# wyhuai/DDNM

Hardware: NVIDIA H100
Metric: restored 256x256 images/sec @100 DDIM steps (higher is better)
Workload: dtype fp32

## Files before the change

ddnm_b200/csrc/api.cu:

```cuda
#include "../../include/ddnm_b200.h"

#include <cstring>
#include <vector>

#include "api_util.cuh"
#include "engine.cuh"
#include "kernels.cuh"
#include "tc_gemm.cuh"

using namespace ddnm;

namespace ddnm {
thread_local std::string g_last_error;
}

extern "C" {

const char* ddnm_last_error(void) { return g_last_error.c_str(); }
int ddnm_version(void) { return 100; }

int ddnm_unet_simple_create(const ddnm_simple_cfg* c, int batch, void** handle) {
  DDNM_API_BEGIN
  DDNM_CHECK(c && handle, "null argument");
  SimpleCfg cfg;
  cfg.ch = c->ch; cfg.out_ch = c->out_ch; cfg.n_levels = c->n_levels;
  DDNM_CHECK(c->n_levels >= 1 && c->n_levels <= 8 && c->n_attn_res >= 0 && c->n_attn_res <= 4, "bad config");
  for (int i = 0; i < 8; ++i) cfg.ch_mult[i] = c->ch_mult[i];
  cfg.num_res_blocks = c->num_res_blocks;
  cfg.n_attn_res = c->n_attn_res;
  for (int i = 0; i < 4; ++i) cfg.attn_res[i] = c->attn_res[i];
  cfg.in_channels = c->in_channels; cfg.resolution = c->resolution; cfg.groups = c->groups; cfg.eps = c->eps;
  *handle = static_cast<UNetEngine*>(new UNetSimple(cfg, batch));
  DDNM_API_END
}

int ddnm_unet_openai_create(const ddnm_openai_cfg* c, int batch, void** handle) {
  DDNM_API_BEGIN
  DDNM_CHECK(c && handle, "null argument");
  DDNM_CHECK(c->n_levels >= 1 && c->n_levels <= 8 && c->n_attn_ds >= 0 && c->n_attn_ds <= 4, "bad config");
  OpenAICfg cfg;
  cfg.image_size = c->image_size; cfg.model_channels = c->model_channels; cfg.num_res_blocks = c->num_res_blocks;
  cfg.n_levels = c->n_levels;
  for (int i = 0; i < 8; ++i) cfg.channel_mult[i] = c->channel_mult[i];
  cfg.n_attn_ds = c->n_attn_ds;
  for (int i = 0; i < 4; ++i) cfg.attn_ds[i] = c->attn_ds[i];
  cfg.num_head_channels = c->num_head_channels; cfg.out_channels = c->out_channels; cfg.in_channels = c->in_channels;
  cfg.groups = c->groups; cfg.eps = c->eps; cfg.num_classes = c->num_classes; cfg.low_res = c->low_res;
  cfg.num_heads = c->num_heads; cfg.num_heads_upsample = c->num_heads_upsample; cfg.new_attention_order = c->new_attention_order;
  DDNM_CHECK(c->num_classes >= 0, "bad num_classes");
  DDNM_CHECK(c->new_attention_order == 0 || c->new_attention_order == 1, "new_attention_order must be 0 or 1");
  DDNM_CHECK(c->num_head_channels > 0 || c->num_heads >= 1, "num_head_channels <= 0 needs num_heads >= 1");
  *handle = static_cast<UNetEngine*>(new UNetOpenAI(cfg, batch));
  DDNM_API_END
}

int ddnm_classifier_create(const ddnm_classifier_cfg* c, int batch, void** handle) {
  DDNM_API_BEGIN
  DDNM_CHECK(c && handle, "null argument");
  DDNM_CHECK(c->n_levels >= 1 && c->n_levels <= 8 && c->n_attn_ds >= 0 && c->n_attn_ds <= 4, "bad config");
  EncoderCfg cfg;
  cfg.image_size = c->image_size; cfg.model_channels = c->model_channels; cfg.num_res_blocks = c->num_res_blocks;
  cfg.n_levels = c->n_levels;
  for (int i = 0; i < 8; ++i) cfg.channel_mult[i] = c->channel_mult[i];
  cfg.n_attn_ds = c->n_attn_ds;
  for (int i = 0; i < 4; ++i) cfg.attn_ds[i] = c->attn_ds[i];
  cfg.num_head_channels = c->num_head_channels; cfg.out_channels = c->out_channels; cfg.in_channels = c->in_channels;
  cfg.groups = c->groups; cfg.eps = c->eps; cfg.pool = c->pool;
  *handle = static_cast<UNetEngine*>(new UNetEncoder(cfg, batch));
  DDNM_API_END
}

static UNetEncoder* as_classifier(void* h) {
  UNetEncoder* e = dynamic_cast<UNetEncoder*>(static_cast<UNetEngine*>(h));
  DDNM_CHECK(e != nullptr, "handle is not a classifier");
  return e;
}

int ddnm_classifier_forward(void* h, const float* x, const float* t, float* logits, void* stream) {
  DDNM_API_BEGIN
  DDNM_CHECK(x && t && logits, "null argument");
  as_classifier(h)->forward(x, t, logits, (cudaStream_t)stream);
  DDNM_API_END
}

int ddnm_classifier_grad(void* h, const float* x, const float* t, const int* labels, float scale, float* grad_out, float* logits_out,
                         void* stream) {
  DDNM_API_BEGIN
  as_classifier(h)->grad(x, t, labels, scale, grad_out, logits_out, (cudaStream_t)stream);
  DDNM_API_END
}

int ddnm_classifier_guidance_fn(void* user, int, int t, void* stream) {
  DDNM_API_BEGIN
  ddnm_classifier_guidance* g = static_cast<ddnm_classifier_guidance*>(user);
  DDNM_CHECK(g && g->classifier && g->x && g->labels && g->grad_buf, "incomplete guidance context");
  UNetEncoder* e = as_classifier(g->classifier);
  DDNM_CHECK(g->batch == e->batch(), "classifier was built for batch " + std::to_string(e->batch()) + ", the guided loop runs " +
                                         std::to_string(g->batch));
  cudaStream_t st = (cudaStream_t)stream;
  if (!g->labels_checked) {
    e->check_labels(g->labels, st);
    g->labels_checked = 1;
  }
  e->fill_t((float)t, st);
  e->grad(g->x, e->t_in(), g->labels, g->scale, g->grad_buf, nullptr, st, true);
  DDNM_API_END
}

int ddnm_unet_set_param(void* h, const char* name, const float* data, long long numel) {
  DDNM_API_BEGIN
  static_cast<UNetEngine*>(h)->set_param(name, data, numel);
  DDNM_API_END
}
int ddnm_unet_finalize(void* h) {
  DDNM_API_BEGIN
  static_cast<UNetEngine*>(h)->finalize();
  DDNM_API_END
}
int ddnm_unet_forward(void* h, const float* x, const float* t, float* out, void* stream) {
  DDNM_API_BEGIN
  static_cast<UNetEngine*>(h)->forward(x, t, out, (cudaStream_t)stream);
  DDNM_API_END
}
int ddnm_unet_forward_cond(void* h, const float* x, const float* t, const int* labels, float* out, void* stream) {
  DDNM_API_BEGIN
  UNetEngine* u = static_cast<UNetEngine*>(h);
  u->set_labels(labels, (cudaStream_t)stream);
  u->forward(x, t, out, (cudaStream_t)stream);
  DDNM_API_END
}
int ddnm_unet_set_low_res(void* h, const float* low_res, void* stream) {
  DDNM_API_BEGIN
  static_cast<UNetEngine*>(h)->set_low_res(low_res, (cudaStream_t)stream);
  DDNM_API_END
}
int ddnm_unet_set_precision(void* h, int fp16_terms) {
  DDNM_API_BEGIN
  static_cast<UNetEngine*>(h)->set_terms(fp16_terms);
  DDNM_API_END
}
int ddnm_unet_set_graph(void* h, int on) {
  DDNM_API_BEGIN
  static_cast<UNetEngine*>(h)->set_use_graph(on != 0);
  DDNM_API_END
}
int ddnm_unet_read_tap(void* h, const char* name, float* dst, long long cap, void* stream) {
  DDNM_API_BEGIN
  DDNM_CHECK(static_cast<UNetEngine*>(h)->read_tap(name, dst, cap, (cudaStream_t)stream), std::string("unknown tap ") + name);
  DDNM_API_END
}
int ddnm_unet_info(void* h, long long* ws, int* launches, double* flops) {
  DDNM_API_BEGIN
  UNetEngine* u = static_cast<UNetEngine*>(h);
  if (ws) *ws = (long long)u->workspace_bytes();
  if (launches) *launches = u->num_launches();
// ... 145 lines not shown

int ddnm_conv_tc_bench(int N, int H, int W, int Cin, int Cout, int mode, int iters, float* ms_per_iter, double* flops) {
  DDNM_API_BEGIN
  const bool random = iters < 0;
  if (random) iters = -iters;
  const int feat = mode >> 4;
  mode &= 15;
  const bool up2 = (feat & 8) != 0;
  Tmp tmp;
  const int taps = up2 ? 4 : (mode == TAPS_1X1 ? 1 : 9);
  const size_t pe = (size_t)N * H * W * Cin;
  SplitView A;
  A.hi = tmp.get<__half>(pe); A.lo = tmp.get<__half>(pe); A.N = N; A.H = H; A.W = W; A.C = Cin;
  float* xf = tmp.get<float>(pe);
  CUDA_CHECK(cudaMemset(xf, 0, pe * 4));
  if (random) bench_fill_f32<<<(unsigned)cdivll((long long)pe, 256), 256>>>(xf, (long long)pe, 0x1234u);
  gn_apply_split(mkview(xf, N, H, W, Cin), 1, false, nullptr, nullptr, 0.f, false, SPLIT_SAME, A.hi, A.lo, 0);
  const int ktot = taps * Cin;
  __half* wh = tmp.get<__half>((size_t)Cout * ktot);
  __half* wl = tmp.get<__half>((size_t)Cout * ktot);
  CUDA_CHECK(cudaMemset(wh, 0, (size_t)Cout * ktot * 2));
  CUDA_CHECK(cudaMemset(wl, 0, (size_t)Cout * ktot * 2));
  if (random) {
    const long long wn = (long long)Cout * ktot;
    bench_fill_split<<<(unsigned)cdivll(wn, 256), 256>>>(wh, wl, wn, 0x9876u, 1.0f / sqrtf((float)ktot));
  }
  const int oH = up2 ? 2 * H : H, oW = up2 ? 2 * W : W;
  const size_t oe = (size_t)N * oH * oW * Cout;
  float* o = tmp.get<float>(oe);
  View ov = mkview(o, N, oH, oW, Cout);
  if (feat & 1) {
    ov.st = tmp.get<StatAcc>((size_t)N * Cout * 2);
    ov.st_ld = Cout;
    CUDA_CHECK(cudaMemset(ov.st, 0, (size_t)N * Cout * 2 * sizeof(StatAcc)));
  }
  float* res = nullptr;
  if (feat & 2) {
    res = tmp.get<float>(oe);
    CUDA_CHECK(cudaMemset(res, 0, oe * 4));
    if (random) bench_fill_f32<<<(unsigned)cdivll((long long)oe, 256), 256>>>(res, (long long)oe, 0x777u);
  }
  float* ca = nullptr;
  if (feat & 4) {
    ca = tmp.get<float>((size_t)N * Cout);
    CUDA_CHECK(cudaMemset(ca, 0, (size_t)N * Cout * 4));
  }
  TcLaunch L = up2 ? tc_make_up2_launch(A, wh, wl, Cout, ov, ca, Cout, 0, 0, sm_count())
                   : tc_make_launch(A, mode, nullptr, wh, wl, 1, Cout, ov, ca, Cout, res, Cout, 1.0f, sm_count());
  for (int i = 0; i < 3; ++i) tc_run(L, 0);
  cudaEvent_t e0, e1;
  CUDA_CHECK(cudaEventCreate(&e0));
  CUDA_CHECK(cudaEventCreate(&e1));
  CUDA_CHECK(cudaEventRecord(e0, 0));
  for (int i = 0; i < iters; ++i) tc_run(L, 0);
  CUDA_CHECK(cudaEventRecord(e1, 0));
  CUDA_CHECK(cudaEventSynchronize(e1));
  float ms = 0;
  CUDA_CHECK(cudaEventElapsedTime(&ms, e0, e1));
  cudaEventDestroy(e0);
  cudaEventDestroy(e1);
  *ms_per_iter = ms / iters;
  *flops = L.flops;
  DDNM_API_END
}

int ddnm_gnconv_chunk_bench(int N, int chunk, int H, int W, int Cin, int Cout, int iters, float* ms_per_pass) {
  DDNM_API_BEGIN
  DDNM_CHECK(chunk >= 1 && N % chunk == 0, "chunk must divide N");
  Tmp tmp;
  const size_t pe = (size_t)N * H * W * Cin, ce = (size_t)chunk * H * W * Cin, oe = (size_t)N * H * W * Cout;
  float* x = tmp.get<float>(pe);
  bench_fill_f32<<<(unsigned)cdivll((long long)pe, 256), 256>>>(x, (long long)pe, 0x4321u);
  StatAcc* st = tmp.get<StatAcc>((size_t)N * Cin * 2);
  CUDA_CHECK(cudaMemset(st, 0, (size_t)N * Cin * 2 * sizeof(StatAcc)));
  View xv = mkview(x, N, H, W, Cin);
  xv.st = st; xv.st_ld = Cin;
  gn_stats(xv, 0);
  float* gamma = tmp.get<float>(Cin);
  float* beta = tmp.get<float>(Cin);
  bench_fill_f32<<<cdiv(Cin, 256), 256>>>(gamma, Cin, 0x11u);
  bench_fill_f32<<<cdiv(Cin, 256), 256>>>(beta, Cin, 0x22u);
  SplitView A;
  A.hi = tmp.get<__half>(ce); A.lo = tmp.get<__half>(ce); A.N = chunk; A.H = H; A.W = W; A.C = Cin;
  const int ktot = 9 * Cin;
  __half* wh = tmp.get<__half>((size_t)Cout * ktot);
  __half* wl = tmp.get<__half>((size_t)Cout * ktot);
  bench_fill_split<<<(unsigned)cdivll((long long)Cout * ktot, 256), 256>>>(wh, wl, (long long)Cout * ktot, 0x9876u, 1.0f / sqrtf((float)ktot));
  float* o = tmp.get<float>(oe);
  StatAcc* ost = tmp.get<StatAcc>((size_t)N * Cout * 2);
  CUDA_CHECK(cudaMemset(ost, 0, (size_t)N * Cout * 2 * sizeof(StatAcc)));
  float* ca = tmp.get<float>((size_t)N * Cout);
  CUDA_CHECK(cudaMemset(ca, 0, (size_t)N * Cout * 4));
  const int nch = N / chunk;
  std::vector<View> xs;
  std::vector<TcLaunch> Ls;
  for (int c = 0; c < nch; ++c) {
    View xc = xv;
    xc.p = x + (size_t)c * chunk * H * W * Cin; xc.N = chunk; xc.st = st + (size_t)c * chunk * Cin * 2;
    View oc = mkview(o + (size_t)c * chunk * H * W * Cout, chunk, H, W, Cout);
    oc.st = ost + (size_t)c * chunk * Cout * 2; oc.st_ld = Cout;
    xs.push_back(xc);
    Ls.push_back(tc_make_launch(A, TAPS_3X3, nullptr, wh, wl, 1, Cout, oc, ca + (size_t)c * chunk * Cout, Cout, nullptr, 0, 1.0f, sm_count()));
  }
  auto pass = [&]() {
    for (int c = 0; c < nch; ++c) {
      gn_apply_split(xs[c], 32, true, gamma, beta, 1e-6f, true, SPLIT_SAME, A.hi, A.lo, 0);
      tc_run(Ls[c], 0);
    }
  };
  for (int i = 0; i < 2; ++i) pass();
  cudaEvent_t e0, e1;
  CUDA_CHECK(cudaEventCreate(&e0));
  CUDA_CHECK(cudaEventCreate(&e1));
  CUDA_CHECK(cudaEventRecord(e0, 0));
  for (int i = 0; i < iters; ++i) pass();
  CUDA_CHECK(cudaEventRecord(e1, 0));
  CUDA_CHECK(cudaEventSynchronize(e1));
  float ms = 0;
  CUDA_CHECK(cudaEventElapsedTime(&ms, e0, e1));
  cudaEventDestroy(e0);
  cudaEventDestroy(e1);
  *ms_per_pass = ms / iters;
  DDNM_API_END
}

int ddnm_groupnorm(const float* x, int N, int H, int W, int C, int groups, const float* gamma, const float* beta, float eps,
                   int silu, float* out, void* stream) {
  DDNM_API_BEGIN
  cudaStream_t s = (cudaStream_t)stream;
  Tmp tmp;
  StatAcc* st = tmp.get<StatAcc>((size_t)N * C * 2);
  CUDA_CHECK(cudaMemsetAsync(st, 0, (size_t)N * C * 2 * sizeof(StatAcc), s));
  View xv = mkview(const_cast<float*>(x), N, H, W, C);
  xv.st = st;
  xv.st_ld = C;
  gn_stats(xv, s);
  gn_apply_f32(xv, groups, gamma, beta, eps, silu != 0, out, s);
  CUDA_CHECK(cudaStreamSynchronize(s));
  DDNM_API_END
}

int ddnm_conv_gn_tc(const float* x, int N, int H, int W, int Cin, int groups, const float* gamma, const float* beta, float eps, int silu,
                    const float* w, const float* bias, int Cout, const float* side_x, int CinSide, const float* side_w,
                    const float* residual, float* out, int iters, float* ms_per_iter, void* stream) {
  DDNM_API_BEGIN
  cudaStream_t s = (cudaStream_t)stream;
  Tmp tmp;
  View xv = mkview(const_cast<float*>(x), N, H, W, Cin);
  StatAcc* st = tmp.get<StatAcc>((size_t)N * Cin * 2);
  CUDA_CHECK(cudaMemsetAsync(st, 0, (size_t)N * Cin * 2 * sizeof(StatAcc), s));
  xv.st = st;
  xv.st_ld = Cin;
  if (gamma) gn_stats(xv, s);
  View sv;
  if (side_x) sv = mkview(const_cast<float*>(side_x), N, H, W, CinSide);
  const int ktot = 9 * Cin + (side_x ? CinSide : 0);
  __half* wh = tmp.get<__half>((size_t)Cout * ktot);
  __half* wl = tmp.get<__half>((size_t)Cout * ktot);
  split_conv_weight(w, Cout, Cin, 9, wh, wl, ktot, 0, s);
  if (side_x) split_conv_weight(side_w, Cout, CinSide, 1, wh, wl, ktot, 9 * Cin, s);
  GnAffine gn;
  gn.gamma = gamma; gn.beta = beta; gn.eps = eps; gn.groups = groups; gn.silu = silu != 0;
  View ov = mkview(out, N, H, W, Cout);
  TcLaunch L = tc_make_gn_launch(xv, gn, side_x ? &sv : nullptr, wh, wl, Cout, ov, bias, 0, residual, Cout, sm_count());
  tc_run(L, s);
  if (iters > 0 && ms_per_iter) {
    cudaEvent_t e0, e1;
    CUDA_CHECK(cudaEventCreate(&e0));
    CUDA_CHECK(cudaEventCreate(&e1));
    for (int i = 0; i < 2; ++i) tc_run(L, s);
    CUDA_CHECK(cudaEventRecord(e0, s));
    for (int i = 0; i < iters; ++i) tc_run(L, s);
    CUDA_CHECK(cudaEventRecord(e1, s));
    CUDA_CHECK(cudaEventSynchronize(e1));
    float ms = 0;
    CUDA_CHECK(cudaEventElapsedTime(&ms, e0, e1));
    cudaEventDestroy(e0);
    cudaEventDestroy(e1);
    *ms_per_iter = ms / iters;
  }
  CUDA_CHECK(cudaStreamSynchronize(s));
  DDNM_API_END
}
int ddnm_tc_debug_gn_fused(int on) {
  DDNM_API_BEGIN
  tc_debug_gn_fused(on);
  DDNM_API_END
}
int ddnm_tc_debug_deal(int mode) {
  DDNM_API_BEGIN
  tc_debug_deal(mode);
  DDNM_API_END
}
int ddnm_tc_debug_pair_mode(int mode) {
  DDNM_API_BEGIN
  tc_debug_pair_mode(mode);
  DDNM_API_END
}
int ddnm_tc_debug_dual_mode(int mode) {
  DDNM_API_BEGIN
  tc_debug_dual_mode(mode);
  DDNM_API_END
}
int ddnm_tc_debug_pair_dual(int on) {
  DDNM_API_BEGIN
  tc_debug_pair_dual(on);
  DDNM_API_END
}
int ddnm_tc_debug_halo(int on) {
  DDNM_API_BEGIN
  tc_debug_halo(on);
  DDNM_API_END
}
int ddnm_tc_debug_pingpong(int on) {
  DDNM_API_BEGIN
  tc_debug_pingpong(on);
  DDNM_API_END
}
int ddnm_tc_debug_force_bn(int bn) {
  DDNM_API_BEGIN
  tc_debug_force_bn(bn);
  DDNM_API_END
}
}
```

ddnm_b200/csrc/common.cuh:

```cuda
#pragma once
#include <cuda_runtime.h>
#include <cuda_fp16.h>
#include <cuda.h>
#include <cstdint>
#include <cstdio>
#include <stdexcept>
#include <string>

namespace ddnm {

struct Error : std::runtime_error {
  using std::runtime_error::runtime_error;
};

#define DDNM_CHECK(cond, msg)                                                                     \
  do {                                                                                            \
    if (!(cond)) throw ::ddnm::Error(std::string(msg) + " [" #cond "] at " __FILE__ ":" + std::to_string(__LINE__)); \
  } while (0)

#define CUDA_CHECK(expr)                                                                          \
  do {                                                                                            \
    cudaError_t _e = (expr);                                                                      \
    if (_e != cudaSuccess)                                                                        \
      throw ::ddnm::Error(std::string("CUDA error: ") + cudaGetErrorString(_e) + " in " #expr " at " __FILE__ ":" + \
// ... 83 lines not shown
__device__ __forceinline__ void pdl_prologue() {
  asm volatile("griddepcontrol.launch_dependents;" ::: "memory");
  asm volatile("griddepcontrol.wait;" ::: "memory");
}
__device__ __forceinline__ uint32_t smem_u32(const void* p) { return (uint32_t)__cvta_generic_to_shared(p); }

__device__ __forceinline__ void mbar_init(uint32_t bar, uint32_t count) {
  asm volatile("mbarrier.init.shared::cta.b64 [%0], %1;" ::"r"(bar), "r"(count));
}
__device__ __forceinline__ void mbar_fence_init() { asm volatile("fence.mbarrier_init.release.cluster;" ::: "memory"); }
__device__ __forceinline__ void mbar_expect_tx(uint32_t bar, uint32_t bytes) {
  asm volatile("mbarrier.arrive.expect_tx.shared::cta.b64 _, [%0], %1;" ::"r"(bar), "r"(bytes) : "memory");
}
__device__ __forceinline__ void mbar_arrive(uint32_t bar) {
  asm volatile("mbarrier.arrive.shared::cta.b64 _, [%0];" ::"r"(bar) : "memory");
}
__device__ __forceinline__ bool mbar_try_wait(uint32_t bar, uint32_t parity) {
  uint32_t ok;
  asm volatile(
      "{\n\t.reg .pred p;\n\t"
      "mbarrier.try_wait.parity.shared::cta.b64 p, [%1], %2;\n\t"
      "selp.u32 %0, 1, 0, p;\n\t}"
      : "=r"(ok)
      : "r"(bar), "r"(parity)
      : "memory");
  return ok != 0;
}
__device__ __forceinline__ void mbar_wait(uint32_t bar, uint32_t parity) {
  if (mbar_try_wait(bar, parity)) return;
  long long t0 = clock64();
  while (!mbar_try_wait(bar, parity)) {
    if (clock64() - t0 > 4000000000LL) __trap();
  }
}

__device__ __forceinline__ void tma_prefetch_desc(const void* tmap) {
  asm volatile("prefetch.tensormap [%0];" ::"l"(tmap) : "memory");
}
__device__ __forceinline__ void tma_load_2d(uint32_t dst, const void* tmap, uint32_t bar, int c0, int c1) {
  asm volatile(
      "cp.async.bulk.tensor.2d.shared::cluster.global.tile.mbarrier::complete_tx::bytes [%0], [%1, {%3, %4}], [%2];" ::"r"(dst),
      "l"(tmap), "r"(bar), "r"(c0), "r"(c1)
      : "memory");
}
__device__ __forceinline__ void tma_load_3d(uint32_t dst, const void* tmap, uint32_t bar, int c0, int c1, int c2) {
  asm volatile(
      "cp.async.bulk.tensor.3d.shared::cluster.global.tile.mbarrier::complete_tx::bytes [%0], [%1, {%3, %4, %5}], [%2];" ::"r"(dst),
      "l"(tmap), "r"(bar), "r"(c0), "r"(c1), "r"(c2)
      : "memory");
}
__device__ __forceinline__ void tma_load_4d(uint32_t dst, const void* tmap, uint32_t bar, int c0, int c1, int c2, int c3) {
  asm volatile(
      "cp.async.bulk.tensor.4d.shared::cluster.global.tile.mbarrier::complete_tx::bytes [%0], [%1, {%3, %4, %5, %6}], [%2];" ::"r"(dst),
      "l"(tmap), "r"(bar), "r"(c0), "r"(c1), "r"(c2), "r"(c3)
      : "memory");
}

__device__ __forceinline__ uint64_t wgmma_desc_sw128(uint32_t saddr) {
  return (uint64_t)((saddr & 0x3FFFFu) >> 4) | ((uint64_t)1 << 16) | ((uint64_t)(1024 >> 4) << 32) | ((uint64_t)1 << 62);
}
__device__ __forceinline__ void wgmma_fence() { asm volatile("wgmma.fence.sync.aligned;" ::: "memory"); }
__device__ __forceinline__ void wgmma_commit() { asm volatile("wgmma.commit_group.sync.aligned;" ::: "memory"); }
template <int N>
__device__ __forceinline__ void wgmma_wait() { asm volatile("wgmma.wait_group.sync.aligned %0;" ::"n"(N) : "memory"); }
__device__ __forceinline__ void wgmma_m64n64k16(float (&d)[32], uint64_t a_desc, uint64_t b_desc, uint32_t accumulate) {
  asm volatile(
      "{\n\t.reg .pred p;\n\t"
      "setp.ne.b32 p, %34, 0;\n\t"
      "wgmma.mma_async.sync.aligned.m64n64k16.f32.f16.f16 "
      "{%0, %1, %2, %3, %4, %5, %6, %7, %8, %9, %10, %11, %12, %13, %14, %15, %16, %17, %18, %19, %20, %21, %22, %23, %24, %25, %26, %27, %28, %29, %30, %31}, "
      "%32, %33, p, 1, 1, 0, 0;\n\t}"
      : "+f"(d[0]), "+f"(d[1]), "+f"(d[2]), "+f"(d[3]), "+f"(d[4]), "+f"(d[5]), "+f"(d[6]), "+f"(d[7]), "+f"(d[8]), "+f"(d[9]), "+f"(d[10]), "+f"(d[11]), "+f"(d[12]), "+f"(d[13]), "+f"(d[14]), "+f"(d[15]), "+f"(d[16]), "+f"(d[17]), "+f"(d[18]), "+f"(d[19]), "+f"(d[20]), "+f"(d[21]), "+f"(d[22]), "+f"(d[23]), "+f"(d[24]), "+f"(d[25]), "+f"(d[26]), "+f"(d[27]), "+f"(d[28]), "+f"(d[29]), "+f"(d[30]), "+f"(d[31])
      : "l"(a_desc), "l"(b_desc), "r"(accumulate));
}
__device__ __forceinline__ void wgmma_m64n128k16(float (&d)[64], uint64_t a_desc, uint64_t b_desc, uint32_t accumulate) {
  asm volatile(
      "{\n\t.reg .pred p;\n\t"
      "setp.ne.b32 p, %66, 0;\n\t"
      "wgmma.mma_async.sync.aligned.m64n128k16.f32.f16.f16 "
      "{%0, %1, %2, %3, %4, %5, %6, %7, %8, %9, %10, %11, %12, %13, %14, %15, %16, %17, %18, %19, %20, %21, %22, %23, %24, %25, %26, %27, %28, %29, %30, %31, %32, %33, %34, %35, %36, %37, %38, %39, %40, %41, %42, %43, %44, %45, %46, %47, %48, %49, %50, %51, %52, %53, %54, %55, %56, %57, %58, %59, %60, %61, %62, %63}, "
      "%64, %65, p, 1, 1, 0, 0;\n\t}"
      : "+f"(d[0]), "+f"(d[1]), "+f"(d[2]), "+f"(d[3]), "+f"(d[4]), "+f"(d[5]), "+f"(d[6]), "+f"(d[7]), "+f"(d[8]), "+f"(d[9]), "+f"(d[10]), "+f"(d[11]), "+f"(d[12]), "+f"(d[13]), "+f"(d[14]), "+f"(d[15]), "+f"(d[16]), "+f"(d[17]), "+f"(d[18]), "+f"(d[19]), "+f"(d[20]), "+f"(d[21]), "+f"(d[22]), "+f"(d[23]), "+f"(d[24]), "+f"(d[25]), "+f"(d[26]), "+f"(d[27]), "+f"(d[28]), "+f"(d[29]), "+f"(d[30]), "+f"(d[31]), "+f"(d[32]), "+f"(d[33]), "+f"(d[34]), "+f"(d[35]), "+f"(d[36]), "+f"(d[37]), "+f"(d[38]), "+f"(d[39]), "+f"(d[40]), "+f"(d[41]), "+f"(d[42]), "+f"(d[43]), "+f"(d[44]), "+f"(d[45]), "+f"(d[46]), "+f"(d[47]), "+f"(d[48]), "+f"(d[49]), "+f"(d[50]), "+f"(d[51]), "+f"(d[52]), "+f"(d[53]), "+f"(d[54]), "+f"(d[55]), "+f"(d[56]), "+f"(d[57]), "+f"(d[58]), "+f"(d[59]), "+f"(d[60]), "+f"(d[61]), "+f"(d[62]), "+f"(d[63])
      : "l"(a_desc), "l"(b_desc), "r"(accumulate));
}
__device__ __forceinline__ void wgmma_m64n256k16(float (&d)[128], uint64_t a_desc, uint64_t b_desc, uint32_t accumulate) {
  asm volatile(
      "{\n\t.reg .pred p;\n\t"
      "setp.ne.b32 p, %130, 0;\n\t"
      "wgmma.mma_async.sync.aligned.m64n256k16.f32.f16.f16 "
      "{%0, %1, %2, %3, %4, %5, %6, %7, %8, %9, %10, %11, %12, %13, %14, %15, %16, %17, %18, %19, %20, %21, %22, %23, %24, %25, %26, %27, %28, %29, %30, %31, %32, %33, %34, %35, %36, %37, %38, %39, %40, %41, %42, %43, %44, %45, %46, %47, %48, %49, %50, %51, %52, %53, %54, %55, %56, %57, %58, %59, %60, %61, %62, %63, %64, %65, %66, %67, %68, %69, %70, %71, %72, %73, %74, %75, %76, %77, %78, %79, %80, %81, %82, %83, %84, %85, %86, %87, %88, %89, %90, %91, %92, %93, %94, %95, %96, %97, %98, %99, %100, %101, %102, %103, %104, %105, %106, %107, %108, %109, %110, %111, %112, %113, %114, %115, %116, %117, %118, %119, %120, %121, %122, %123, %124, %125, %126, %127}, "
      "%128, %129, p, 1, 1, 0, 0;\n\t}"
      : "+f"(d[0]), "+f"(d[1]), "+f"(d[2]), "+f"(d[3]), "+f"(d[4]), "+f"(d[5]), "+f"(d[6]), "+f"(d[7]), "+f"(d[8]), "+f"(d[9]), "+f"(d[10]), "+f"(d[11]), "+f"(d[12]), "+f"(d[13]), "+f"(d[14]), "+f"(d[15]), "+f"(d[16]), "+f"(d[17]), "+f"(d[18]), "+f"(d[19]), "+f"(d[20]), "+f"(d[21]), "+f"(d[22]), "+f"(d[23]), "+f"(d[24]), "+f"(d[25]), "+f"(d[26]), "+f"(d[27]), "+f"(d[28]), "+f"(d[29]), "+f"(d[30]), "+f"(d[31]), "+f"(d[32]), "+f"(d[33]), "+f"(d[34]), "+f"(d[35]), "+f"(d[36]), "+f"(d[37]), "+f"(d[38]), "+f"(d[39]), "+f"(d[40]), "+f"(d[41]), "+f"(d[42]), "+f"(d[43]), "+f"(d[44]), "+f"(d[45]), "+f"(d[46]), "+f"(d[47]), "+f"(d[48]), "+f"(d[49]), "+f"(d[50]), "+f"(d[51]), "+f"(d[52]), "+f"(d[53]), "+f"(d[54]), "+f"(d[55]), "+f"(d[56]), "+f"(d[57]), "+f"(d[58]), "+f"(d[59]), "+f"(d[60]), "+f"(d[61]), "+f"(d[62]), "+f"(d[63]), "+f"(d[64]), "+f"(d[65]), "+f"(d[66]), "+f"(d[67]), "+f"(d[68]), "+f"(d[69]), "+f"(d[70]), "+f"(d[71]), "+f"(d[72]), "+f"(d[73]), "+f"(d[74]), "+f"(d[75]), "+f"(d[76]), "+f"(d[77]), "+f"(d[78]), "+f"(d[79]), "+f"(d[80]), "+f"(d[81]), "+f"(d[82]), "+f"(d[83]), "+f"(d[84]), "+f"(d[85]), "+f"(d[86]), "+f"(d[87]), "+f"(d[88]), "+f"(d[89]), "+f"(d[90]), "+f"(d[91]), "+f"(d[92]), "+f"(d[93]), "+f"(d[94]), "+f"(d[95]), "+f"(d[96]), "+f"(d[97]), "+f"(d[98]), "+f"(d[99]), "+f"(d[100]), "+f"(d[101]), "+f"(d[102]), "+f"(d[103]), "+f"(d[104]), "+f"(d[105]), "+f"(d[106]), "+f"(d[107]), "+f"(d[108]), "+f"(d[109]), "+f"(d[110]), "+f"(d[111]), "+f"(d[112]), "+f"(d[113]), "+f"(d[114]), "+f"(d[115]), "+f"(d[116]), "+f"(d[117]), "+f"(d[118]), "+f"(d[119]), "+f"(d[120]), "+f"(d[121]), "+f"(d[122]), "+f"(d[123]), "+f"(d[124]), "+f"(d[125]), "+f"(d[126]), "+f"(d[127])
      : "l"(a_desc), "l"(b_desc), "r"(accumulate));
}
__device__ __forceinline__ uint32_t cluster_ctarank() {
  uint32_t r;
  asm volatile("mov.u32 %0, %%cluster_ctarank;" : "=r"(r));
  return r;
}
__device__ __forceinline__ uint32_t cluster_id_x() {
  uint32_t r;
  asm volatile("mov.u32 %0, %%clusterid.x;" : "=r"(r));
  return r;
}
__device__ __forceinline__ void cluster_sync_all() {
  asm volatile("barrier.cluster.arrive.release.aligned;" ::: "memory");
  asm volatile("barrier.cluster.wait.acquire.aligned;" ::: "memory");
}
__device__ __forceinline__ void mbar_arrive_cluster(uint32_t bar, uint32_t cta) {
  uint32_t remote;
  asm volatile("mapa.shared::cluster.u32 %0, %1, %2;" : "=r"(remote) : "r"(bar), "r"(cta));
  asm volatile("mbarrier.arrive.release.cluster.shared::cluster.b64 _, [%0];" ::"r"(remote) : "memory");
}
__device__ __forceinline__ void tma_load_3d_multicast(uint32_t dst, const void* tmap, uint32_t bar, int c0, int c1, int c2, uint16_t mask) {
  asm volatile(
      "cp.async.bulk.tensor.3d.shared::cluster.global.mbarrier::complete_tx::bytes.multicast::cluster [%0], [%1, {%3, %4, %5}], [%2], %6;" ::"r"(dst),
      "l"(tmap), "r"(bar), "r"(c0), "r"(c1), "r"(c2), "h"(mask)
      : "memory");
}
__device__ __forceinline__ void named_bar_sync(int id, int threads) { asm volatile("bar.sync %0, %1;" ::"r"(id), "r"(threads) : "memory"); }
template <int R>
__device__ __forceinline__ void setmaxnreg_dec() { asm volatile("setmaxnreg.dec.sync.aligned.u32 %0;" ::"n"(R)); }
template <int R>
__device__ __forceinline__ void setmaxnreg_inc() { asm volatile("setmaxnreg.inc.sync.aligned.u32 %0;" ::"n"(R)); }

__device__ __forceinline__ void stat_add(StatAcc* acc, float p) {
  const int bits = __float_as_int(p);
  int ex = (bits >> 23) & 0xff;
  unsigned long long m = (unsigned long long)(bits & 0x7fffff);
  if (ex) m |= 0x800000ull; else ex = 1;
  const int sh = ex - 150 + 48;
  unsigned long long lo = 0, hi = 0;
  if (sh >= 64) hi = m << min(sh - 64, 7);
  else if (sh > 0) { lo = m << sh; hi = sh > 40 ? m >> (64 - sh) : 0ull; }
  else if (sh > -24) lo = m >> (-sh);
  if (bits < 0) {
    lo = ~lo + 1ull;
    hi = ~hi + (lo == 0ull ? 1ull : 0ull);
  }
  const unsigned long long w0 = lo & 0xffffffffull;
  const unsigned long long w1 = (hi << 32) | (lo >> 32);
  if (w0) atomicAdd(&acc->lo, w0);
  if (w1) atomicAdd(reinterpret_cast<unsigned long long*>(&acc->hi), w1);
}
__device__ __forceinline__ void two_sum_acc(float& sum, float& comp, float v) {
  const float s = __fadd_rn(sum, v);
  const float bb = __fadd_rn(s, -sum);
  comp = __fadd_rn(comp, __fadd_rn(__fadd_rn(sum, -__fadd_rn(s, -bb)), __fadd_rn(v, -bb)));
  sum = s;
}
__device__ __forceinline__ double stat_value(const StatAcc& a) {
  return ((double)a.hi * 4294967296.0 + (double)a.lo) * (1.0 / 281474976710656.0);
}

__device__ __forceinline__ float swishf_fast(float x) {
  float e;
  asm("ex2.approx.ftz.f32 %0, %1;" : "=f"(e) : "f"(x * -1.4426950408889634f));
  return __fdividef(x, 1.0f + e);
}
__device__ __forceinline__ void split_f16(float x, __half& hi, __half& lo) {
  unsigned short h;
  asm("cvt.rn.satfinite.f16.f32 %0, %1;" : "=h"(h) : "f"(x));
  hi = __ushort_as_half(h);
  float r = x - __half2float(hi);
  asm("cvt.rn.satfinite.f16.f32 %0, %1;" : "=h"(h) : "f"(r));
  lo = __ushort_as_half(h);
}
__device__ __forceinline__ void split2_f16(float x0, float x1, uint32_t& hi, uint32_t& lo) {
  asm("cvt.rn.satfinite.f16x2.f32 %0, %1, %2;" : "=r"(hi) : "f"(x1), "f"(x0));
  const __half2 h = *reinterpret_cast<const __half2*>(&hi);
  const float2 f = __half22float2(h);
  asm("cvt.rn.satfinite.f16x2.f32 %0, %1, %2;" : "=r"(lo) : "f"(x1 - f.y), "f"(x0 - f.x));
}

#endif

}
```

ddnm_b200/csrc/engine.cu:

```cuda
#include "engine.cuh"

#include <algorithm>
#include <cmath>
#include <cstdlib>
#include <sstream>

#include "kernels.cuh"

namespace ddnm {

Arena::~Arena() {
  for (void* b : blocks_) cudaFree(b);
}
void* Arena::alloc(size_t bytes) {
  bytes = (bytes + 1023) / 1024 * 1024;
  if (bytes == 0) bytes = 1024;
  void* p = nullptr;
  CUDA_CHECK(cudaMalloc(&p, bytes));
  blocks_.push_back(p);
  total_ += bytes;
  return p;
}

UNetEngine::UNetEngine(int batch, int in_channels, int out_ch, int resolution, int groups, float eps)
    : B_(batch), in_ch_(in_channels), out_ch_(out_ch), R_(resolution), groups_(groups), eps_(eps) {
  DDNM_CHECK(batch >= 1, "batch must be positive");
  int dev = 0;
  CUDA_CHECK(cudaGetDevice(&dev));
  cudaDeviceProp prop;
  CUDA_CHECK(cudaGetDeviceProperties(&prop, dev));
  DDNM_CHECK(prop.major == 9 && prop.minor == 0, "ddnm_b200 kernels are built for sm_90a (H100) only");
  num_sms_ = prop.multiProcessorCount;
}

UNetEngine::~UNetEngine() {
  if (graph_exec_) cudaGraphExecDestroy(graph_exec_);
  if (graph_) cudaGraphDestroy(graph_);
  for (auto& kv : params_) cudaFree(kv.second.p);
}

void UNetEngine::set_param(const std::string& name, const float* data, long long numel) {
  DDNM_CHECK(!finalized_, "set_param after finalize");
  DDNM_CHECK(numel > 0 && data != nullptr, "empty parameter " + name);
  float* d = nullptr;
  CUDA_CHECK(cudaMalloc(&d, (size_t)numel * sizeof(float)));
  CUDA_CHECK(cudaMemcpy(d, data, (size_t)numel * sizeof(float), cudaMemcpyDefault));
  auto it = params_.find(name);
  if (it != params_.end()) cudaFree(it->second.p);
  params_[name] = Param{d, numel};
}

const float* UNetEngine::P(const std::string& name, long long expect) const {
  auto it = params_.find(name);
  DDNM_CHECK(it != params_.end(), "missing parameter '" + name + "'");
  if (expect >= 0)
    DDNM_CHECK(it->second.n == expect, "parameter '" + name + "' has " + std::to_string(it->second.n) + " elements, expected " +
                                           std::to_string(expect));
  return it->second.p;
}

View UNetEngine::new_view(int H, int W, int C) {
  View v;
  v.N = B_; v.H = H; v.W = W; v.C = C; v.ld = C;
  v.p = (float*)arena_.alloc((size_t)B_ * H * W * C * sizeof(float));
  v.st = new_stats(C);
  v.st_ld = C;
  return v;
}

StatAcc* UNetEngine::new_stats(int C) {
  const size_t need = (size_t)B_ * C * 2;
  if (stats_chunks_.empty() || stats_chunks_.back().used + need > stats_chunks_.back().cap) {
    StatsChunk c;
    c.cap = std::max<size_t>(need, (size_t)1 << 20);
    c.used = 0;
    c.p = (StatAcc*)arena_.alloc(c.cap * sizeof(StatAcc));
    stats_chunks_.push_back(c);
  }
  StatsChunk& c = stats_chunks_.back();
  StatAcc* p = c.p + c.used;
  c.used += need;
  return p;
}

UNetEngine::TcWeights UNetEngine::prep_weights(const std::string& main, int Cout, int Cin, int taps, const std::string& side,
                                               int CinSide) {
  TcWeights w;
  w.ktot = taps * Cin + CinSide;
  const size_t n = (size_t)Cout * w.ktot;
  w.hi = (__half*)arena_.alloc(n * sizeof(__half));
  w.lo = (__half*)arena_.alloc(n * sizeof(__half));
  split_conv_weight(P(main, (long long)Cout * Cin * taps), Cout, Cin, taps, w.hi, w.lo, w.ktot, 0, 0);
  if (CinSide) split_conv_weight(P(side, (long long)Cout * CinSide), Cout, CinSide, 1, w.hi, w.lo, w.ktot, taps * Cin, 0);
  return w;
}

const float* UNetEngine::bias_sum(const std::string& a, const std::string& b, int C) {
  std::vector<float> ha(C), hb(C, 0.f);
  CUDA_CHECK(cudaMemcpy(ha.data(), P(a, C), C * sizeof(float), cudaMemcpyDeviceToHost));
  if (!b.empty()) CUDA_CHECK(cudaMemcpy(hb.data(), P(b, C), C * sizeof(float), cudaMemcpyDeviceToHost));
  for (int i = 0; i < C; ++i) ha[i] += hb[i];
  float* d = (float*)arena_.alloc(C * sizeof(float));
  CUDA_CHECK(cudaMemcpy(d, ha.data(), C * sizeof(float), cudaMemcpyHostToDevice));
  return d;
}

float* UNetEngine::dev_copy(const std::vector<float>& v) {
  float* d = (float*)arena_.alloc(v.size() * sizeof(float));
  CUDA_CHECK(cudaMemcpy(d, v.data(), v.size() * sizeof(float), cudaMemcpyHostToDevice));
  return d;
}

void UNetEngine::add_op(const std::string& name, const std::string& kind, double flops, double bytes,
                        std::function<void(cudaStream_t)> f) {
  ops_.push_back(OpRecord{name, kind, flops, bytes, std::move(f)});
}

void UNetEngine::emit_gn_split(const std::string& name, const View& x, const std::string& norm, bool silu, int mode,
                               SplitView& dst, const float* ss, int ss_ld, SplitView* raw) {
  const long long out_elems = mode == SPLIT_AVG2 ? x.pixels() * x.C / 4 : x.pixels() * x.C;
  DDNM_CHECK((size_t)out_elems <= split_elems_, "split scratch too small");
  dst.C = x.C;
  if (mode == SPLIT_SAME) { dst.N = x.N; dst.H = x.H; dst.W = x.W; }
  else if (mode == SPLIT_AVG2) { dst.N = x.N; dst.H = x.H / 2; dst.W = x.W / 2; }
  else { dst.N = 4 * x.N; dst.H = x.H / 2; dst.W = x.W / 2; }
  const double in_bytes = (double)x.pixels() * x.C * 4;
  if (!norm.empty()) {
    DDNM_CHECK(x.st != nullptr, "GroupNorm input without producer-side statistics: " + name);
    const float* g = P(norm + ".weight", x.C);
    const float* b = P(norm + ".bias", x.C);
    const int groups = groups_;
    const float eps = eps_;
    __half *hi = dst.hi, *lo = dst.lo, *rhi = nullptr, *rlo = nullptr;
    if (raw) {
      DDNM_CHECK(mode == SPLIT_SAME, "raw side output only with the plain split");
      raw->N = x.N; raw->H = x.H; raw->W = x.W; raw->C = x.C;
      rhi = raw->hi; rlo = raw->lo;
    }
    add_op(name + ".gn_split", "gn_split", 0, in_bytes + out_elems * 4.0 * (raw ? 2 : 1),
           [=](cudaStream_t s) { gn_apply_split(x, groups, true, g, b, eps, silu, mode, hi, lo, s, ss, ss_ld, rhi, rlo); });
  } else {
    __half *hi = dst.hi, *lo = dst.lo;
    add_op(name + ".split", "gn_split", 0, in_bytes + out_elems * 4.0,
           [=](cudaStream_t s) { gn_apply_split(x, 1, false, nullptr, nullptr, 0.f, silu, mode, hi, lo, s); });
  }
}

void UNetEngine::emit_tc(const std::string& name, const SplitView& a, int mode, const SplitView* side, const TcWeights& w,
                         int Cout, const View& out, const float* chanadd, int ca_ld, const float* residual, int ldr, int res_mode) {
  TcLaunch L = tc_make_launch(a, mode, side, w.hi, w.lo, 1, Cout, out, chanadd, ca_ld, residual, ldr, 1.0f, num_sms_, res_mode);
  const double bytes = (double)a.N * a.H * a.W * a.C * 4 + (side ? (double)side->N * side->H * side->W * side->C * 4 : 0) +
                       (double)Cout * w.ktot * 4 + (double)out.pixels() * Cout * 4 * (residual ? 2 : 1);
  const int tiles = L.p.tiles_x * L.p.tiles_y * L.p.tiles_n * L.p.n_tiles, kblocks = L.p.kb0 + L.p.kb1;
  static const bool split_on = std::getenv("DDNM_SPLITK") == nullptr || std::atoi(std::getenv("DDNM_SPLITK")) != 0;
  if (split_on && !L.pair && res_mode == 0 && 2 * tiles <= num_sms_ && kblocks >= 32) {
    const int S = 4 * tiles <= num_sms_ ? 4 : 2;
    const long long stride = out.pixels() * Cout;
    float* part = (float*)arena_.alloc((size_t)S * stride * sizeof(float));
    View pv;
    pv.p = part; pv.N = out.N; pv.H = out.H; pv.W = out.W; pv.C = Cout; pv.ld = Cout;
    TcLaunch Ls = tc_make_launch(a, mode, side, w.hi, w.lo, 1, Cout, pv, nullptr, 0, nullptr, 0, 1.0f, num_sms_, 0);
    DDNM_CHECK(!Ls.pair && Ls.BN == L.BN, "split-K: tile shape changed");
    Ls.p.split_k = S;
    Ls.p.split_stride = stride;
    Ls.halo = false;
    Ls.grid = std::min(tiles * S, num_sms_);
    add_op(name, "tc", L.flops, bytes, [Ls](cudaStream_t s) { tc_run(Ls, s); });
    add_op(name + ".splitk_reduce", "reduce", 0, (double)(S + 1 + (residual ? 1 : 0)) * stride * 4,
           [=](cudaStream_t s) { splitk_reduce(part, S, stride, out, chanadd, ca_ld, residual, ldr, s); });
    return;
  }
  add_op(name, "tc", L.flops, bytes, [L](cudaStream_t s) { tc_run(L, s); });
}

bool UNetEngine::fused_ok(const View& x, const View* side, int Cout, const View& out) const {
  return terms_ == 3 && x.st != nullptr && tc_gn_eligible(x, side, Cout, out);
}

void UNetEngine::emit_tcgn(const std::string& name, const View& x, const std::string& norm, const float* ss, int ss_ld, const View* side,
                           const TcWeights& w, int Cout, const View& out, const float* chanadd, int ca_ld, const float* residual, int ldr) {
  GnAffine gn;
  gn.gamma = P(norm + ".weight", x.C);
  gn.beta = P(norm + ".bias", x.C);
  gn.eps = eps_;
  gn.groups = groups_;
  gn.silu = true;
  gn.ss = ss;
  gn.ss_ld = ss_ld;
  TcLaunch L = tc_make_gn_launch(x, gn, side, w.hi, w.lo, Cout, out, chanadd, ca_ld, residual, ldr, num_sms_);
  const double bytes = (double)x.pixels() * x.C * 4 + (side ? (double)side->pixels() * side->C * 4 : 0) + (double)Cout * w.ktot * 4 +
                       (double)out.pixels() * Cout * 4 * (residual ? 2 : 1);
  add_op(name, "tc", L.flops, bytes, [L](cudaStream_t s) { tc_run(L, s); });
}

void UNetEngine::alloc_common(size_t split_elems, size_t hbuf_elems) {
  split_elems_ = split_elems;
  hbuf_elems_ = hbuf_elems;
  splitA_hi_ = (__half*)arena_.alloc(split_elems * 2);
  splitA_lo_ = (__half*)arena_.alloc(split_elems * 2);
  splitB_hi_ = (__half*)arena_.alloc(split_elems * 2);
  splitB_lo_ = (__half*)arena_.alloc(split_elems * 2);
  hbuf_ = (float*)arena_.alloc(hbuf_elems * 4);
  x_in_ = (float*)arena_.alloc((size_t)B_ * in_ch_ * R_ * R_ * 4);
  t_in_ = (float*)arena_.alloc((size_t)B_ * 4);
  labels_in_ = (int*)arena_.alloc((size_t)B_ * 4);
  CUDA_CHECK(cudaMemset(labels_in_, 0, (size_t)B_ * 4));
  out_ = (float*)arena_.alloc((size_t)B_ * out_ch_ * R_ * R_ * 4);
  if (lowres_ > 0) lowres_in_ = (float*)arena_.alloc((size_t)B_ * in_ch_ * lowres_ * lowres_ * 4);
}

void UNetEngine::emit_up2_conv(const std::string& name, const SplitView& a, const std::string& wname, int Cout, const View& out,
                               const float* chanadd, int ca_ld) {
  const int Cin = a.C;
  const size_t per_phase = (size_t)Cout * 4 * Cin;
  __half* wh = (__half*)arena_.alloc(4 * per_phase * sizeof(__half));
  __half* wl = (__half*)arena_.alloc(4 * per_phase * sizeof(__half));
  presum_up2_weights(P(wname, (long long)Cout * Cin * 9), Cout, Cin, wh, wl, 0);
  for (int ph = 0; ph < 4; ++ph) {
    TcLaunch L = tc_make_up2_launch(a, wh + ph * per_phase, wl + ph * per_phase, Cout, out, chanadd, ca_ld, ph >> 1, ph & 1, num_sms_);
    const double bytes = (double)a.N * a.H * a.W * Cin * 4 + (double)per_phase * 4 + (double)a.N * a.H * a.W * Cout * 4;
    add_op(name + ".ph" + std::to_string(ph), "tc", L.flops, bytes, [L](cudaStream_t s) { tc_run(L, s); });
  }
}

void UNetEngine::alloc_attention(size_t qkv_elems, size_t s_elems, size_t o_elems) {
  qkv_ = (float*)arena_.alloc(qkv_elems * 4);
  attS_ = (float*)arena_.alloc(s_elems * 4);
  attO_ = (float*)arena_.alloc(o_elems * 4);
  qkvh_ = (__half*)arena_.alloc(qkv_elems * 2);
  qkvl_ = (__half*)arena_.alloc(qkv_elems * 2);
  ph_ = (__half*)arena_.alloc(s_elems * 2);
  pl_ = (__half*)arena_.alloc(s_elems * 2);
  vth_ = (__half*)arena_.alloc(o_elems * 2);
  vtl_ = (__half*)arena_.alloc(o_elems * 2);
}

void UNetEngine::emit_attention_core(const std::string& name, int T, int heads, int ch, int qkv_ld, int head_stride, int q_off,
                                     int k_off, int v_off, float alpha) {
  float *q = qkv_, *S = attS_, *O = attO_;
  const int Bn = B_, C = heads * ch;
  const long long img = (long long)T * qkv_ld;
  const double fl = 2.0 * Bn * heads * (double)T * T * ch;
  const double sbytes = (double)Bn * heads * T * T * 4;
  if (T % 128 == 0 && ch % 8 == 0) {
    __half *qh = qkvh_, *ql = qkvl_, *ph = ph_, *pl = pl_, *vh = vth_, *vl = vtl_;
    DDNM_CHECK(qkv_ld % C == 0, "qkv row is not a multiple of the attention width");
    View qv;
    qv.p = qkv_; qv.N = B_; qv.H = 1; qv.W = T * (qkv_ld / C); qv.C = C; qv.ld = C;
    add_op(name + ".qkv_split", "gn_split", 0, (double)Bn * T * qkv_ld * 8,
           [=](cudaStream_t s) { gn_apply_split(qv, 1, false, nullptr, nullptr, 0.f, false, SPLIT_SAME, qh, ql, s); });
    const long long hs = head_stride ? head_stride : qkv_ld;
    GemmOperand A{qh + q_off, ql + q_off, qkv_ld, hs, img};
    GemmOperand Bk{qh + k_off, ql + k_off, qkv_ld, hs, img};
    TcLaunch L1 = tc_make_gemm_launch(A, Bk, T, T, ch, heads, Bn, S, (long long)heads * T * T, (long long)T * T, T, alpha, num_sms_);
    add_op(name + ".qk", "tc", L1.flops, (double)Bn * T * qkv_ld * 4 + sbytes, [L1](cudaStream_t s) { tc_run(L1, s); });
    add_op(name + ".softmax", "softmax", 0, sbytes * 2, [=](cudaStream_t s) { softmax_split(S, (long long)Bn * heads * T, T, ph, pl, s); });
    add_op(name + ".v_transpose", "gn_split", 0, (double)Bn * T * C * 8,
           [=](cudaStream_t s) { transpose_split(q, qkv_ld, head_stride, v_off, Bn, T, heads, ch, vh, vl, s); });
    GemmOperand P{ph, pl, T, (long long)T * T, (long long)heads * T * T};
    GemmOperand Vt{vh, vl, T, (long long)ch * T, (long long)heads * ch * T};
    TcLaunch L2 = tc_make_gemm_launch(P, Vt, T, ch, T, heads, Bn, O, (long long)T * C, ch, C, 1.0f, num_sms_);
    add_op(name + ".pv", "tc", L2.flops, sbytes + (double)Bn * T * C * 8, [L2](cudaStream_t s) { tc_run(L2, s); });
  } else {
    add_op(name + ".qk", "sgemm", fl, (double)Bn * heads * T * (2.0 * ch + T) * 4, [=](cudaStream_t s) {
      sgemm_batched(true, Bn, heads, T, T, ch, alpha, q + q_off, qkv_ld, img, head_stride, q + k_off, qkv_ld, img, head_stride, S, T,
                    (long long)heads * T * T, (long long)T * T, s);
    });
    add_op(name + ".softmax", "softmax", 0, sbytes * 2, [=](cudaStream_t s) { softmax_rows(S, (long long)Bn * heads * T, T, s); });
    add_op(name + ".pv", "sgemm", fl, (double)Bn * heads * T * (2.0 * ch + T) * 4, [=](cudaStream_t s) {
      sgemm_batched(false, Bn, heads, T, ch, T, 1.0f, S, T, (long long)heads * T * T, (long long)T * T, q + v_off, qkv_ld, img, head_stride, O,
                    C, (long long)T * C, ch, s);
    });
  }
}

void UNetEngine::emit_stem(const std::string& wname, const View& out) {
  const float* xin = x_in_;
  if (lowres_ > 0) {
    const float *w = P(wname + ".weight", (long long)out.C * 2 * in_ch_ * 9), *b = P(wname + ".bias", out.C);
    const float* lr = lowres_in_;
    const int cin = in_ch_, s = lowres_;
    add_op("stem.sr", "stem", 2.0 * B_ * R_ * R_ * (double)out.C * 2 * cin * 9,
           (double)B_ * (R_ * R_ * (cin + out.C) + (double)s * s * cin) * 4,
           [=](cudaStream_t st) { conv3x3_stem_sr(xin, lr, cin, s, s, w, b, out, st); });
    return;
  }
  const float *w = P(wname + ".weight", (long long)out.C * in_ch_ * 9), *b = P(wname + ".bias", out.C);
  const int cin = in_ch_;
  add_op("stem", "stem", 2.0 * B_ * R_ * R_ * (double)out.C * cin * 9, (double)B_ * R_ * R_ * (cin + out.C) * 4,
         [=](cudaStream_t s) { conv3x3_small_cin(xin, cin, w, b, out, s); });
}

void UNetEngine::emit_head(const std::string& norm, const std::string& conv, const View& fh) {
  DDNM_CHECK(fh.st != nullptr, "head input without statistics");
  DDNM_CHECK(out_ch_ <= 64, "head convolution: out_ch <= 64");
  if (head_conv_supported(fh, out_ch_) && std::getenv("DDNM_HEAD_TC") == nullptr) {
    const float *g = P(norm + ".weight", fh.C), *b = P(norm + ".bias", fh.C);
    const float *w = P(conv + ".weight", (long long)out_ch_ * fh.C * 9), *cb = P(conv + ".bias", out_ch_);
    const int groups = groups_, oc = out_ch_;
    const float eps = eps_;
    float* o = out_;
    add_op("head.conv", "head", 2.0 * fh.pixels() * (double)oc * fh.C * 9, (double)fh.pixels() * (fh.C + oc) * 4,
           [=](cudaStream_t s) { head_conv(fh, groups, g, b, eps, w, cb, oc, o, s); });
    return;
  }
  SplitView A{splitA_hi_, splitA_lo_};
  emit_gn_split("head", fh, norm, true, SPLIT_SAME, A);
  const int ktot = 9 * fh.C;
  TcWeights w;
  w.ktot = ktot;
  w.hi = (__half*)arena_.alloc((size_t)64 * ktot * sizeof(__half));
  w.lo = (__half*)arena_.alloc((size_t)64 * ktot * sizeof(__half));
  CUDA_CHECK(cudaMemset(w.hi, 0, (size_t)64 * ktot * sizeof(__half)));
  CUDA_CHECK(cudaMemset(w.lo, 0, (size_t)64 * ktot * sizeof(__half)));
  split_conv_weight(P(conv + ".weight", (long long)out_ch_ * fh.C * 9), out_ch_, fh.C, 9, w.hi, w.lo, ktot, 0, 0);
  std::vector<float> hb(64, 0.f);
  CUDA_CHECK(cudaMemcpy(hb.data(), P(conv + ".bias", out_ch_), out_ch_ * sizeof(float), cudaMemcpyDeviceToHost));
  float* bias64 = dev_copy(hb);
  View o64;
  o64.N = B_; o64.H = fh.H; o64.W = fh.W; o64.C = 64; o64.ld = 64;
  o64.p = (float*)arena_.alloc((size_t)B_ * fh.H * fh.W * 64 * sizeof(float));
  emit_tc("head.conv", A, TAPS_3X3, nullptr, w, 64, o64, bias64, 0, nullptr, 0);
  float* o = out_;
  const View real = o64.slice(0, out_ch_);
  add_op("head.to_nchw", "head", 0, (double)fh.pixels() * (64 + out_ch_) * 4, [=](cudaStream_t s) { nhwc_to_nchw(real, o, s); });
}

void UNetEngine::set_terms(int t) {
  DDNM_CHECK(!finalized_, "precision must be chosen before finalize");
  DDNM_CHECK(t == 1 || t == 3, "terms must be 1 (fast fp16) or 3 (fp32-grade)");
  terms_ = t;
}

void UNetEngine::finalize() {
  DDNM_CHECK(!finalized_, "finalize called twice");
  const int prev = tc_get_terms();
  tc_set_terms(terms_);
  try {
    build_program();
  } catch (...) {
    tc_set_terms(prev);
    throw;
  }
  tc_set_terms(prev);
// ... 113 lines not shown
```

ddnm_b200/csrc/engine.cuh:

```cuda
#pragma once
#include <functional>
#include <map>
#include <memory>
#include <string>
#include <vector>

#include "common.cuh"
#include "tc_gemm.cuh"

namespace ddnm {

struct SimpleCfg {
  int ch = 128, out_ch = 3, n_levels = 6;
  int ch_mult[8] = {1, 1, 2, 2, 4, 4, 0, 0};
  int num_res_blocks = 2;
  int n_attn_res = 1;
  int attn_res[4] = {16, 0, 0, 0};
  int in_channels = 3, resolution = 256, groups = 32;
  float eps = 1e-6f;
};

class Arena {
 public:
  ~Arena();
  void* alloc(size_t bytes);
  size_t used() const { return total_; }

 private:
  std::vector<void*> blocks_;
  size_t total_ = 0;
};

struct OpRecord {
  std::string name;
  std::string kind;
  double flops = 0;
  double bytes = 0;
  std::function<void(cudaStream_t)> run;
};

struct OpenAICfg {
  int image_size = 256, model_channels = 256, num_res_blocks = 2, n_levels = 6;
  int channel_mult[8] = {1, 1, 2, 2, 4, 4, 0, 0};
  int n_attn_ds = 3;
  int attn_ds[4] = {8, 16, 32, 0};
  int num_head_channels = 64;
  int out_channels = 6, in_channels = 3, groups = 32;
  float eps = 1e-5f;
  int num_classes = 0;
  int low_res = 0;
  int num_heads = 1, num_heads_upsample = -1;
  int new_attention_order = 0;
};

class UNetEngine {
 public:
  UNetEngine(int batch, int in_channels, int out_ch, int resolution, int groups, float eps);
  virtual ~UNetEngine();
  void set_param(const std::string& name, const float* data, long long numel);
  void finalize();
  void forward(const float* x, const float* t, float* out, cudaStream_t stream);
  bool read_tap(const std::string& name, float* dst_nchw, long long capacity, cudaStream_t stream);
  std::string profile(const float* x, const float* t, float* out, cudaStream_t stream);
  int batch() const { return B_; }
  int out_ch() const { return out_ch_; }
  int in_channels() const { return in_ch_; }
  int resolution() const { return R_; }
  float* x_in() const { return x_in_; }
  float* t_in() const { return t_in_; }
  int* labels_in() const { return labels_in_; }
  bool class_conditional() const { return class_cond_; }
  void set_labels(const int* labels_dev, cudaStream_t stream);
  int low_res_size() const { return lowres_; }
  void set_low_res(const float* low_res_dev, cudaStream_t stream);
  float* out_buf() const { return out_; }
  void set_use_graph(bool on) { use_graph_ = on; }
  void set_terms(int t);
  size_t workspace_bytes() const { return arena_.used(); }
  int num_launches() const { return (int)ops_.size(); }
  double flops_per_forward() const;

 protected:
  struct Param { float* p; long long n; };
  const float* P(const std::string& name, long long expect = -1) const;
  View new_view(int H, int W, int C);
  StatAcc* new_stats(int C);
  struct TcWeights { __half *hi, *lo; int ktot; };
  TcWeights prep_weights(const std::string& main, int Cout, int Cin, int taps, const std::string& side, int CinSide);
  const float* bias_sum(const std::string& a, const std::string& b, int C);
  float* dev_copy(const std::vector<float>& v);
  bool has_param(const std::string& name) const { return params_.count(name) != 0; }

  void add_op(const std::string& name, const std::string& kind, double flops, double bytes, std::function<void(cudaStream_t)> f);
  void emit_gn_split(const std::string& name, const View& x, const std::string& norm, bool silu, int mode, SplitView& dst,
                     const float* ss = nullptr, int ss_ld = 0, SplitView* raw = nullptr);
  void emit_tc(const std::string& name, const SplitView& a, int mode, const SplitView* side, const TcWeights& w, int Cout,
               const View& out, const float* chanadd, int ca_ld, const float* residual, int ldr, int res_mode = 0);
  bool fused_ok(const View& x, const View* side, int Cout, const View& out) const;
  void emit_tcgn(const std::string& name, const View& x, const std::string& norm, const float* ss, int ss_ld, const View* side,
                 const TcWeights& w, int Cout, const View& out, const float* chanadd, int ca_ld, const float* residual, int ldr);
  void emit_attention_core(const std::string& name, int T, int heads, int ch, int qkv_ld, int head_stride, int q_off, int k_off,
                           int v_off, float alpha);
  void alloc_attention(size_t qkv_elems, size_t s_elems, size_t o_elems);
  void emit_up2_conv(const std::string& name, const SplitView& a, const std::string& wname, int Cout, const View& out,
                     const float* chanadd, int ca_ld);
  void emit_stem(const std::string& wname, const View& out);
  void emit_head(const std::string& norm, const std::string& conv, const View& h);
  void alloc_common(size_t split_elems, size_t hbuf_elems);
  virtual void build_program() = 0;
  virtual size_t out_elems() const { return (size_t)B_ * out_ch_ * R_ * R_; }
  void run_ops(cudaStream_t s, size_t n = (size_t)-1);
  void replay(cudaStream_t stream, size_t n, cudaGraph_t& g, cudaGraphExec_t& exec);

  int B_, in_ch_, out_ch_, R_, groups_;
  float eps_;
  int num_sms_ = 132;
  bool finalized_ = false, use_graph_ = true;
  int terms_ = 3;
  Arena arena_;
  std::map<std::string, Param> params_;
  std::vector<OpRecord> ops_;
  size_t n_tail_ops_ = 0;
  std::map<std::string, View> taps_;
  float *x_in_ = nullptr, *t_in_ = nullptr, *out_ = nullptr;
  int* labels_in_ = nullptr;
  bool class_cond_ = false;
  float* lowres_in_ = nullptr;
  int lowres_ = 0;
  bool lowres_set_ = false;
  __half *splitA_hi_ = nullptr, *splitA_lo_ = nullptr, *splitB_hi_ = nullptr, *splitB_lo_ = nullptr;
  size_t split_elems_ = 0;
  float* hbuf_ = nullptr;
  size_t hbuf_elems_ = 0;
  float *qkv_ = nullptr, *attS_ = nullptr, *attO_ = nullptr;
  __half *qkvh_ = nullptr, *qkvl_ = nullptr, *ph_ = nullptr, *pl_ = nullptr, *vth_ = nullptr, *vtl_ = nullptr;
  struct StatsChunk { StatAcc* p; size_t cap, used; };
  std::vector<StatsChunk> stats_chunks_;
  float *emb_ = nullptr, *temb0_ = nullptr, *temb_ = nullptr, *ca_all_ = nullptr, *freq_ = nullptr;
  int ca_total_ = 0;
  std::map<std::string, int> ca_off_;
  float *tembW_all_ = nullptr, *tembB_all_ = nullptr;
  cudaGraph_t graph_ = nullptr;
  cudaGraphExec_t graph_exec_ = nullptr;
};

class UNetSimple : public UNetEngine {
 public:
  UNetSimple(const SimpleCfg& cfg, int batch);

 private:
  void build_program() override;
  void emit_resblock(const std::string& p, const View& x, const View& out);
  void emit_attn(const std::string& p, const View& x, const View& out);
  void emit_downsample(const std::string& p, const View& x, const View& out);
  void emit_upsample(const std::string& p, const View& x, const View& out);
  SimpleCfg cfg_;
};

class UNetOpenAI : public UNetEngine {
 public:
  UNetOpenAI(const OpenAICfg& cfg, int batch);

 private:
  enum ResKind { RES_PLAIN = 0, RES_DOWN = 1, RES_UP = 2 };
  void build_program() override;
  void emit_resblock(const std::string& p, const View& x, const View& out, int kind);
  int attn_heads(int C, bool upsample) const;
  void emit_attn(const std::string& p, const View& x, const View& out, int heads);
  OpenAICfg cfg_;
  float* ss_all_ = nullptr;
  int ss_total_ = 0;
  std::map<std::string, int> ss_off_;
  float *embW_all_ = nullptr, *embB_all_ = nullptr;
};

struct EncoderCfg {
  int image_size = 256, model_channels = 128, num_res_blocks = 2, n_levels = 6;
  int channel_mult[8] = {1, 1, 2, 2, 4, 4, 0, 0};
  int n_attn_ds = 3;
  int attn_ds[4] = {8, 16, 32, 0};
  int num_head_channels = 64;
  int out_channels = 1000, in_channels = 3, groups = 32;
  float eps = 1e-5f;
  int pool = 1;
};

class UNetEncoder : public UNetEngine {
 public:
  UNetEncoder(const EncoderCfg& cfg, int batch);
  ~UNetEncoder() override;
  void grad(const float* x, const float* t, const int* labels, float scale, float* grad_out, float* logits, cudaStream_t stream,
            bool labels_checked = false);
  void check_labels(const int* labels, cudaStream_t stream) const;
  void fill_t(float t, cudaStream_t stream);
  int num_classes() const { return cfg_.out_channels; }

 private:
  void build_program() override;
  size_t out_elems() const override { return (size_t)B_ * cfg_.out_channels; }
  struct Res { std::string p; View x, h, out; bool down, skip_conv; };
  struct Attn { std::string p; View x, out; float* qkv; };
  struct Layer { int kind; Res r; Attn a; };
  void emit_resblock(const std::string& p, const View& x, const View& out, bool down, Layer& rec);
  void emit_attn(const std::string& p, const View& x, const View& out, Layer& rec);
  void emit_head(const View& h);
  void emit_backward(const View& stem_out, const std::vector<Layer>& layers, const View& top);
  void emit_gn_backward(const std::string& name, const float* g, const View& x, const std::string& norm, const float* ss, int ss_ld,
                        bool silu, bool pool, const float* add, bool add_pool, float* dx32, const SplitView& dst);
  TcWeights prep_weights_t(const std::string& w, int Cout, int Cin, int taps);
  EncoderCfg cfg_;
  float* ss_all_ = nullptr;
  int ss_total_ = 0;
  std::map<std::string, int> ss_off_;
  float *embW_all_ = nullptr, *embB_all_ = nullptr;
  int headT_ = 0;
  float *hf_ = nullptr, *tok_ = nullptr, *hqkv_ = nullptr, *hp_ = nullptr, *ha0_ = nullptr;
  float *scale_in_ = nullptr, *grad_ = nullptr, *gx_[2] = {nullptr, nullptr}, *g1_ = nullptr, *g2_ = nullptr, *gqkv_ = nullptr;
  float *sP_ = nullptr, *sdP_ = nullptr, *gnb_part_ = nullptr;
  size_t gnb_part_elems_ = 0;
  cudaGraph_t ggraph_ = nullptr;
  cudaGraphExec_t ggraph_exec_ = nullptr;
};

}
```

ddnm_b200/csrc/kernels.cu:

```cuda
#include <cstdlib>

#include "kernels.cuh"
#include "tc_gemm.cuh"

namespace ddnm {

static constexpr int MAX_C = 2048;

bool pdl_enabled() {
  static const bool on = [] {
    const char* v = std::getenv("DDNM_PDL");
    return !(v && v[0] == '0');
  }();
  return on;
}

__device__ __forceinline__ float swishf(float x) { return x / (1.0f + expf(-x)); }

__global__ void gn_stats_kernel(const float* __restrict__ x, int HW, int C, int ld, int pix_per_cta,
                                StatAcc* __restrict__ stats, int st_ld) {
  pdl_prologue();
  const int n = blockIdx.y;
  const int C4 = C >> 2;
  const int rows = blockDim.x / C4;
  const int c4 = threadIdx.x % C4;
  const int prow = threadIdx.x / C4;
  const int p0 = blockIdx.x * pix_per_cta;
  const int p1 = min(HW, p0 + pix_per_cta);
  float s[4] = {0, 0, 0, 0}, q[4] = {0, 0, 0, 0};
  if (prow < rows) {
    const float* base = x + (long long)n * HW * ld + c4 * 4;
    const size_t step = (size_t)rows * ld;
    int p = p0 + prow;
    const float* ptr = base + (size_t)p * ld;
    for (; p + 3 * rows < p1; p += 4 * rows, ptr += 4 * step) {
      const float4 v0 = __ldg(reinterpret_cast<const float4*>(ptr));
      const float4 v1 = __ldg(reinterpret_cast<const float4*>(ptr + step));
      const float4 v2 = __ldg(reinterpret_cast<const float4*>(ptr + 2 * step));
      const float4 v3 = __ldg(reinterpret_cast<const float4*>(ptr + 3 * step));
      s[0] += (v0.x + v1.x) + (v2.x + v3.x); q[0] += (v0.x * v0.x + v1.x * v1.x) + (v2.x * v2.x + v3.x * v3.x);
      s[1] += (v0.y + v1.y) + (v2.y + v3.y); q[1] += (v0.y * v0.y + v1.y * v1.y) + (v2.y * v2.y + v3.y * v3.y);
      s[2] += (v0.z + v1.z) + (v2.z + v3.z); q[2] += (v0.z * v0.z + v1.z * v1.z) + (v2.z * v2.z + v3.z * v3.z);
      s[3] += (v0.w + v1.w) + (v2.w + v3.w); q[3] += (v0.w * v0.w + v1.w * v1.w) + (v2.w * v2.w + v3.w * v3.w);
    }
    for (; p < p1; p += rows, ptr += step) {
      const float4 v = __ldg(reinterpret_cast<const float4*>(ptr));
      s[0] += v.x; q[0] += v.x * v.x;
      s[1] += v.y; q[1] += v.y * v.y;
      s[2] += v.z; q[2] += v.z * v.z;
      s[3] += v.w; q[3] += v.w * v.w;
    }
#pragma unroll
    for (int j = 0; j < 4; ++j) {
      StatAcc* d = stats + ((size_t)n * st_ld + c4 * 4 + j) * 2;
      stat_add(d, s[j]);
      stat_add(d + 1, q[j]);
    }
  }
}

void gn_stats(const View& x, cudaStream_t st) {
  DDNM_CHECK(x.C % 4 == 0 && x.C <= MAX_C && x.ld % 4 == 0 && x.st != nullptr, "gn_stats: unsupported channel count / no stats slot");
  const int C4 = x.C / 4;
  const int rows = std::max(1, 256 / C4);
  const int threads = C4 * rows;
  const int HW = x.H * x.W;
  long long want = cdivll((long long)HW * x.N, 592);
  int ppc = (int)std::max<long long>(rows * 4, cdivll(want, rows) * rows);
  dim3 grid(cdiv(HW, ppc), x.N);
  launch_pdl(gn_stats_kernel, grid, dim3(threads), 0, st, 1, (const float*)x.p, HW, x.C, x.ld, ppc, x.st, x.st_ld);
  CUDA_CHECK(cudaGetLastError());
}

template <bool F32OUT>
__global__ void gn_apply_kernel(const float* __restrict__ x, int H, int W, int C, int ld, int N, int groups,
                                const StatAcc* __restrict__ stats, int st_ld, const float* __restrict__ gamma,
                                const float* __restrict__ beta, float eps, int silu, int mode, int pix_per_cta,
                                __half* __restrict__ hi, __half* __restrict__ lo, float* __restrict__ out32,
                                const float* __restrict__ ss, int ss_ld, __half* __restrict__ raw_hi,
                                __half* __restrict__ raw_lo) {
  pdl_prologue();
  extern __shared__ double gn_smem[];
  double* sd = gn_smem;
  float* sc = reinterpret_cast<float*>(gn_smem + 2 * (size_t)C);
  float* sh = sc + C;
  const int n = blockIdx.y;
  const int HW = H * W;
  if (stats) {
    const int cpg = C / groups;
    const double cnt = (double)HW * cpg;
    const StatAcc* gsrc = stats + (size_t)n * st_ld * 2;
    for (int c = threadIdx.x; c < 2 * C; c += blockDim.x) sd[c] = stat_value(gsrc[c]);
    __syncthreads();
    for (int c = threadIdx.x; c < C; c += blockDim.x) {
      const int g0 = (c / cpg) * cpg;
      double s1 = 0, s2 = 0;
      for (int j = 0; j < cpg; ++j) {
        s1 += sd[2 * (g0 + j)];
        s2 += sd[2 * (g0 + j) + 1];
      }
      const double mean = s1 / cnt;
      double var = s2 / cnt - mean * mean;
      var = var < 0 ? 0 : var;
      const float rstd = (float)(1.0 / sqrt(var + (double)eps));
      float a = rstd * gamma[c];
      float b = beta[c] - (float)mean * a;
      if (ss) {
        const float one_plus = 1.0f + ss[(size_t)n * ss_ld + c];
        a *= one_plus;
        b = fmaf(b, one_plus, ss[(size_t)n * ss_ld + C + c]);
      }
      sc[c] = a;
      sh[c] = b;
    }
  } else {
    for (int c = threadIdx.x; c < C; c += blockDim.x) {
      sc[c] = 1.f;
      sh[c] = 0.f;
    }
  }
  __syncthreads();
  const int C8 = C >> 3;
  const int rows = blockDim.x / C8;
  const int c8 = threadIdx.x % C8, prow = threadIdx.x / C8;
  if (prow >= rows) return;
  const int c = c8 * 8;
  float a8[8], b8[8];
#pragma unroll
  for (int j = 0; j < 8; ++j) { a8[j] = sc[c + j]; b8[j] = sh[c + j]; }
  const int p0 = blockIdx.x * pix_per_cta;
  if (mode == SPLIT_AVG2) {
    const int Wo = W >> 1, HWo = (H >> 1) * Wo;
    const int q1 = min(HWo, p0 + pix_per_cta);
    for (int q = p0 + prow; q < q1; q += rows) {
      const int oy = q / Wo, ox = q - oy * Wo;
      float acc[8] = {0, 0, 0, 0, 0, 0, 0, 0};
#pragma unroll
      for (int d = 0; d < 4; ++d) {
        const float* sp = x + ((size_t)n * HW + (size_t)(2 * oy + (d >> 1)) * W + 2 * ox + (d & 1)) * ld + c;
        const float4 a = __ldg(reinterpret_cast<const float4*>(sp));
        const float4 b = __ldg(reinterpret_cast<const float4*>(sp + 4));
        float v[8] = {a.x, a.y, a.z, a.w, b.x, b.y, b.z, b.w};
#pragma unroll
        for (int j = 0; j < 8; ++j) {
          v[j] = fmaf(v[j], a8[j], b8[j]);
          if (silu) v[j] = swishf_fast(v[j]);
          acc[j] += v[j];
        }
      }
      __align__(16) __half h8[8];
      __align__(16) __half l8[8];
#pragma unroll
      for (int j = 0; j < 8; ++j) split_f16(acc[j] * 0.25f, h8[j], l8[j]);
      const size_t o = ((size_t)n * HWo + q) * C + c;
      *reinterpret_cast<uint4*>(hi + o) = *reinterpret_cast<const uint4*>(h8);
      *reinterpret_cast<uint4*>(lo + o) = *reinterpret_cast<const uint4*>(l8);
    }
    return;
  }
  const int p1 = min(HW, p0 + pix_per_cta);
  const float* src = x + ((size_t)n * HW + p0 + prow) * ld + c;
  const size_t step = (size_t)rows * ld;
  float4 a = make_float4(0.f, 0.f, 0.f, 0.f), b = a;
  if (p0 + prow < p1) {
    a = __ldg(reinterpret_cast<const float4*>(src));
    b = __ldg(reinterpret_cast<const float4*>(src + 4));
  }
  for (int p = p0 + prow; p < p1; p += rows, src += step) {
    float v[8] = {a.x, a.y, a.z, a.w, b.x, b.y, b.z, b.w};
    if (p + rows < p1) {
      a = __ldg(reinterpret_cast<const float4*>(src + step));
      b = __ldg(reinterpret_cast<const float4*>(src + step + 4));
    }
    if (!F32OUT && raw_hi) {
      uint4 rh, rl;
      split2_f16(v[0], v[1], rh.x, rl.x);
      split2_f16(v[2], v[3], rh.y, rl.y);
      split2_f16(v[4], v[5], rh.z, rl.z);
      split2_f16(v[6], v[7], rh.w, rl.w);
      const size_t o = ((size_t)n * HW + p) * C + c;
      *reinterpret_cast<uint4*>(raw_hi + o) = rh;
      *reinterpret_cast<uint4*>(raw_lo + o) = rl;
    }
#pragma unroll
    for (int j = 0; j < 8; ++j) {
      v[j] = fmaf(v[j], a8[j], b8[j]);
      if (silu) v[j] = swishf_fast(v[j]);
    }
    if (F32OUT) {
      float* d = out32 + ((size_t)n * HW + p) * C + c;
      *reinterpret_cast<float4*>(d) = make_float4(v[0], v[1], v[2], v[3]);
      *reinterpret_cast<float4*>(d + 4) = make_float4(v[4], v[5], v[6], v[7]);
    } else {
      uint4 hv, lv;
      split2_f16(v[0], v[1], hv.x, lv.x);
      split2_f16(v[2], v[3], hv.y, lv.y);
      split2_f16(v[4], v[5], hv.z, lv.z);
      split2_f16(v[6], v[7], hv.w, lv.w);
      if (mode == SPLIT_SAME) {
        const size_t o = ((size_t)n * HW + p) * C + c;
        *reinterpret_cast<uint4*>(hi + o) = hv;
        *reinterpret_cast<uint4*>(lo + o) = lv;
      } else {
        const int y = p / W, xx = p - y * W;
        {
          const int ph = (y & 1) * 2 + (xx & 1);
          const int Hh = H >> 1, Wh = W >> 1;
          const size_t o = ((((size_t)ph * N + n) * Hh + (y >> 1)) * Wh + (xx >> 1)) * C + c;
          *reinterpret_cast<uint4*>(hi + o) = hv;
          *reinterpret_cast<uint4*>(lo + o) = lv;
        }
      }
    }
  }
}

static void gn_apply_launch(const View& x, int groups, bool normalise, const float* gamma, const float* beta, float eps,
                            bool silu, int mode, __half* hi, __half* lo, float* out32, cudaStream_t st, const float* ss, int ss_ld,
                            __half* raw_hi = nullptr, __half* raw_lo = nullptr) {
  if (raw_hi) DDNM_CHECK(mode == SPLIT_SAME && raw_lo && !out32, "raw side output only with the plain split");
  DDNM_CHECK(x.C % 8 == 0 && x.C <= MAX_C && x.ld % 4 == 0, "gn_apply: unsupported channel count");
  if (mode == SPLIT_S2D || mode == SPLIT_AVG2) DDNM_CHECK(x.H % 2 == 0 && x.W % 2 == 0, "space-to-depth / avg-pool need even dims");
  const StatAcc* stats = normalise ? x.st : nullptr;
  if (normalise) DDNM_CHECK(x.st != nullptr && x.C % groups == 0, "normalisation needs the tensor's per-channel sums (View::st)");
  if (ss) DDNM_CHECK(normalise, "scale-shift needs a normalisation");
  const int HW = mode == SPLIT_AVG2 ? x.H * x.W / 4 : x.H * x.W;
  const int C8 = x.C / 8;
  const int rows = std::max(1, 256 / C8);
  const int threads = C8 * rows;
  int dev = 0, sms = 0;
  CUDA_CHECK(cudaGetDevice(&dev));
  CUDA_CHECK(cudaDeviceGetAttribute(&sms, cudaDevAttrMultiProcessorCount, dev));
  long long want = cdivll((long long)HW * x.N, (long long)sms * 8);
  int ppc = (int)std::max<long long>(rows, cdivll(want, rows) * rows);
  dim3 grid(cdiv(HW, ppc), x.N);
  const size_t smem = (size_t)x.C * 24;
  if (out32)
    launch_pdl(gn_apply_kernel<true>, grid, dim3(threads), smem, st, 1, (const float*)x.p, x.H, x.W, x.C, x.ld, x.N, groups, stats, x.st_ld, gamma,
               beta, eps, (int)silu, mode, ppc, (__half*)nullptr, (__half*)nullptr, out32, ss, ss_ld, (__half*)nullptr, (__half*)nullptr);
  else
    launch_pdl(gn_apply_kernel<false>, grid, dim3(threads), smem, st, 1, (const float*)x.p, x.H, x.W, x.C, x.ld, x.N, groups, stats, x.st_ld, gamma,
               beta, eps, (int)silu, mode, ppc, hi, lo, (float*)nullptr, ss, ss_ld, raw_hi, raw_lo);
  CUDA_CHECK(cudaGetLastError());
}

void gn_apply_split(const View& x, int groups, bool normalise, const float* gamma, const float* beta, float eps,
                    bool silu, int mode, __half* hi, __half* lo, cudaStream_t s, const float* ss, int ss_ld, __half* raw_hi,
                    __half* raw_lo) {
  gn_apply_launch(x, groups, normalise, gamma, beta, eps, silu, mode, hi, lo, nullptr, s, ss, ss_ld, raw_hi, raw_lo);
}
void gn_apply_f32(const View& x, int groups, const float* gamma, const float* beta, float eps, bool silu, float* out,
                  cudaStream_t s) {
  gn_apply_launch(x, groups, true, gamma, beta, eps, silu, SPLIT_SAME, nullptr, nullptr, out, s, nullptr, 0);
}

template <int CIN>
__global__ void __launch_bounds__(256) conv_small_cin_kernel(const float* __restrict__ x, const float* __restrict__ w,
                                                             const float* __restrict__ bias, float* __restrict__ out,
                                                             int H, int W, int Cout, int ld, StatAcc* __restrict__ stats, int st_ld) {
  pdl_prologue();
  constexpr int KT = CIN * 9;
  constexpr int TW = 64, TH = 8;
  __shared__ float tile[CIN][TH + 2][TW + 2];
  __shared__ float red[TH][128][2];
  const int slabs = (Cout + 127) / 128;
  const int n = blockIdx.z / slabs;
  const int slab = blockIdx.z % slabs;
// ... 809 lines not shown
```

ddnm_b200/csrc/tc_gemm.cu:

```cuda
#include "tc_gemm.cuh"

#include <cstdlib>

namespace ddnm {

static constexpr int BM = 128;
static constexpr int kConsumerThreads = 256;
static constexpr int kTcThreads = kConsumerThreads + 32;
static constexpr int BK = 64;
static constexpr int A_PLANE_BYTES = BM * BK * 2;
static constexpr int kGnMaxC = 512;

static constexpr int HALO_PLANE_BYTES = 17 * 1024;
static constexpr int HALO_UNITS = 2;

template <int BN, bool DUAL, bool HALO = false>
struct TcCfg {
  static constexpr int B_PLANE_BYTES = BN * BK * 2;
  static constexpr int A_UNIT_BYTES = 2 * HALO_PLANE_BYTES;
  static constexpr int A_RING_BYTES = HALO ? HALO_UNITS * A_UNIT_BYTES : 0;
  static constexpr int STAGE_BYTES = (HALO ? 0 : 2 * A_PLANE_BYTES) + 2 * B_PLANE_BYTES;
  static constexpr int STAGES = (HALO || BN == 64) ? 4 : 3;
  static constexpr int RING_BYTES = A_RING_BYTES + STAGES * STAGE_BYTES;
  static constexpr int PART_BYTES = 8 * BN * 8;
  static constexpr int RUN_BYTES = 4 * 2 * BN * 8;
  static constexpr int GN_BYTES = 2 * kGnMaxC * 4;
  static constexpr int SMEM_BYTES = RING_BYTES + 1024  + 256  + PART_BYTES + RUN_BYTES + GN_BYTES;
  static constexpr int ACC = DUAL ? BN : BN / 2;
  static_assert(SMEM_BYTES <= 227 * 1024, "shared memory capacity");
};

template <int N, int R>
__device__ __forceinline__ void wgmma_tile(float (&d)[R], uint64_t a, uint64_t b, uint32_t accumulate) {
  static_assert(N / 2 <= R, "accumulator too small");
  if constexpr (N == 64) wgmma_m64n64k16(*reinterpret_cast<float(*)[32]>(&d[0]), a, b, accumulate);
  else if constexpr (N == 128) wgmma_m64n128k16(*reinterpret_cast<float(*)[64]>(&d[0]), a, b, accumulate);
  else wgmma_m64n256k16(*reinterpret_cast<float(*)[128]>(&d[0]), a, b, accumulate);
}

__device__ __forceinline__ void gn_store_row(uint8_t* a_hi, int row, int chunk0, const float (&v)[32]) {
#pragma unroll
  for (int q = 0; q < 4; ++q) {
    uint4 h, l;
    split2_f16(v[8 * q + 0], v[8 * q + 1], h.x, l.x);
    split2_f16(v[8 * q + 2], v[8 * q + 3], h.y, l.y);
    split2_f16(v[8 * q + 4], v[8 * q + 5], h.z, l.z);
    split2_f16(v[8 * q + 6], v[8 * q + 7], h.w, l.w);
    const int off = row * 128 + (((chunk0 + q) ^ (row & 7)) << 4);
    *reinterpret_cast<uint4*>(a_hi + off) = h;
    *reinterpret_cast<uint4*>(a_hi + A_PLANE_BYTES + off) = l;
  }
}

__device__ __forceinline__ void tc_decode(const TcParams& p, int tile, int& n_idx, int& x0, int& y0, int& n0) {
  n_idx = tile % p.n_tiles;
  const int m = tile / p.n_tiles;
  const int tx = m % p.tiles_x;
  const int t2 = m / p.tiles_x;
  const int ty = t2 % p.tiles_y;
  const int tn = t2 / p.tiles_y;
  x0 = tx * p.bw;
  y0 = ty * p.bh;
  n0 = tn * p.bn;
}

template <int STAGES>
struct TcBars {
  uint32_t base;
  __device__ uint32_t full(int s) const { return base + 8u * s; }
  __device__ uint32_t empty(int s) const { return base + 8u * (STAGES + s); }
  __device__ uint32_t a_full(int u) const { return base + 8u * (2 * STAGES + u); }
  __device__ uint32_t a_empty(int u) const { return base + 8u * (2 * STAGES + HALO_UNITS + u); }
  __device__ uint32_t turn(int w) const { return base + 8u * (2 * STAGES + 2 * HALO_UNITS + w); }
};

struct TcRing {
  uint32_t stage = 0, phase = 0;
  uint32_t aunit = 0, aphase = 0;
};

template <class Cfg, bool PAIR, bool GN, bool HALO>
__device__ __forceinline__ void tc_produce_tile(const CUtensorMap* tm_a0h, const CUtensorMap* tm_a0l, const CUtensorMap* tm_a1h,
                                                const CUtensorMap* tm_a1l, const CUtensorMap* tm_bh, const CUtensorMap* tm_bl,
                                                const TcParams& p, uint32_t smem_base, TcBars<Cfg::STAGES> bars, int tile, int kb_lo,
                                                int kb_hi, uint32_t rank, TcRing& r) {
  const int halo_r = p.mode0 == TAPS_UP2X2 ? 2 : 3;
  const int halo_w = p.bw + halo_r - 1;
  const bool lo = p.terms != 1;
  const uint32_t planes = lo ? 2u : 1u;
  const uint32_t stage_tx = (GN || HALO) ? planes * Cfg::B_PLANE_BYTES : (uint32_t)(lo ? Cfg::STAGE_BYTES : Cfg::STAGE_BYTES / 2);
  int n_idx, x0, y0, n0;
  tc_decode(p, tile, n_idx, x0, y0, n0);
  const int bz = p.b_batched == 1 ? n0 : 0;
  for (int kb = kb_lo; kb < kb_hi; ++kb) {
    int bkb = kb;
    if constexpr (HALO) {
      const int ua = kb / halo_r, dx = kb - ua * halo_r, dy = ua / p.cb0, cs = ua - dy * p.cb0;
      bkb = (dy * halo_r + dx) * p.cb0 + cs;
      if (dx == 0) {
        mbar_wait(bars.a_empty(r.aunit), r.aphase ^ 1u);
        const uint32_t ua_s = smem_base + r.aunit * Cfg::A_UNIT_BYTES;
        const uint32_t fa = bars.a_full(r.aunit);
        const int cy = y0 + dy - 1 + p.up_py, cx = x0 - 1 + p.up_px;
        mbar_expect_tx(fa, planes * (uint32_t)(halo_w * p.bh * 128));
        tma_load_4d(ua_s, tm_a0h, fa, cs * BK, cx, cy, n0);
        if (lo) tma_load_4d(ua_s + HALO_PLANE_BYTES, tm_a0l, fa, cs * BK, cx, cy, n0);
      }
      if (dx == halo_r - 1) {
        if (++r.aunit == HALO_UNITS) {
          r.aunit = 0;
          r.aphase ^= 1u;
        }
      }
    }
    mbar_wait(bars.empty(r.stage), r.phase ^ 1u);
    const uint32_t sa = smem_base + Cfg::A_RING_BYTES + r.stage * Cfg::STAGE_BYTES;
    const uint32_t sb = HALO ? sa : sa + 2 * A_PLANE_BYTES;
    const uint32_t fb = bars.full(r.stage);
    mbar_expect_tx(fb, stage_tx);
    if (GN || HALO) {
    } else if (kb < p.kb0) {
      const int tap = kb / p.cb0;
      const int c = (kb - tap * p.cb0) * BK;
      int cx = x0, cy = y0, cn = n0;
      if (p.mode0 == TAPS_3X3) {
        cy += tap / 3 - 1;
        cx += tap % 3 - 1;
      } else if (p.mode0 == TAPS_UP2X2) {
        cy += tap / 2 + p.up_py - 1;
        cx += tap % 2 + p.up_px - 1;
      } else if (p.mode0 == TAPS_3X3_S2) {
        const int dy = tap / 3, dx = tap % 3;
        cy += dy >> 1;
        cx += dx >> 1;
        cn += ((dy & 1) * 2 + (dx & 1)) * p.phase_stride;
      }
      tma_load_4d(sa, tm_a0h, fb, c, cx, cy, cn);
      if (lo) tma_load_4d(sa + A_PLANE_BYTES, tm_a0l, fb, c, cx, cy, cn);
    } else {
      const int c = (kb - p.kb0) * BK;
      tma_load_4d(sa, tm_a1h, fb, c, x0, y0, n0);
      if (lo) tma_load_4d(sa + A_PLANE_BYTES, tm_a1l, fb, c, x0, y0, n0);
    }
    if (PAIR) {
      constexpr int BN = Cfg::B_PLANE_BYTES / (BK * 2);
      const uint32_t half = rank * (BN / 2) * 128u;
      const int brow = n_idx * BN + (int)rank * (BN / 2);
      tma_load_3d_multicast(sb + half, tm_bh, fb, kb * BK, brow, 0, (uint16_t)3);
      if (lo) tma_load_3d_multicast(sb + Cfg::B_PLANE_BYTES + half, tm_bl, fb, kb * BK, brow, 0, (uint16_t)3);
    } else if (p.b_batched == 2) {
      constexpr int BN = Cfg::B_PLANE_BYTES / (BK * 2);
      tma_load_4d(sb, tm_bh, fb, kb * BK, n_idx * BN, y0, n0);
      if (lo) tma_load_4d(sb + Cfg::B_PLANE_BYTES, tm_bl, fb, kb * BK, n_idx * BN, y0, n0);
    } else {
      constexpr int BN = Cfg::B_PLANE_BYTES / (BK * 2);
      tma_load_3d(sb, tm_bh, fb, bkb * BK, n_idx * BN, bz);
      if (lo) tma_load_3d(sb + Cfg::B_PLANE_BYTES, tm_bl, fb, bkb * BK, n_idx * BN, bz);
    }
    if (++r.stage == Cfg::STAGES) {
      r.stage = 0;
      r.phase ^= 1u;
    }
  }
}

template <int BN, bool DUAL, bool NTAIL, int R>
__device__ __forceinline__ void tc_epilogue_rows(const TcParams& p, float (&d)[R], bool dual, int r0, int cq, int n_idx, int x0,
                                                 int y0, int n0, int split_off) {
  const int ppi = p.bw * p.bh;
  float* orow[2];
  const float* rrow[2];
  const float* crow[2];
  bool valid[2];
#pragma unroll
  for (int h = 0; h < 2; ++h) {
    const int r = r0 + 8 * h;
    const int xi = r % p.bw, yi = (r / p.bw) % p.bh, ni = r / ppi;
    const int n = n0 + ni;
    valid[h] = n < p.N;
    orow[h] = p.out + (long long)n * p.out_sn + (long long)(y0 + yi) * p.out_sy + (long long)(x0 + xi) * p.out_sx + n_idx * BN +
              (long long)split_off * p.split_stride;
    rrow[h] = nullptr;
    if (p.residual) {
      long long rp;
      if (p.res_mode == 0) rp = ((long long)n * p.H + (y0 + yi)) * p.W + (x0 + xi);
      else if (p.res_mode == 1) rp = ((long long)n * (p.H >> 1) + ((y0 + yi) >> 1)) * (p.W >> 1) + ((x0 + xi) >> 1);
      else rp = ((long long)n * (2 * p.H) + 2 * (y0 + yi)) * (2 * p.W) + 2 * (x0 + xi);
      rrow[h] = p.residual + rp * p.ldr + n_idx * BN;
    }
    crow[h] = p.chanadd ? p.chanadd + (long long)n * p.ca_ld + n_idx * BN : nullptr;
  }
#pragma unroll
  for (int j = 0; j < BN / 8; ++j) {
    const int c = 8 * j + cq;
#pragma unroll
    for (int h = 0; h < 2; ++h) {
      float a0 = d[4 * j + 2 * h], a1 = d[4 * j + 2 * h + 1];
      if constexpr (DUAL) {
        if (dual) {
          a0 += d[4 * (j + BN / 8) + 2 * h];
          a1 += d[4 * (j + BN / 8) + 2 * h + 1];
        }
      }
      float v0 = p.alpha * a0, v1 = p.alpha * a1;
      if (crow[h] && valid[h]) {
        const float2 cv = __ldg(reinterpret_cast<const float2*>(crow[h] + c));
        v0 += cv.x;
        v1 += cv.y;
      }
      if (rrow[h] && valid[h]) {
        float2 rv = __ldg(reinterpret_cast<const float2*>(rrow[h] + c));
        if (p.res_mode == 2) {
          const long long r_dx = p.ldr, r_dy = (long long)2 * p.W * p.ldr;
          const float2 q1 = __ldg(reinterpret_cast<const float2*>(rrow[h] + r_dx + c));
          const float2 q2 = __ldg(reinterpret_cast<const float2*>(rrow[h] + r_dy + c));
          const float2 q3 = __ldg(reinterpret_cast<const float2*>(rrow[h] + r_dy + r_dx + c));
          rv.x = ((rv.x + q1.x) + (q2.x + q3.x)) * 0.25f;
          rv.y = ((rv.y + q1.y) + (q2.y + q3.y)) * 0.25f;
        }
        v0 += rv.x;
        v1 += rv.y;
      }
      if (!valid[h]) v0 = v1 = 0.f;
      d[4 * j + 2 * h] = v0;
      d[4 * j + 2 * h + 1] = v1;
      if (valid[h] && (!NTAIL || n_idx * BN + c < p.Cout)) *reinterpret_cast<float2*>(orow[h] + c) = make_float2(v0, v1);
    }
  }
}

template <int BN, int R>
__device__ __forceinline__ void tc_stats_rows(const float (&d)[R], float2* part, int lane, int cq) {
#pragma unroll
  for (int j = 0; j < BN / 8; ++j) {
#pragma unroll
    for (int e = 0; e < 2; ++e) {
      const float a = d[4 * j + e], b = d[4 * j + 2 + e];
      float s = a + b, q = a * a + b * b;
#pragma unroll
      for (int k = 4; k <= 16; k <<= 1) {
        s += __shfl_xor_sync(0xffffffffu, s, k);
        q += __shfl_xor_sync(0xffffffffu, q, k);
      }
      if (lane < 4) part[8 * j + cq + e] = make_float2(s, q);
    }
  }
}

template <int BN, bool PAIR, bool DUAL, bool GN, bool HALO, bool NTAIL>
__global__ void __launch_bounds__(kTcThreads, 1)
conv_tc_kernel(const __grid_constant__ CUtensorMap tm_a0h, const __grid_constant__ CUtensorMap tm_a0l,
               const __grid_constant__ CUtensorMap tm_a1h, const __grid_constant__ CUtensorMap tm_a1l,
               const __grid_constant__ CUtensorMap tm_bh, const __grid_constant__ CUtensorMap tm_bl, const TcParams p,
               const TcGnArgs g) {
  static_assert(!GN || !PAIR, "the GN form runs on single CTAs");
  static_assert(!HALO || (!PAIR && !GN), "the HALO form runs on single CTAs with TMA-loaded A");
  using Cfg = TcCfg<BN, DUAL, HALO>;
  constexpr int STAGES = Cfg::STAGES;
  extern __shared__ uint8_t smem_raw[];
  const uint32_t smem_base = (smem_u32(smem_raw) + 1023u) & ~1023u;
  const uint32_t bar_base = smem_base + Cfg::RING_BYTES;
  const TcBars<STAGES> bars{bar_base};
  auto full_bar = [&](int s) { return bars.full(s); };
  auto empty_bar = [&](int s) { return bars.empty(s); };
  auto a_full_bar = [&](int u) { return bars.a_full(u); };
  auto a_empty_bar = [&](int u) { return bars.a_empty(u); };
  const int halo_r = p.mode0 == TAPS_UP2X2 ? 2 : 3;
  const int halo_w = p.bw + halo_r - 1;
  uint8_t* stat_smem = smem_raw + (bar_base + 256u - smem_u32(smem_raw));
  float2* part = reinterpret_cast<float2*>(stat_smem);
  float2* run = reinterpret_cast<float2*>(stat_smem + Cfg::PART_BYTES);
  float* gn_sc = reinterpret_cast<float*>(stat_smem + Cfg::PART_BYTES + Cfg::RUN_BYTES);
  float* gn_sh = gn_sc + kGnMaxC;

  pdl_prologue();
  const int warp = threadIdx.x >> 5;
  const int lane = threadIdx.x & 31;
  const int KB = p.kb0 + p.kb1;
  const int m_tiles = p.tiles_x * p.tiles_y * p.tiles_n;
  const int total_tiles = m_tiles * p.n_tiles;
  const uint32_t rank = PAIR ? cluster_ctarank() : 0u;
  const int n_units = PAIR ? total_tiles / 2 : total_tiles * p.split_k;
  const int n_workers = PAIR ? (int)(gridDim.x / 2) : (int)gridDim.x;
  const int worker = PAIR ? (int)cluster_id_x() : (int)blockIdx.x;
  const int unit_begin = p.deal ? (int)((long long)worker * n_units / n_workers) : worker;
  const int unit_end = p.deal ? (int)((long long)(worker + 1) * n_units / n_workers) : n_units;
  const int unit_step = p.deal ? 1 : n_workers;
  auto k_lo = [&](int u) { return (int)((long long)(u % p.split_k) * KB / p.split_k); };
  auto k_hi = [&](int u) { return (int)((long long)(u % p.split_k + 1) * KB / p.split_k); };
  auto tile_of = [&](int u) {
    if (!PAIR) return u / p.split_k;
    const int mp = u / p.n_tiles;
    return (2 * mp + (int)rank) * p.n_tiles + (u - mp * p.n_tiles);
  };

  if (warp == 8 && lane == 0) {
    if (!GN) {
      tma_prefetch_desc(&tm_a0h);
      tma_prefetch_desc(&tm_a0l);
    }
    tma_prefetch_desc(&tm_bh);
    tma_prefetch_desc(&tm_bl);
    if (p.kb1 && !GN) {
      tma_prefetch_desc(&tm_a1h);
      tma_prefetch_desc(&tm_a1l);
    }
    for (int s = 0; s < STAGES; ++s) {
      mbar_init(full_bar(s), 1);
      mbar_init(empty_bar(s), PAIR ? 16 : 8);
    }
    if (HALO) {
      for (int u = 0; u < HALO_UNITS; ++u) {
        mbar_init(a_full_bar(u), 1);
        mbar_init(a_empty_bar(u), 8);
      }
    }
    mbar_fence_init();
  }
  if (PAIR) cluster_sync_all();
  else __syncthreads();

  auto decode = [&](int tile, int& n_idx, int& x0, int& y0, int& n0) { tc_decode(p, tile, n_idx, x0, y0, n0); };

  if (warp == 8) {
    if (lane == 0) {
      TcRing ring;
      for (int u = unit_begin; u < unit_end; u += unit_step)
        tc_produce_tile<Cfg, PAIR, GN, HALO>(&tm_a0h, &tm_a0l, &tm_a1h, &tm_a1l, &tm_bh, &tm_bl, p, smem_base, bars, tile_of(u), k_lo(u),
                                             k_hi(u), rank, ring);
    }
  } else {
  const int wg = warp >> 2;
  const uint32_t a_row_off = (uint32_t)wg * 64u * 128u;
  const uint32_t halo_row_off = (uint32_t)(((wg * 64) / p.bw) * halo_w + (wg * 64) % p.bw) * 128u;
  const int r0 = warp * 16 + (lane >> 2);
  const int cq = (lane & 3) * 2;
  const int tid = threadIdx.x;
  const int ppi = p.bw * p.bh;
  const int wpi = ppi >= 128 ? 8 : ppi / 16;
  uint32_t stage = 0, phase = 0;
  uint32_t a_done = 0;
  if (p.stats) {
    for (int i = tid; i < 4 * 2 * BN; i += kConsumerThreads) run[i] = make_float2(0.f, 0.f);
  }
  float d[Cfg::ACC];
  const bool dual = DUAL && p.terms != 1;
  int gn_image = -1;
  auto release = [&](int s) {
    if (lane == 0) {
      mbar_arrive(empty_bar(s));
      if (PAIR) mbar_arrive_cluster(empty_bar(s), rank ^ 1u);
    }
  };
  auto release_a = [&](int a) {
    if (lane == 0) mbar_arrive(a_empty_bar(a));
  };
  for (int u = unit_begin; u < unit_end; u += unit_step) {
    const int kb_lo = k_lo(u), kb_hi = k_hi(u);
    int prev = -1;
    int t_nidx, t_x0, t_y0, t_n0;
    decode(tile_of(u), t_nidx, t_x0, t_y0, t_n0);
    if constexpr (GN) {
      if (g.norm && t_n0 != gn_image && t_n0 < p.N) {
        named_bar_sync(1, kConsumerThreads);
        const int cpg = g.C / g.groups;
        const double cnt = (double)p.H * p.W * cpg;
        for (int c = tid; c < g.C; c += kConsumerThreads) {
          const int g0 = (c / cpg) * cpg;
          double s1 = 0, s2 = 0;
          for (int j = 0; j < cpg; ++j) {
            s1 += stat_value(g.st[((size_t)t_n0 * g.st_ld + g0 + j) * 2]);
            s2 += stat_value(g.st[((size_t)t_n0 * g.st_ld + g0 + j) * 2 + 1]);
          }
          const double mean = s1 / cnt;
          double var = s2 / cnt - mean * mean;
          var = var < 0 ? 0 : var;
          const float rstd = (float)(1.0 / sqrt(var + (double)g.eps));
          float a = rstd * g.gamma[c];
          float b = g.beta[c] - (float)mean * a;
          if (g.ss) {
            const float one_plus = 1.0f + g.ss[(size_t)t_n0 * g.ss_ld + c];
            a *= one_plus;
            b = fmaf(b, one_plus, g.ss[(size_t)t_n0 * g.ss_ld + g.C + c]);
          }
          gn_sc[c] = a;
          gn_sh[c] = b;
        }
        named_bar_sync(1, kConsumerThreads);
        gn_image = t_n0;
      }
    }
    for (int kb = kb_lo; kb < kb_hi; ++kb) {
      uint32_t a_base = smem_base + stage * Cfg::STAGE_BYTES + a_row_off;
      uint32_t a_plane = A_PLANE_BYTES;
      uint32_t a_unit = 0;
      bool a_first = false;
      if constexpr (HALO) {
        int ua = 0, dx = 0;
        if (kb < p.kb0) {
          ua = halo_r == 3 ? (int)(__umulhi((uint32_t)kb, 0xAAAAAAABu) >> 1) : kb >> 1;
          dx = kb - ua * halo_r;
        }
        a_unit = a_done + (uint32_t)ua;
        a_first = dx == 0;
        if (a_first) mbar_wait(a_full_bar(a_unit % HALO_UNITS), (a_unit / HALO_UNITS) & 1u);
        a_base = smem_base + (a_unit % HALO_UNITS) * Cfg::A_UNIT_BYTES + (kb < p.kb0 ? halo_row_off + 128u * dx : a_row_off);
        a_plane = HALO_PLANE_BYTES;
      }
      mbar_wait(full_bar(stage), phase);
      const uint32_t sa = smem_base + Cfg::A_RING_BYTES + stage * Cfg::STAGE_BYTES;
      const uint32_t sb = HALO ? sa : sa + 2 * A_PLANE_BYTES;
      if constexpr (GN) {
        const int rr = (tid & 127) >> 1, half = tid & 1, row = wg * 64 + rr;
        float v[32];
        bool valid = t_n0 < p.N;
        const float* src;
        if (kb < p.kb0) {
          const int tap = kb / p.cb0, c0 = (kb - tap * p.cb0) * BK + half * 32;
          const int yy = t_y0 + tap / 3 - 1, xx = t_x0 + row + tap % 3 - 1;
          valid = valid && yy >= 0 && yy < p.H && xx >= 0 && xx < p.W;
          src = g.x + (((long long)t_n0 * p.H + yy) * p.W + xx) * g.x_ld + c0;
          if (valid) {
#pragma unroll
            for (int q = 0; q < 8; ++q) {
              const float4 f = __ldg(reinterpret_cast<const float4*>(src + 4 * q));
              v[4 * q] = f.x; v[4 * q + 1] = f.y; v[4 * q + 2] = f.z; v[4 * q + 3] = f.w;
            }
#pragma unroll
            for (int j = 0; j < 32; ++j) {
              if (g.norm) v[j] = fmaf(v[j], gn_sc[c0 + j], gn_sh[c0 + j]);
              if (g.silu) v[j] = swishf_fast(v[j]);
            }
          }
        } else {
          const int c0 = (kb - p.kb0) * BK + half * 32;
          src = g.xs + (((long long)t_n0 * p.H + t_y0) * p.W + t_x0 + row) * g.xs_ld + c0;
          if (valid) {
#pragma unroll
            for (int q = 0; q < 8; ++q) {
              const float4 f = __ldg(reinterpret_cast<const float4*>(src + 4 * q));
              v[4 * q] = f.x; v[4 * q + 1] = f.y; v[4 * q + 2] = f.z; v[4 * q + 3] = f.w;
            }
          }
        }
        if (!valid) {
#pragma unroll
          for (int j = 0; j < 32; ++j) v[j] = 0.f;
        }
        gn_store_row(smem_raw + (sa - smem_u32(smem_raw)), row, half * 4, v);
        asm volatile("fence.proxy.async.shared::cta;" ::: "memory");
        named_bar_sync(2 + wg, 128);
      }
      const uint64_t ah = wgmma_desc_sw128(a_base);
      const uint64_t al = wgmma_desc_sw128(a_base + a_plane);
      const uint64_t bh = wgmma_desc_sw128(sb);
      const uint64_t bl = wgmma_desc_sw128(sb + Cfg::B_PLANE_BYTES);
      wgmma_fence();
#pragma unroll
      for (int k = 0; k < BK / 16; ++k) {
        const uint64_t adv = 2u * k;
        const uint32_t acc = (uint32_t)(kb != kb_lo || k != 0);
        if (dual) {
          wgmma_tile<DUAL ? 2 * BN : BN>(d, ah + adv, bh + adv, acc);
          wgmma_tile<BN>(d, al + adv, bh + adv, 1u);
        } else {
          wgmma_tile<BN>(d, ah + adv, bh + adv, acc);
          if (p.terms != 1) {
            wgmma_tile<BN>(d, ah + adv, bl + adv, 1u);
            wgmma_tile<BN>(d, al + adv, bh + adv, 1u);
          }
        }
      }
      wgmma_commit();
      wgmma_wait<1>();
      if (prev >= 0) release(prev);
      prev = (int)stage;
      if (++stage == STAGES) {
        stage = 0;
        phase ^= 1u;
      }
      if (HALO && a_first && kb != kb_lo) release_a((a_unit - 1) % HALO_UNITS);
    }
    wgmma_wait<0>();
    if (prev >= 0) release(prev);
    if constexpr (HALO) {
      a_done += p.cb0 * halo_r;
      release_a((a_done - 1) % HALO_UNITS);
    }

    int n_idx, x0, y0, n0;
    decode(tile_of(u), n_idx, x0, y0, n0);
    tc_epilogue_rows<BN, DUAL, NTAIL>(p, d, dual, r0, cq, n_idx, x0, y0, n0, PAIR ? 0 : u % p.split_k);
    if (p.stats) {
      tc_stats_rows<BN>(d, part + warp * BN, lane, cq);
      named_bar_sync(1, kConsumerThreads);
      const int nslots = 8 / wpi;
      bool flush = true;
      if (u + unit_step < unit_end) {
        int nn_idx, nx0, ny0, nn0;
        decode(tile_of(u + unit_step), nn_idx, nx0, ny0, nn0);
        flush = nslots > 1 || nn0 != n0 || nn_idx != n_idx;
      }
      for (int i = tid; i < 2 * BN; i += kConsumerThreads) {
        const int which = i / BN, col = i - which * BN;
        for (int g = 0; g < nslots; ++g) {
          float2& acc = run[(g * 2 + which) * BN + col];
          for (int w = g * wpi; w < (g + 1) * wpi; ++w) {
            const float2 pv = part[w * BN + col];
            two_sum_acc(acc.x, acc.y, which ? pv.y : pv.x);
          }
          if (flush) {
            const int n = n0 + g;
            if (n < p.N) {
              StatAcc* dst = p.stats + ((size_t)n * p.st_ld + n_idx * BN + col) * 2 + which;
              stat_add(dst, acc.x);
              stat_add(dst, acc.y);
            }
            acc = make_float2(0.f, 0.f);
          }
        }
      }
      named_bar_sync(1, kConsumerThreads);
    }
  }
  }
  __syncwarp();
  if (PAIR) cluster_sync_all();
}

static constexpr int kPpThreads = 384;

template <int BN, bool HALO>
struct PpCfg {
  using Ring = TcCfg<BN, false, HALO>;
  static constexpr int PART_BYTES = 8 * BN * 8;
  static constexpr int RUN_BYTES = 2 * BN * 8;
  static constexpr int STAT_BYTES = PART_BYTES + RUN_BYTES;
  static constexpr int SMEM_BYTES = Ring::RING_BYTES + 1024  + 256  + 2 * STAT_BYTES;
  static_assert(SMEM_BYTES <= 227 * 1024, "shared memory capacity");
};

template <int BN, int TERMS, bool HALO, bool NTAIL>
__global__ void __launch_bounds__(kPpThreads, 1)
conv_tc_pingpong_kernel(const __grid_constant__ CUtensorMap tm_a0h, const __grid_constant__ CUtensorMap tm_a0l,
                        const __grid_constant__ CUtensorMap tm_a1h, const __grid_constant__ CUtensorMap tm_a1l,
                        const __grid_constant__ CUtensorMap tm_bh, const __grid_constant__ CUtensorMap tm_bl, const TcParams p) {
  static_assert(TERMS == 1 || TERMS == 3, "1 or 3 fp16 products per MAC");
  using Cfg = PpCfg<BN, HALO>;
  using Ring = typename Cfg::Ring;
  constexpr int STAGES = Ring::STAGES;
  extern __shared__ uint8_t smem_raw[];
  const uint32_t smem_base = (smem_u32(smem_raw) + 1023u) & ~1023u;
  const TcBars<STAGES> bars{smem_base + Ring::RING_BYTES};

  pdl_prologue();
  const int warp = threadIdx.x >> 5;
  const int lane = threadIdx.x & 31;
  const int KB = p.kb0 + p.kb1;
  const int n_units = p.tiles_x * p.tiles_y * p.tiles_n * p.n_tiles * p.split_k;
  const int n_workers = (int)gridDim.x, worker = (int)blockIdx.x;
  const int unit_begin = p.deal ? (int)((long long)worker * n_units / n_workers) : worker;
  const int unit_end = p.deal ? (int)((long long)(worker + 1) * n_units / n_workers) : n_units;
  const int unit_step = p.deal ? 1 : n_workers;
  auto k_lo = [&](int u) { return (int)((long long)(u % p.split_k) * KB / p.split_k); };
  auto k_hi = [&](int u) { return (int)((long long)(u % p.split_k + 1) * KB / p.split_k); };

  if (threadIdx.x == 0) {
    tma_prefetch_desc(&tm_a0h);
    tma_prefetch_desc(&tm_a0l);
    tma_prefetch_desc(&tm_bh);
    tma_prefetch_desc(&tm_bl);
    if (p.kb1) {
      tma_prefetch_desc(&tm_a1h);
      tma_prefetch_desc(&tm_a1l);
    }
    for (int s = 0; s < STAGES; ++s) {
      mbar_init(bars.full(s), 1);
      mbar_init(bars.empty(s), 4);
    }
    if (HALO) {
      for (int u = 0; u < HALO_UNITS; ++u) {
        mbar_init(bars.a_full(u), 1);
        mbar_init(bars.a_empty(u), 4);
      }
    }
    mbar_init(bars.turn(0), 4);
    mbar_init(bars.turn(1), 4);
    mbar_fence_init();
  }
  __syncthreads();

  if (warp < 4) {
    setmaxnreg_dec<40>();
    if (threadIdx.x == 0) {
      TcRing ring;
      for (int u = unit_begin; u < unit_end; u += unit_step)
        tc_produce_tile<Ring, false, false, HALO>(&tm_a0h, &tm_a0l, &tm_a1h, &tm_a1l, &tm_bh, &tm_bl, p, smem_base, bars,
                                                  u / p.split_k, k_lo(u), k_hi(u), 0u, ring);
    }
    return;
  }
  setmaxnreg_inc<232>();
  const int c = (warp >> 2) - 1;
  const int wq = warp & 3;
  const int tid = threadIdx.x - 128 * (c + 1);
  const int r0 = wq * 16 + (lane >> 2);
  const int cq = (lane & 3) * 2;
  const int halo_r = p.mode0 == TAPS_UP2X2 ? 2 : 3;
  const int halo_w = p.bw + halo_r - 1;
  const int units_per_tile = p.cb0 * halo_r;
  uint32_t halo_row_off[2];
#pragma unroll
  for (int f = 0; f < 2; ++f) halo_row_off[f] = (uint32_t)(((f * 64) / p.bw) * halo_w + (f * 64) % p.bw) * 128u;
  const int wpi = p.bw * p.bh >= 128 ? 8 : p.bw * p.bh / 16;
  uint8_t* stat_smem = smem_raw + (bars.base + 256u - smem_u32(smem_raw)) + c * Cfg::STAT_BYTES;
  float2* part = reinterpret_cast<float2*>(stat_smem);
  float2* run = reinterpret_cast<float2*>(stat_smem + Cfg::PART_BYTES);
  if (p.stats) {
    for (int i = tid; i < 2 * BN; i += 128) run[i] = make_float2(0.f, 0.f);
  }
  auto release = [&](int s) {
    if (lane == 0) mbar_arrive(bars.empty(s));
  };
  auto release_a = [&](uint32_t a) {
    if (lane == 0) mbar_arrive(bars.a_empty(a % HALO_UNITS));
  };
  uint32_t kpos = c ? (uint32_t)(k_hi(unit_begin) - k_lo(unit_begin)) : 0u;
  float d[2][BN / 2];
  int turn = 0;
  for (int u = unit_begin + c * unit_step; u < unit_end; u += 2 * unit_step, ++turn) {
    const int kb_lo = k_lo(u), kb_hi = k_hi(u);
    if (c == 1 || turn > 0) mbar_wait(bars.turn(c), (uint32_t)(c ? turn : turn - 1) & 1u);
    uint32_t stage = kpos % STAGES, phase = (kpos / STAGES) & 1u;
    const uint32_t a_done = (uint32_t)((2 * turn + c) * units_per_tile);
    int prev = -1;
    for (int kb = kb_lo; kb < kb_hi; ++kb) {
      const uint32_t sb = smem_base + Ring::A_RING_BYTES + stage * Ring::STAGE_BYTES;
      uint32_t a_base = sb;
      uint32_t a_frag1 = 64u * 128u;
      uint32_t a_plane = A_PLANE_BYTES;
      uint32_t a_unit = 0;
      bool a_first = false;
      if constexpr (HALO) {
        const int ua = halo_r == 3 ? (int)(__umulhi((uint32_t)kb, 0xAAAAAAABu) >> 1) : kb >> 1;
        const int dx = kb - ua * halo_r;
        a_unit = a_done + (uint32_t)ua;
        a_first = dx == 0;
        if (a_first) mbar_wait(bars.a_full(a_unit % HALO_UNITS), (a_unit / HALO_UNITS) & 1u);
        a_base = smem_base + (a_unit % HALO_UNITS) * Ring::A_UNIT_BYTES + halo_row_off[0] + 128u * dx;
        a_frag1 = halo_row_off[1] - halo_row_off[0];
        a_plane = HALO_PLANE_BYTES;
      }
      mbar_wait(bars.full(stage), phase);
      const uint32_t sbb = HALO ? sb : sb + 2 * A_PLANE_BYTES;
      const uint64_t ah0 = wgmma_desc_sw128(a_base), ah1 = wgmma_desc_sw128(a_base + a_frag1);
      const uint64_t al0 = wgmma_desc_sw128(a_base + a_plane), al1 = wgmma_desc_sw128(a_base + a_frag1 + a_plane);
      const uint64_t bh = wgmma_desc_sw128(sbb);
      const uint64_t bl = wgmma_desc_sw128(sbb + Ring::B_PLANE_BYTES);
      wgmma_fence();
#pragma unroll
      for (int k = 0; k < BK / 16; ++k) {
        const uint64_t adv = 2u * k;
        const uint32_t acc = (uint32_t)(kb != kb_lo || k != 0);
        wgmma_tile<BN>(d[0], ah0 + adv, bh + adv, acc);
        wgmma_tile<BN>(d[1], ah1 + adv, bh + adv, acc);
        if constexpr (TERMS == 3) {
          wgmma_tile<BN>(d[0], ah0 + adv, bl + adv, 1u);
          wgmma_tile<BN>(d[1], ah1 + adv, bl + adv, 1u);
          wgmma_tile<BN>(d[0], al0 + adv, bh + adv, 1u);
          wgmma_tile<BN>(d[1], al1 + adv, bh + adv, 1u);
        }
      }
      wgmma_commit();
      wgmma_wait<1>();
      if (prev >= 0) release(prev);
      prev = (int)stage;
      if (++stage == STAGES) {
        stage = 0;
        phase ^= 1u;
      }
      if (HALO && a_first && kb != kb_lo) release_a(a_unit - 1);
    }
    __syncwarp();
    if (lane == 0) mbar_arrive(bars.turn(c ^ 1));
    wgmma_wait<0>();
    if (prev >= 0) release(prev);
    if (HALO) release_a(a_done + units_per_tile - 1);
    kpos += (uint32_t)(kb_hi - kb_lo) + (uint32_t)(k_hi(u + unit_step) - k_lo(u + unit_step));

    int n_idx, x0, y0, n0;
    tc_decode(p, u / p.split_k, n_idx, x0, y0, n0);
#pragma unroll
    for (int f = 0; f < 2; ++f) tc_epilogue_rows<BN, false, NTAIL>(p, d[f], false, 64 * f + r0, cq, n_idx, x0, y0, n0, u % p.split_k);
    if (p.stats) {
#pragma unroll
      for (int f = 0; f < 2; ++f) tc_stats_rows<BN>(d[f], part + (4 * f + wq) * BN, lane, cq);
      named_bar_sync(1 + c, 128);
      const int nslots = 8 / wpi;
      bool flush = true;
      const int un = u + 2 * unit_step;
      if (un < unit_end) {
        int nn_idx, nx0, ny0, nn0;
        tc_decode(p, un / p.split_k, nn_idx, nx0, ny0, nn0);
        flush = nslots > 1 || nn0 != n0 || nn_idx != n_idx;
      }
      for (int i = tid; i < 2 * BN; i += 128) {
        const int which = i / BN, col = i - which * BN;
        for (int g = 0; g < nslots; ++g) {
          float2 acc = nslots == 1 ? run[i] : make_float2(0.f, 0.f);
          for (int w = g * wpi; w < (g + 1) * wpi; ++w) {
            const float2 pv = part[w * BN + col];
            two_sum_acc(acc.x, acc.y, which ? pv.y : pv.x);
          }
          if (flush) {
            const int n = n0 + g;
            if (n < p.N) {
              StatAcc* dst = p.stats + ((size_t)n * p.st_ld + n_idx * BN + col) * 2 + which;
              stat_add(dst, acc.x);
              stat_add(dst, acc.y);
            }
            acc = make_float2(0.f, 0.f);
          }
          if (nslots == 1) run[i] = acc;
        }
      }
      named_bar_sync(1 + c, 128);
    }
  }
}

typedef CUresult (*EncodeTiledFn)(CUtensorMap*, CUtensorMapDataType, cuuint32_t, void*, const cuuint64_t*, const cuuint64_t*,
                                  const cuuint32_t*, const cuuint32_t*, CUtensorMapInterleave, CUtensorMapSwizzle,
                                  CUtensorMapL2promotion, CUtensorMapFloatOOBfill);

static EncodeTiledFn encode_fn() {
  static EncodeTiledFn fn = nullptr;
  if (!fn) {
    void* f = nullptr;
    cudaDriverEntryPointQueryResult q;
    CUDA_CHECK(cudaGetDriverEntryPoint("cuTensorMapEncodeTiled", &f, cudaEnableDefault, &q));
    DDNM_CHECK(f != nullptr && q == cudaDriverEntryPointSuccess, "cuTensorMapEncodeTiled not available");
    fn = reinterpret_cast<EncodeTiledFn>(f);
  }
  return fn;
}

static CUtensorMap make_map_f16(const void* base, int rank, const uint64_t* dims, const uint32_t* box,
                                const uint64_t* strides_elems = nullptr) {
  CUtensorMap m;
  cuuint64_t gdim[5], gstr[4];
  cuuint32_t b[5], es[5];
  uint64_t stride = 2;
  for (int i = 0; i < rank; ++i) {
    gdim[i] = dims[i];
    b[i] = box[i];
// ... 35 lines not shown
static int g_deal = -1;
void tc_debug_deal(int mode) {
  DDNM_CHECK(mode >= -1 && mode <= 1, "deal mode must be -1 (default rule), 0 (round-robin) or 1 (contiguous ranges)");
  g_deal = mode;
}

TcLaunch tc_make_launch(const SplitView& src0, int mode0, const SplitView* src1, const __half* w_hi, const __half* w_lo,
                        int w_batches, int Cout, const View& out, const float* chanadd, int ca_ld, const float* residual,
                        int ldr, float alpha, int num_sms, int res_mode) {
  TcLaunch L;
  TcParams& p = L.p;
  const int taps = (mode0 == TAPS_1X1) ? 1 : (mode0 == TAPS_UP2X2 ? 4 : 9);
  DDNM_CHECK(src0.C % BK == 0, "tensor-core conv needs Cin % 64 == 0");
  DDNM_CHECK(Cout % 64 == 0, "tensor-core conv needs Cout % 64 == 0");
  p.H = out.H; p.W = out.W; p.N = out.N;
  p.bw = out.W >= 128 ? 128 : out.W;
  DDNM_CHECK(128 % p.bw == 0 && out.W % p.bw == 0, "unsupported width for the 128-pixel tile");
  p.bh = std::min(out.H, 128 / p.bw);
  DDNM_CHECK(out.H % p.bh == 0 && 128 % (p.bw * p.bh) == 0, "unsupported height for the 128-pixel tile");
  p.bn = 128 / (p.bw * p.bh);
  p.tiles_x = out.W / p.bw;
  p.tiles_y = out.H / p.bh;
  p.tiles_n = cdiv(out.N, p.bn);
  {
    const int m_tiles = p.tiles_x * p.tiles_y * p.tiles_n;
    L.BN = 64;
    if (Cout % 128 == 0 && (long long)m_tiles * (Cout / 128) >= num_sms / 2) L.BN = 128;
    if (g_force_bn && Cout % g_force_bn == 0) L.BN = g_force_bn;
  }
  p.n_tiles = Cout / L.BN;
  {
    const int m_tiles = p.tiles_x * p.tiles_y * p.tiles_n;
    L.pair = g_pair_mode == 1 && w_batches == 1 && m_tiles % 2 == 0;
  }
  L.dual = g_dual_mode != 0 && (!L.pair || g_pair_dual != 0);
  L.pingpong = g_pingpong_enable != 0;
  p.mode0 = mode0;
  p.cb0 = src0.C / BK;
  p.kb0 = taps * p.cb0;
  p.kb1 = src1 ? src1->C / BK : 0;
  if (src1) DDNM_CHECK(src1->C % BK == 0 && src1->H == out.H && src1->W == out.W && src1->N == out.N, "bad 1x1 side input");
  p.phase_stride = 0;
  p.up_py = p.up_px = 0;
  p.b_batched = w_batches > 1 ? 1 : 0;
  if (p.b_batched) DDNM_CHECK(p.bn == 1 && w_batches == out.N, "batched B operand needs one image per tile");
  if (mode0 == TAPS_3X3_S2) {
    DDNM_CHECK(src0.H == out.H && src0.W == out.W && src0.N == 4 * out.N, "stride-2 source must be 4 parity phases");
    p.phase_stride = out.N;
  } else {
    DDNM_CHECK(src0.H == out.H && src0.W == out.W && src0.N == out.N, "source/output shape mismatch");
  }
  p.Cout = Cout; p.ldc = out.ld; p.out = out.p;
  p.out_sx = out.ld; p.out_sy = (long long)out.W * out.ld; p.out_sn = (long long)out.H * out.W * out.ld;
  DDNM_CHECK(out.C == Cout && out.ld % 2 == 0 && ((uintptr_t)out.p & 7) == 0, "output view misaligned (rows move as float2)");
  p.chanadd = chanadd; p.ca_ld = ca_ld; p.residual = residual; p.ldr = ldr; p.alpha = alpha; p.res_mode = res_mode;
  p.stats = out.st; p.st_ld = out.st_ld;
  p.terms = g_terms;
  if (out.st) DDNM_CHECK(p.bw * p.bh >= 32, "GroupNorm statistics need >= 32 pixels per image");
  if (residual) DDNM_CHECK(ldr % 2 == 0 && ((uintptr_t)residual & 7) == 0, "residual misaligned (rows move as float2)");
  if (chanadd) DDNM_CHECK(ca_ld % 2 == 0 && ((uintptr_t)chanadd & 7) == 0, "channel-add rows misaligned");

  const uint64_t ad[4] = {(uint64_t)src0.C, (uint64_t)src0.W, (uint64_t)src0.H, (uint64_t)src0.N};
  const uint32_t abox[4] = {(uint32_t)BK, (uint32_t)p.bw, (uint32_t)p.bh, (uint32_t)p.bn};
  L.a0h = make_map_f16(src0.hi, 4, ad, abox);
  L.a0l = make_map_f16(src0.lo, 4, ad, abox);
  L.halo = g_halo_enable != 0 && !L.pair && (mode0 == TAPS_3X3 || mode0 == TAPS_UP2X2) && p.bw % 64 == 0 && p.bn == 1 && !src1;
  if (L.halo) {
    const uint32_t hbox[4] = {(uint32_t)BK, (uint32_t)(p.bw + (mode0 == TAPS_UP2X2 ? 1 : 2)), (uint32_t)p.bh, 1u};
    L.hh = make_map_f16(src0.hi, 4, ad, hbox);
    L.hl = make_map_f16(src0.lo, 4, ad, hbox);
  }
  if (src1) {
    const uint64_t ad1[4] = {(uint64_t)src1->C, (uint64_t)src1->W, (uint64_t)src1->H, (uint64_t)src1->N};
    L.a1h = make_map_f16(src1->hi, 4, ad1, abox);
    L.a1l = make_map_f16(src1->lo, 4, ad1, abox);
  } else {
    L.a1h = L.a0h;
    L.a1l = L.a0l;
  }
  const int Ktot = (p.kb0 + p.kb1) * BK;
  const uint64_t bd[3] = {(uint64_t)Ktot, (uint64_t)Cout, (uint64_t)w_batches};
  const uint32_t bbox[3] = {(uint32_t)BK, (uint32_t)(L.pair ? L.BN / 2 : L.BN), 1u};
  L.bh = make_map_f16(w_hi, 3, bd, bbox);
  L.bl = make_map_f16(w_lo, 3, bd, bbox);
  const int total = p.tiles_x * p.tiles_y * p.tiles_n * p.n_tiles;
  L.grid = L.pair ? 2 * std::min(total / 2, num_sms / 2) : std::min(total, num_sms);
  const int units = L.pair ? total / 2 : total, workers = L.pair ? L.grid / 2 : L.grid;
  p.deal = g_deal >= 0 ? g_deal : (out.st != nullptr && p.n_tiles == 1 && units >= 2 * workers ? 1 : 0);
  if (p.n_tiles != 1) p.deal = 0;
  L.flops = 2.0 * (double)out.pixels() * Cout * Ktot;
  return L;
}

TcLaunch tc_make_up2_launch(const SplitView& src, const __half* w_hi, const __half* w_lo, int Cout, const View& out, const float* chanadd,
                            int ca_ld, int py, int px, int num_sms) {
  DDNM_CHECK(out.H == 2 * src.H && out.W == 2 * src.W && out.N == src.N, "upsample phase: output must be twice the source size");
  View lr = out;
  lr.H = src.H;
  lr.W = src.W;
  TcLaunch L = tc_make_launch(src, TAPS_UP2X2, nullptr, w_hi, w_lo, 1, Cout, lr, chanadd, ca_ld, nullptr, 0, 1.0f, num_sms, 0);
  TcParams& p = L.p;
  p.up_py = py;
  p.up_px = px;
  p.out = out.p + ((size_t)py * out.W + px) * out.ld;
  p.out_sx = 2LL * out.ld;
  p.out_sy = 2LL * out.W * out.ld;
  p.out_sn = (long long)out.H * out.W * out.ld;
  return L;
}

TcLaunch tc_make_gemm_launch(const GemmOperand& A, const GemmOperand& B, int M, int N, int K, int heads, int images, float* out,
                             long long out_sn, long long out_sy, long long out_sx, float alpha, int num_sms) {
  TcLaunch L;
  TcParams& p = L.p;
  DDNM_CHECK(M % 128 == 0 && N % 8 == 0 && K % 8 == 0, "attention GEMM: M % 128, N % 8, K % 8");
  p.H = heads; p.W = M; p.N = images;
  p.bw = 128; p.bh = 1; p.bn = 1;
  p.tiles_x = M / 128; p.tiles_y = heads; p.tiles_n = images;
  const int m_tiles = p.tiles_x * p.tiles_y * p.tiles_n;
  L.BN = 64;
  if (N % 128 == 0 && (long long)m_tiles * (N / 128) >= num_sms / 2) L.BN = 128;
  L.dual = g_dual_mode != 0;
  L.pingpong = g_pingpong_enable != 0;
  p.n_tiles = cdiv(N, L.BN);
  L.ntail = N % L.BN != 0;
  p.mode0 = TAPS_1X1;
  p.cb0 = cdiv(K, BK); p.kb0 = p.cb0; p.kb1 = 0;
  p.phase_stride = 0;
  p.up_py = p.up_px = 0;
  p.b_batched = 2;
  p.Cout = N; p.ldc = (int)out_sx; p.out = out;
  p.out_sn = out_sn; p.out_sy = out_sy; p.out_sx = out_sx;
  DDNM_CHECK(out_sx % 2 == 0 && out_sy % 2 == 0 && out_sn % 2 == 0 && ((uintptr_t)out & 7) == 0, "attention GEMM output misaligned");
  p.chanadd = nullptr; p.ca_ld = 0; p.residual = nullptr; p.ldr = 0; p.res_mode = 0; p.alpha = alpha;
  p.stats = nullptr; p.st_ld = 0;
  p.terms = g_terms;
  const uint64_t ad[4] = {(uint64_t)K, (uint64_t)M, (uint64_t)heads, (uint64_t)images};
  const uint64_t as[3] = {(uint64_t)A.s_row, (uint64_t)A.s_head, (uint64_t)A.s_img};
  const uint32_t abox[4] = {(uint32_t)BK, 128u, 1u, 1u};
  L.a0h = make_map_f16(A.hi, 4, ad, abox, as);
  L.a0l = make_map_f16(A.lo, 4, ad, abox, as);
  L.a1h = L.a0h;
  L.a1l = L.a0l;
  const uint64_t bd[4] = {(uint64_t)K, (uint64_t)N, (uint64_t)heads, (uint64_t)images};
  const uint64_t bs[3] = {(uint64_t)B.s_row, (uint64_t)B.s_head, (uint64_t)B.s_img};
  const uint32_t bbox[4] = {(uint32_t)BK, (uint32_t)L.BN, 1u, 1u};
  L.bh = make_map_f16(B.hi, 4, bd, bbox, bs);
  L.bl = make_map_f16(B.lo, 4, bd, bbox, bs);
  L.grid = std::min(m_tiles * p.n_tiles, num_sms);
  L.flops = 2.0 * (double)images * heads * M * (double)N * K;
  return L;
}

template <int BN, bool PAIR, bool DUAL, bool GN = false, bool HALO = false, bool NTAIL = false>
static void launch_bn(const TcLaunch& L, cudaStream_t stream) {
  using Cfg = TcCfg<BN, DUAL, HALO>;
  static bool attr_set[64] = {};
  if (first_use_on_device(attr_set))
    CUDA_CHECK(cudaFuncSetAttribute(conv_tc_kernel<BN, PAIR, DUAL, GN, HALO, NTAIL>, cudaFuncAttributeMaxDynamicSharedMemorySize,
                                    Cfg::SMEM_BYTES));
  launch_pdl(conv_tc_kernel<BN, PAIR, DUAL, GN, HALO, NTAIL>, dim3(L.grid), dim3(kTcThreads), (size_t)Cfg::SMEM_BYTES, stream, PAIR ? 2 : 1,
             HALO ? L.hh : L.a0h, HALO ? L.hl : L.a0l, L.a1h, L.a1l, L.bh, L.bl, L.p, L.g);
  CUDA_CHECK(cudaGetLastError());
}

template <int BN>
static void launch_forms(const TcLaunch& L, cudaStream_t stream) {
  if (L.ntail) {
    if constexpr (BN == 64) {
      if (L.dual) launch_bn<BN, false, true, false, false, true>(L, stream);
      else launch_bn<BN, false, false, false, false, true>(L, stream);
      return;
    }
    throw Error("partial N tiles need BN = 64");
  }
  if (L.halo && L.dual) launch_bn<BN, false, true, false, true>(L, stream);
  else if (L.halo) launch_bn<BN, false, false, false, true>(L, stream);
  else if (L.gn && L.dual) launch_bn<BN, false, true, true>(L, stream);
  else if (L.gn) launch_bn<BN, false, false, true>(L, stream);
  else if (L.pair && L.dual) launch_bn<BN, true, true>(L, stream);
  else if (L.pair) launch_bn<BN, true, false>(L, stream);
  else if (L.dual) launch_bn<BN, false, true>(L, stream);
  else launch_bn<BN, false, false>(L, stream);
}

template <int BN, int TERMS, bool HALO, bool NTAIL = false>
static void launch_pingpong(const TcLaunch& L, cudaStream_t stream) {
  using Cfg = PpCfg<BN, HALO>;
  static bool attr_set[64] = {};
  if (first_use_on_device(attr_set))
    CUDA_CHECK(cudaFuncSetAttribute(conv_tc_pingpong_kernel<BN, TERMS, HALO, NTAIL>, cudaFuncAttributeMaxDynamicSharedMemorySize,
                                    Cfg::SMEM_BYTES));
  launch_pdl(conv_tc_pingpong_kernel<BN, TERMS, HALO, NTAIL>, dim3(L.grid), dim3(kPpThreads), (size_t)Cfg::SMEM_BYTES, stream, 1,
             HALO ? L.hh : L.a0h, HALO ? L.hl : L.a0l, L.a1h, L.a1l, L.bh, L.bl, L.p);
  CUDA_CHECK(cudaGetLastError());
}

template <int BN>
static void launch_pingpong_forms(const TcLaunch& L, cudaStream_t stream) {
  if (L.ntail) {
    if constexpr (BN == 64) {
      if (L.p.terms == 1) launch_pingpong<BN, 1, false, true>(L, stream);
      else launch_pingpong<BN, 3, false, true>(L, stream);
      return;
    }
    throw Error("partial N tiles need BN = 64");
  }
  if (L.p.terms == 1) {
    if (L.halo) launch_pingpong<BN, 1, true>(L, stream);
    else launch_pingpong<BN, 1, false>(L, stream);
  } else {
    if (L.halo) launch_pingpong<BN, 3, true>(L, stream);
    else launch_pingpong<BN, 3, false>(L, stream);
  }
}

static int g_gn_enable = [] { const char* v = std::getenv("DDNM_GN_FUSED"); return v && *v ? std::atoi(v) : 0; }();
void tc_debug_gn_fused(int on) { g_gn_enable = on; }

static bool gn_shape_ok(const View& x, const View* side, int Cout, const View& out) {
  if (out.W % 128 != 0 || x.C % BK != 0 || x.C > kGnMaxC || Cout % 64 != 0) return false;
  if (x.H != out.H || x.W != out.W || x.N != out.N) return false;
  if (x.ld % 4 != 0 || ((uintptr_t)x.p & 15) != 0) return false;
  if (side && (side->C % BK != 0 || side->ld % 4 != 0 || ((uintptr_t)side->p & 15) != 0 || side->H != out.H || side->W != out.W ||
               side->N != out.N))
    return false;
  return true;
}

bool tc_gn_eligible(const View& x, const View* side, int Cout, const View& out) { return g_gn_enable != 0 && gn_shape_ok(x, side, Cout, out); }

TcLaunch tc_make_gn_launch(const View& x, const GnAffine& gn, const View* side, const __half* w_hi, const __half* w_lo, int Cout,
                           const View& out, const float* chanadd, int ca_ld, const float* residual, int ldr, int num_sms) {
  DDNM_CHECK(gn_shape_ok(x, side, Cout, out), "fused GroupNorm convolution: unsupported shape");
  DDNM_CHECK(g_terms == 3, "the fused GroupNorm convolution implements the fp32-grade (3-term) arithmetic only");
  SplitView a;
  a.hi = const_cast<__half*>(w_hi);
  a.lo = const_cast<__half*>(w_lo);
  a.N = x.N; a.H = x.H; a.W = x.W; a.C = x.C;
  SplitView s1;
  if (side) {
    s1 = a;
    s1.C = side->C;
  }
  const int gp = g_pair_mode;
  g_pair_mode = 0;
  TcLaunch L = tc_make_launch(a, TAPS_3X3, side ? &s1 : nullptr, w_hi, w_lo, 1, Cout, out, chanadd, ca_ld, residual, ldr, 1.0f, num_sms, 0);
  g_pair_mode = gp;
  L.gn = true;
  L.halo = false;
  L.dual = L.dual && L.BN == 64;
  TcGnArgs& g = L.g;
  g.x = x.p; g.x_ld = x.ld; g.C = x.C;
  g.xs = side ? side->p : nullptr; g.xs_ld = side ? side->ld : 0;
  g.norm = gn.gamma != nullptr ? 1 : 0;
  if (g.norm) DDNM_CHECK(x.st != nullptr && x.C % gn.groups == 0, "normalisation needs the tensor's per-channel sums (View::st)");
  g.st = x.st; g.st_ld = x.st_ld;
  g.gamma = gn.gamma; g.beta = gn.beta; g.eps = gn.eps; g.groups = gn.groups; g.ss = gn.ss; g.ss_ld = gn.ss_ld; g.silu = gn.silu ? 1 : 0;
  return L;
}

void tc_run(const TcLaunch& L, cudaStream_t stream) {
  DDNM_CHECK(!L.pair || L.p.split_k == 1, "CTA pairs do not split K");
  DDNM_CHECK(!L.halo || (L.p.split_k == 1 && !L.pair && !L.gn && L.p.kb1 == 0),
             "the HALO form runs unsplit single-CTA launches with TMA-loaded A and no 1x1 side input");
  const int units = L.p.tiles_x * L.p.tiles_y * L.p.tiles_n * L.p.n_tiles * L.p.split_k;
  if (L.pingpong && !L.pair && !L.gn && units > L.grid) {
    switch (L.BN) {
      case 128: launch_pingpong_forms<128>(L, stream); return;
      case 64: launch_pingpong_forms<64>(L, stream); return;
      default: throw Error("bad BN");
    }
  }
  switch (L.BN) {
    case 128: launch_forms<128>(L, stream); break;
    case 64: launch_forms<64>(L, stream); break;
    default: throw Error("bad BN");
  }
}

}
```

ddnm_b200/csrc/tc_gemm.cuh:

```cuda
#pragma once
#include "common.cuh"

namespace ddnm {

enum TcTapMode : int {
  TAPS_3X3 = 0,
  TAPS_1X1 = 1,
  TAPS_3X3_S2 = 2,
  TAPS_UP2X2 = 3,
};

struct TcParams {
  int H, W, N;
  int bw, bh, bn;
  int tiles_x, tiles_y, tiles_n;
  int n_tiles;
  int mode0;
  int cb0, kb0;
  int kb1;
  int phase_stride;
  int up_py, up_px;
  int b_batched;
  long long out_sn, out_sy, out_sx;
  int Cout, ldc;
  float* out;
  const float* chanadd;
  int ca_ld;
  const float* residual;
  int ldr;
  int res_mode;
  float alpha;
  StatAcc* stats;
  int st_ld;
  int split_k = 1;
  long long split_stride = 0;
  int deal = 0;
  int terms;
};

struct TcGnArgs {
  const float* x = nullptr;
  int x_ld = 0, C = 0;
  const float* xs = nullptr;
  int xs_ld = 0;
  const StatAcc* st = nullptr;
  int st_ld = 0;
  const float* gamma = nullptr;
  const float* beta = nullptr;
  float eps = 0.f;
  int groups = 32;
  const float* ss = nullptr;
  int ss_ld = 0;
  int silu = 0, norm = 0;
};

struct TcLaunch {
  CUtensorMap a0h, a0l, a1h, a1l, bh, bl;
  CUtensorMap hh, hl;
  TcParams p;
  int BN = 128;
  bool pair = false;
  bool dual = false;
  bool gn = false;
  bool halo = false;
  bool pingpong = false;
  bool ntail = false;
  TcGnArgs g;
  int grid = 0;
  double flops = 0;
};

TcLaunch tc_make_launch(const SplitView& src0, int mode0, const SplitView* src1, const __half* w_hi, const __half* w_lo,
                        int w_batches, int Cout, const View& out, const float* chanadd, int ca_ld, const float* residual,
                        int ldr, float alpha, int num_sms, int res_mode = 0);
void tc_run(const TcLaunch& L, cudaStream_t stream);
TcLaunch tc_make_up2_launch(const SplitView& src, const __half* w_hi, const __half* w_lo, int Cout, const View& out, const float* chanadd,
                            int ca_ld, int py, int px, int num_sms);

struct GemmOperand {
  const __half* hi;
  const __half* lo;
  long long s_row, s_head, s_img;
};
TcLaunch tc_make_gemm_launch(const GemmOperand& A, const GemmOperand& B, int M, int N, int K, int heads, int images, float* out,
                             long long out_sn, long long out_sy, long long out_sx, float alpha, int num_sms);

struct GnAffine {
  const float* gamma = nullptr;
  const float* beta = nullptr;
  float eps = 1e-6f;
  int groups = 32;
  bool silu = true;
  const float* ss = nullptr;
  int ss_ld = 0;
};
bool tc_gn_eligible(const View& x, const View* side, int Cout, const View& out);
TcLaunch tc_make_gn_launch(const View& x, const GnAffine& gn, const View* side, const __half* w_hi, const __half* w_lo, int Cout,
                           const View& out, const float* chanadd, int ca_ld, const float* residual, int ldr, int num_sms);
void tc_debug_gn_fused(int on);

void tc_debug_force_bn(int bn);
void tc_debug_deal(int mode);
void tc_debug_pair_mode(int mode);
void tc_debug_dual_mode(int mode);
void tc_debug_pair_dual(int on);
void tc_debug_halo(int on);
void tc_debug_pingpong(int on);
void tc_set_terms(int terms);
int tc_get_terms();

}
```

ddnm_b200/csrc/unet_openai.cu:

```cuda
#include <algorithm>
#include <cmath>

#include "engine.cuh"
#include "kernels.cuh"

namespace ddnm {

UNetOpenAI::UNetOpenAI(const OpenAICfg& cfg, int batch)
    : UNetEngine(batch, cfg.in_channels, cfg.out_channels, cfg.image_size, cfg.groups, cfg.eps), cfg_(cfg) {
  class_cond_ = cfg.num_classes > 0;
  DDNM_CHECK(cfg.low_res >= 0 && cfg.low_res <= cfg.image_size, "low_res size must be in [0, image_size]");
  lowres_ = cfg.low_res;
}

void UNetOpenAI::emit_resblock(const std::string& p, const View& x, const View& out, int kind) {
  const int Cin = x.C, Cout = out.C;
  DDNM_CHECK((size_t)(out.pixels() * Cout) <= hbuf_elems_, "hbuf too small");
  if (kind != RES_PLAIN) DDNM_CHECK(Cin == Cout, "up/down ResBlocks keep the channel count");
  SplitView A{splitA_hi_, splitA_lo_}, Bs{splitB_hi_, splitB_lo_};
  const int mode1 = kind == RES_DOWN ? SPLIT_AVG2 : SPLIT_SAME;
  const bool has_skip_conv = has_param(p + ".skip_connection.weight");
  View h;
  h.p = hbuf_; h.N = B_; h.H = out.H; h.W = out.W; h.C = Cout; h.ld = Cout;
  h.st = new_stats(Cout); h.st_ld = Cout;
  if (kind == RES_PLAIN && fused_ok(x, nullptr, Cout, h) && fused_ok(h, has_skip_conv ? &x : nullptr, Cout, out)) {
    TcWeights w1 = prep_weights(p + ".in_layers.2.weight", Cout, Cin, 9, "", 0);
    emit_tcgn(p + ".conv1", x, p + ".in_layers.0", nullptr, 0, nullptr, w1, Cout, h, P(p + ".in_layers.2.bias", Cout), 0, nullptr, 0);
    if (has_skip_conv) {
      TcWeights w2 = prep_weights(p + ".out_layers.3.weight", Cout, Cout, 9, p + ".skip_connection.weight", Cin);
      emit_tcgn(p + ".conv2+skip", h, p + ".out_layers.0", ss_all_ + ss_off_.at(p), ss_total_, &x, w2, Cout, out,
                bias_sum(p + ".out_layers.3.bias", p + ".skip_connection.bias", Cout), 0, nullptr, 0);
    } else {
      DDNM_CHECK(Cin == Cout, "identity skip needs equal channels");
      TcWeights w2 = prep_weights(p + ".out_layers.3.weight", Cout, Cout, 9, "", 0);
      emit_tcgn(p + ".conv2", h, p + ".out_layers.0", ss_all_ + ss_off_.at(p), ss_total_, nullptr, w2, Cout, out,
                P(p + ".out_layers.3.bias", Cout), 0, x.p, x.ld);
    }
    return;
  }
  emit_gn_split(p + ".in", x, p + ".in_layers.0", true, mode1, A, nullptr, 0, has_skip_conv ? &Bs : nullptr);
  if (kind == RES_UP) {
    emit_up2_conv(p + ".conv1", A, p + ".in_layers.2.weight", Cout, h, P(p + ".in_layers.2.bias", Cout), 0);
  } else {
    TcWeights w1 = prep_weights(p + ".in_layers.2.weight", Cout, Cin, 9, "", 0);
    emit_tc(p + ".conv1", A, TAPS_3X3, nullptr, w1, Cout, h, P(p + ".in_layers.2.bias", Cout), 0, nullptr, 0);
  }
  emit_gn_split(p + ".out", h, p + ".out_layers.0", true, SPLIT_SAME, A, ss_all_ + ss_off_.at(p), ss_total_);
  if (has_skip_conv) {
    DDNM_CHECK(kind == RES_PLAIN, "skip convolution on an up/down block");
    TcWeights w2 = prep_weights(p + ".out_layers.3.weight", Cout, Cout, 9, p + ".skip_connection.weight", Cin);
    emit_tc(p + ".conv2+skip", A, TAPS_3X3, &Bs, w2, Cout, out, bias_sum(p + ".out_layers.3.bias", p + ".skip_connection.bias", Cout), 0,
            nullptr, 0);
  } else {
    DDNM_CHECK(Cin == Cout, "identity skip needs equal channels");
    TcWeights w2 = prep_weights(p + ".out_layers.3.weight", Cout, Cout, 9, "", 0);
    emit_tc(p + ".conv2", A, TAPS_3X3, nullptr, w2, Cout, out, P(p + ".out_layers.3.bias", Cout), 0, x.p, x.ld,
            kind == RES_UP ? 1 : (kind == RES_DOWN ? 2 : 0));
  }
}

int UNetOpenAI::attn_heads(int C, bool upsample) const {
  int heads = cfg_.num_heads;
  if (cfg_.num_head_channels > 0) heads = C / cfg_.num_head_channels;
  else if (upsample && cfg_.num_heads_upsample > 0) heads = cfg_.num_heads_upsample;
  DDNM_CHECK(heads >= 1 && C % heads == 0 && (cfg_.num_head_channels <= 0 || C % cfg_.num_head_channels == 0),
             "attention channels " + std::to_string(C) + " do not split into equal heads");
  return heads;
}

void UNetOpenAI::emit_attn(const std::string& p, const View& x, const View& out, int heads) {
  const int C = x.C, T = x.H * x.W, ch = C / heads;
  SplitView A{splitA_hi_, splitA_lo_};
  emit_gn_split(p + ".norm", x, p + ".norm", false, SPLIT_SAME, A);
  TcWeights wqkv = prep_weights(p + ".qkv.weight", 3 * C, C, 1, "", 0);
  View qkv;
  qkv.p = qkv_; qkv.N = B_; qkv.H = x.H; qkv.W = x.W; qkv.C = 3 * C; qkv.ld = 3 * C;
  emit_tc(p + ".qkv", A, TAPS_1X1, nullptr, wqkv, 3 * C, qkv, P(p + ".qkv.bias", 3 * C), 0, nullptr, 0);
  const float alpha = 1.0f / std::sqrt((float)ch);
  if (cfg_.new_attention_order) emit_attention_core(p, T, heads, ch, 3 * C, ch, 0, C, 2 * C, alpha);
  else emit_attention_core(p, T, heads, ch, 3 * C, 3 * ch, 0, ch, 2 * ch, alpha);
  View ov;
  ov.p = attO_; ov.N = B_; ov.H = x.H; ov.W = x.W; ov.C = C; ov.ld = C;
  emit_gn_split(p + ".proj_in", ov, "", false, SPLIT_SAME, A);
  TcWeights wp = prep_weights(p + ".proj_out.weight", C, C, 1, "", 0);
  emit_tc(p + ".proj_out", A, TAPS_1X1, nullptr, wp, C, out, P(p + ".proj_out.bias", C), 0, x.p, x.ld);
}

void UNetOpenAI::build_program() {
  const OpenAICfg& c = cfg_;
  const int mc = c.model_channels, R = c.image_size, nrb = c.num_res_blocks, L = c.n_levels;
  DDNM_CHECK(mc % 64 == 0, "model_channels must be a multiple of 64 (tensor-core K blocks)");
  auto attn_at = [&](int ds) {
    for (int i = 0; i < c.n_attn_ds; ++i)
      if (c.attn_ds[i] == ds) return true;
    return false;
  };
  struct Layer { int kind; int cin, cout; };
  struct Block { std::vector<Layer> layers; int res_in, res_out, cout; };
  std::vector<Block> inp, outb;
  std::vector<int> chans, chan_res;
  int ch = c.channel_mult[0] * mc, ds = 1, res = R;
  inp.push_back({{{0, c.in_channels, ch}}, res, res, ch});
  chans.push_back(ch);
  chan_res.push_back(res);
  for (int lv = 0; lv < L; ++lv) {
    for (int i = 0; i < nrb; ++i) {
      Block b{{}, res, res, c.channel_mult[lv] * mc};
      b.layers.push_back({1, ch, c.channel_mult[lv] * mc});
      ch = c.channel_mult[lv] * mc;
      if (attn_at(ds)) b.layers.push_back({4, ch, ch});
      inp.push_back(b);
      chans.push_back(ch);
      chan_res.push_back(res);
    }
    if (lv != L - 1) {
      inp.push_back({{{2, ch, ch}}, res, res / 2, ch});
      res /= 2;
      ds *= 2;
      chans.push_back(ch);
      chan_res.push_back(res);
    }
  }
  const int mid_ch = ch, mid_res = res;
  {
    std::vector<int> cs = chans, rs = chan_res;
    for (int lv = L - 1; lv >= 0; --lv) {
      for (int i = 0; i <= nrb; ++i) {
        const int ich = cs.back();
        DDNM_CHECK(rs.back() == res, "skip resolution mismatch");
        cs.pop_back();
        rs.pop_back();
        Block b{{}, res, res, c.channel_mult[lv] * mc};
        b.layers.push_back({1, ch + ich, c.channel_mult[lv] * mc});
        ch = c.channel_mult[lv] * mc;
        if (attn_at(ds)) b.layers.push_back({4, ch, ch});
        if (lv && i == nrb) {
          b.layers.push_back({3, ch, ch});
          b.res_out = res * 2;
          res *= 2;
          ds /= 2;
        }
        outb.push_back(b);
      }
    }
  }
  const int n_out = (int)outb.size();
  DDNM_CHECK(n_out == (int)inp.size(), "input / output block count mismatch");

  size_t split_max = 0, hbuf_max = 0, att_qkv = 0, att_S = 0, att_O = 0;
  int n_gn = 1;
  std::vector<std::string> rb_names;
  std::vector<int> rb_cout;
  auto plan_layers = [&](const std::string& prefix, const std::vector<Layer>& layers, int r) {
    for (size_t j = 0; j < layers.size(); ++j) {
      const Layer& l = layers[j];
      const std::string p = prefix + "." + std::to_string(j);
      if (l.kind == 1 || l.kind == 2 || l.kind == 3) {
        const int ro = l.kind == 2 ? r / 2 : (l.kind == 3 ? r * 2 : r);
        split_max = std::max(split_max, (size_t)B_ * ro * ro * std::max(l.cin, l.cout));
        split_max = std::max(split_max, (size_t)B_ * r * r * l.cin);
        hbuf_max = std::max(hbuf_max, (size_t)B_ * ro * ro * l.cout);
        n_gn += 2;
        rb_names.push_back(p);
        rb_cout.push_back(l.cout);
        r = ro;
      } else if (l.kind == 4) {
        const size_t T = (size_t)r * r, heads = attn_heads(l.cin, prefix.rfind("output_blocks", 0) == 0);
        split_max = std::max(split_max, (size_t)B_ * T * l.cin);
        att_qkv = std::max(att_qkv, (size_t)B_ * T * 3 * l.cin);
        att_S = std::max(att_S, (size_t)B_ * heads * T * T);
        att_O = std::max(att_O, (size_t)B_ * T * l.cin);
        n_gn += 1;
      }
    }
  };
  for (size_t i = 0; i < inp.size(); ++i) plan_layers("input_blocks." + std::to_string(i), inp[i].layers, inp[i].res_in);
  std::vector<Layer> mid = {{1, mid_ch, mid_ch}, {4, mid_ch, mid_ch}, {1, mid_ch, mid_ch}};
  plan_layers("middle_block", mid, mid_res);
  for (int i = 0; i < n_out; ++i) plan_layers("output_blocks." + std::to_string(i), outb[i].layers, outb[i].res_in);
  alloc_common(split_max, hbuf_max);
  alloc_attention(att_qkv, att_S, att_O);

  const int tdim = mc * 4;
  emb_ = (float*)arena_.alloc((size_t)B_ * mc * 4);
  temb0_ = (float*)arena_.alloc((size_t)B_ * tdim * 4);
  temb_ = (float*)arena_.alloc((size_t)B_ * tdim * 4);
  freq_ = (float*)arena_.alloc((size_t)(mc / 2) * 4);
  CUDA_CHECK(cudaMemcpy(freq_, P("__freq", mc / 2), (mc / 2) * 4, cudaMemcpyDeviceToDevice));
  ss_total_ = 0;
  for (size_t i = 0; i < rb_names.size(); ++i) {
    ss_off_[rb_names[i]] = ss_total_;
    ss_total_ += 2 * rb_cout[i];
  }
  embW_all_ = (float*)arena_.alloc((size_t)ss_total_ * tdim * 4);
  embB_all_ = (float*)arena_.alloc((size_t)ss_total_ * 4);
  ss_all_ = (float*)arena_.alloc((size_t)B_ * ss_total_ * 4);
  for (size_t i = 0; i < rb_names.size(); ++i) {
    const int off = ss_off_[rb_names[i]], n2 = 2 * rb_cout[i];
// ... 77 lines not shown
```

ddnm_b200/csrc/unet_simple.cu:

```cuda
#include <algorithm>
#include <cmath>

#include "engine.cuh"
#include "kernels.cuh"

namespace ddnm {

UNetSimple::UNetSimple(const SimpleCfg& cfg, int batch)
    : UNetEngine(batch, cfg.in_channels, cfg.out_ch, cfg.resolution, cfg.groups, cfg.eps), cfg_(cfg) {}

void UNetSimple::emit_resblock(const std::string& p, const View& x, const View& out) {
  const int Cin = x.C, Cout = out.C;
  DDNM_CHECK((size_t)(x.pixels() * Cout) <= hbuf_elems_, "hbuf too small");
  SplitView A{splitA_hi_, splitA_lo_}, Bs{splitB_hi_, splitB_lo_};
  View h;
  h.p = hbuf_; h.N = B_; h.H = x.H; h.W = x.W; h.C = Cout; h.ld = Cout;
  h.st = new_stats(Cout); h.st_ld = Cout;
  if (fused_ok(x, nullptr, Cout, h) && fused_ok(h, Cin != Cout ? &x : nullptr, Cout, out)) {
    TcWeights w1 = prep_weights(p + ".conv1.weight", Cout, Cin, 9, "", 0);
    emit_tcgn(p + ".conv1", x, p + ".norm1", nullptr, 0, nullptr, w1, Cout, h, ca_all_ + ca_off_.at(p), ca_total_, nullptr, 0);
    if (Cin != Cout) {
      TcWeights w2 = prep_weights(p + ".conv2.weight", Cout, Cout, 9, p + ".nin_shortcut.weight", Cin);
      emit_tcgn(p + ".conv2+nin", h, p + ".norm2", nullptr, 0, &x, w2, Cout, out,
                bias_sum(p + ".conv2.bias", p + ".nin_shortcut.bias", Cout), 0, nullptr, 0);
    } else {
      TcWeights w2 = prep_weights(p + ".conv2.weight", Cout, Cout, 9, "", 0);
      emit_tcgn(p + ".conv2", h, p + ".norm2", nullptr, 0, nullptr, w2, Cout, out, P(p + ".conv2.bias", Cout), 0, x.p, x.ld);
    }
    return;
  }
  emit_gn_split(p + ".norm1", x, p + ".norm1", true, SPLIT_SAME, A, nullptr, 0, Cin != Cout ? &Bs : nullptr);
  TcWeights w1 = prep_weights(p + ".conv1.weight", Cout, Cin, 9, "", 0);
  emit_tc(p + ".conv1", A, TAPS_3X3, nullptr, w1, Cout, h, ca_all_ + ca_off_.at(p), ca_total_, nullptr, 0);
  emit_gn_split(p + ".norm2", h, p + ".norm2", true, SPLIT_SAME, A);
  if (Cin != Cout) {
    TcWeights w2 = prep_weights(p + ".conv2.weight", Cout, Cout, 9, p + ".nin_shortcut.weight", Cin);
    emit_tc(p + ".conv2+nin", A, TAPS_3X3, &Bs, w2, Cout, out, bias_sum(p + ".conv2.bias", p + ".nin_shortcut.bias", Cout), 0,
            nullptr, 0);
  } else {
    TcWeights w2 = prep_weights(p + ".conv2.weight", Cout, Cout, 9, "", 0);
    emit_tc(p + ".conv2", A, TAPS_3X3, nullptr, w2, Cout, out, P(p + ".conv2.bias", Cout), 0, x.p, x.ld);
  }
}

void UNetSimple::emit_attn(const std::string& p, const View& x, const View& out) {
  const int C = x.C, T = x.H * x.W;
  SplitView A{splitA_hi_, splitA_lo_};
  emit_gn_split(p + ".norm", x, p + ".norm", false, SPLIT_SAME, A);
  TcWeights wqkv;
  wqkv.ktot = C;
  wqkv.hi = (__half*)arena_.alloc((size_t)3 * C * C * sizeof(__half));
  wqkv.lo = (__half*)arena_.alloc((size_t)3 * C * C * sizeof(__half));
  std::vector<float> hb(3 * C);
  const char* nm[3] = {".q", ".k", ".v"};
  for (int i = 0; i < 3; ++i) {
    split_conv_weight(P(p + nm[i] + ".weight", (long long)C * C), C, C, 1, wqkv.hi + (size_t)i * C * C, wqkv.lo + (size_t)i * C * C, C, 0, 0);
    CUDA_CHECK(cudaMemcpy(hb.data() + i * C, P(p + nm[i] + ".bias", C), C * sizeof(float), cudaMemcpyDeviceToHost));
  }
  float* bqkv = dev_copy(hb);
  View qkv;
  qkv.p = qkv_; qkv.N = B_; qkv.H = x.H; qkv.W = x.W; qkv.C = 3 * C; qkv.ld = 3 * C;
  emit_tc(p + ".qkv", A, TAPS_1X1, nullptr, wqkv, 3 * C, qkv, bqkv, 0, nullptr, 0);
  emit_attention_core(p, T, 1, C, 3 * C, 0, 0, C, 2 * C, 1.0f / sqrtf((float)C));
  View ov;
  ov.p = attO_; ov.N = B_; ov.H = x.H; ov.W = x.W; ov.C = C; ov.ld = C;
  emit_gn_split(p + ".proj_in", ov, "", false, SPLIT_SAME, A);
  TcWeights wp = prep_weights(p + ".proj_out.weight", C, C, 1, "", 0);
  emit_tc(p + ".proj_out", A, TAPS_1X1, nullptr, wp, C, out, P(p + ".proj_out.bias", C), 0, x.p, x.ld);
}

void UNetSimple::emit_downsample(const std::string& p, const View& x, const View& out) {
  SplitView A{splitA_hi_, splitA_lo_};
  emit_gn_split(p + ".s2d", x, "", false, SPLIT_S2D, A);
  TcWeights w = prep_weights(p + ".conv.weight", x.C, x.C, 9, "", 0);
  emit_tc(p + ".conv", A, TAPS_3X3_S2, nullptr, w, x.C, out, P(p + ".conv.bias", x.C), 0, nullptr, 0);
}

void UNetSimple::emit_upsample(const std::string& p, const View& x, const View& out) {
  SplitView A{splitA_hi_, splitA_lo_};
  emit_gn_split(p + ".split", x, "", false, SPLIT_SAME, A);
  emit_up2_conv(p + ".conv", A, p + ".conv.weight", x.C, out, P(p + ".conv.bias", x.C), 0);
}

void UNetSimple::build_program() {
  const SimpleCfg& c = cfg_;
  const int L = c.n_levels, R = c.resolution, nrb = c.num_res_blocks;
  DDNM_CHECK(c.ch % 64 == 0, "base channel count must be a multiple of 64 (tensor-core K blocks)");
  auto has_attn = [&](int res) {
    for (int i = 0; i < c.n_attn_res; ++i)
      if (c.attn_res[i] == res) return true;
    return false;
  };
  auto mult = [&](int lv) { return c.ch * c.ch_mult[lv]; };
  auto in_mult = [&](int lv) { return lv == 0 ? c.ch : c.ch * c.ch_mult[lv - 1]; };

  struct HS { int res, C; };
  std::vector<HS> hs_shape;
  hs_shape.push_back({R, c.ch});
  {
    int res = R;
    for (int lv = 0; lv < L; ++lv) {
      for (int ib = 0; ib < nrb; ++ib) hs_shape.push_back({res, mult(lv)});
      if (lv != L - 1) {
        res /= 2;
        hs_shape.push_back({res, mult(lv)});
      }
    }
  }
  const int n_up = L * (nrb + 1);
  DDNM_CHECK((int)hs_shape.size() == n_up, "skip stack / up-block count mismatch");
  struct UpB { int lv, ib, res, Ch, Cs, Cout; };
  std::vector<UpB> upb;
  {
    int res = R >> (L - 1);
    int block_in = mult(L - 1);
    for (int lv = L - 1; lv >= 0; --lv) {
      for (int ib = 0; ib <= nrb; ++ib) {
        const int skip = (ib == nrb) ? in_mult(lv) : mult(lv);
        upb.push_back({lv, ib, res, block_in, skip, mult(lv)});
        block_in = mult(lv);
      }
      if (lv != 0) res *= 2;
    }
    for (int u = 0; u < n_up; ++u) {
      const HS& h = hs_shape[n_up - 1 - u];
      DDNM_CHECK(h.res == upb[u].res && h.C == upb[u].Cs, "skip shape does not match its up block");
    }
  }

  size_t split_max = 0, hbuf_max = 0, att_tok = 0, att_c = 0, att_T = 0;
  int n_gn = 0;
  std::vector<std::string> rb_names;
  std::vector<int> rb_cout;
  auto plan_conv_in = [&](int res, int Cin, bool up2) {
    split_max = std::max(split_max, (size_t)B_ * res * res * Cin * (up2 ? 4 : 1));
  };
  auto plan_rb = [&](const std::string& p, int res, int Cin, int Cout) {
    plan_conv_in(res, Cin, false);
    plan_conv_in(res, Cout, false);
    hbuf_max = std::max(hbuf_max, (size_t)B_ * res * res * Cout);
    n_gn += 2;
    rb_names.push_back(p);
    rb_cout.push_back(Cout);
  };
  auto plan_attn = [&](int res, int C) {
    plan_conv_in(res, C, false);
    att_tok = std::max(att_tok, (size_t)res * res);
    att_c = std::max(att_c, (size_t)C);
    att_T = std::max(att_T, (size_t)res * res);
    n_gn += 1;
  };
  {
    int res = R;
    for (int lv = 0; lv < L; ++lv) {
      int cin = in_mult(lv);
      for (int ib = 0; ib < nrb; ++ib) {
        plan_rb("down." + std::to_string(lv) + ".block." + std::to_string(ib), res, cin, mult(lv));
        cin = mult(lv);
        if (has_attn(res)) plan_attn(res, cin);
      }
      if (lv != L - 1) {
        plan_conv_in(res, cin, false);
        res /= 2;
      }
    }
    plan_rb("mid.block_1", res, mult(L - 1), mult(L - 1));
    plan_attn(res, mult(L - 1));
    plan_rb("mid.block_2", res, mult(L - 1), mult(L - 1));
    for (const UpB& u : upb) {
      plan_rb("up." + std::to_string(u.lv) + ".block." + std::to_string(u.ib), u.res, u.Ch + u.Cs, u.Cout);
      if (has_attn(u.res)) plan_attn(u.res, u.Cout);
      if (u.ib == nrb && u.lv != 0) plan_conv_in(u.res, u.Cout, true);
    }
    n_gn += 1;
  }
  alloc_common(split_max, hbuf_max);
  alloc_attention((size_t)B_ * att_tok * 3 * att_c, (size_t)B_ * att_T * att_T, (size_t)B_ * att_tok * att_c);

  const int tch = c.ch * 4;
  emb_ = (float*)arena_.alloc((size_t)B_ * c.ch * 4);
  temb0_ = (float*)arena_.alloc((size_t)B_ * tch * 4);
  temb_ = (float*)arena_.alloc((size_t)B_ * tch * 4);
  freq_ = (float*)arena_.alloc((size_t)(c.ch / 2) * 4);
  CUDA_CHECK(cudaMemcpy(freq_, P("__freq", c.ch / 2), (c.ch / 2) * 4, cudaMemcpyDeviceToDevice));
  ca_total_ = 0;
  for (size_t i = 0; i < rb_names.size(); ++i) {
// ... 105 lines not shown
```

Baseline: 3.103.

## Move fused GroupNorm conv onto ping-pong HALO kernel, drop side-input fusion

Moves the fused GroupNorm+SiLU prologue out of the old single-CTA GN kernel form and into the ping-pong HALO tensor-core kernel. Blocks with a 1x1 side input (nin/skip shortcuts) now fall back to a separate split pass for that path. Eligibility is decided per convolution rather than per resblock, so conv1 and conv2 can each take the fused path on their own. The goal is to keep the halo-reuse ping-pong schedule while skipping the separate normalize-and-split pass over the activations. The trade-off is that shortcut convs and non-eligible shapes lose fusion and pay an extra split pass.

```diff
diff --git a/ddnm_b200/csrc/api.cu b/ddnm_b200/csrc/api.cu
--- a/ddnm_b200/csrc/api.cu
+++ b/ddnm_b200/csrc/api.cu
@@ -1,6 +1,7 @@
 #include "../../include/ddnm_b200.h"
 
 #include <cstring>
+#include <functional>
 #include <vector>
 
 #include "api_util.cuh"
@@ -452,25 +453,42 @@
   xv.st = st;
   xv.st_ld = Cin;
   if (gamma) gn_stats(xv, s);
-  View sv;
-  if (side_x) sv = mkview(const_cast<float*>(side_x), N, H, W, CinSide);
   const int ktot = 9 * Cin + (side_x ? CinSide : 0);
   __half* wh = tmp.get<__half>((size_t)Cout * ktot);
   __half* wl = tmp.get<__half>((size_t)Cout * ktot);
   split_conv_weight(w, Cout, Cin, 9, wh, wl, ktot, 0, s);
   if (side_x) split_conv_weight(side_w, Cout, CinSide, 1, wh, wl, ktot, 9 * Cin, s);
-  GnAffine gn;
-  gn.gamma = gamma; gn.beta = beta; gn.eps = eps; gn.groups = groups; gn.silu = silu != 0;
   View ov = mkview(out, N, H, W, Cout);
-  TcLaunch L = tc_make_gn_launch(xv, gn, side_x ? &sv : nullptr, wh, wl, Cout, ov, bias, 0, residual, Cout, sm_count());
-  tc_run(L, s);
+  std::function<void()> run;
+  if (!side_x && tc_gn_applies(xv, Cout, ov, sm_count())) {
+    GnAffine gn;
+    gn.gamma = gamma; gn.beta = beta; gn.eps = eps; gn.groups = groups; gn.silu = silu != 0;
+    const TcLaunch L = tc_make_gn_launch(xv, gn, wh, wl, Cout, ov, bias, 0, residual, Cout, sm_count());
+    run = [L, s] { tc_run(L, s); };
+  } else {
+    const size_t pe = (size_t)N * H * W * Cin;
+    SplitView A, S;
+    A.hi = tmp.get<__half>(pe); A.lo = tmp.get<__half>(pe); A.N = N; A.H = H; A.W = W; A.C = Cin;
+    if (side_x) {
+      const size_t se = (size_t)N * H * W * CinSide;
+      S.hi = tmp.get<__half>(se); S.lo = tmp.get<__half>(se); S.N = N; S.H = H; S.W = W; S.C = CinSide;
+    }
+    const TcLaunch L = tc_make_launch(A, TAPS_3X3, side_x ? &S : nullptr, wh, wl, 1, Cout, ov, bias, 0, residual, Cout, 1.0f, sm_count());
+    const View sv = mkview(const_cast<float*>(side_x), N, H, W, CinSide);
+    run = [=] {
+      gn_apply_split(xv, groups, gamma != nullptr, gamma, beta, eps, silu != 0, SPLIT_SAME, A.hi, A.lo, s);
+      if (side_x) gn_apply_split(sv, 1, false, nullptr, nullptr, 0.f, false, SPLIT_SAME, S.hi, S.lo, s);
+      tc_run(L, s);
+    };
+  }
+  run();
   if (iters > 0 && ms_per_iter) {
     cudaEvent_t e0, e1;
     CUDA_CHECK(cudaEventCreate(&e0));
     CUDA_CHECK(cudaEventCreate(&e1));
-    for (int i = 0; i < 2; ++i) tc_run(L, s);
+    for (int i = 0; i < 2; ++i) run();
     CUDA_CHECK(cudaEventRecord(e0, s));
-    for (int i = 0; i < iters; ++i) tc_run(L, s);
+    for (int i = 0; i < iters; ++i) run();
     CUDA_CHECK(cudaEventRecord(e1, s));
     CUDA_CHECK(cudaEventSynchronize(e1));
     float ms = 0;
diff --git a/ddnm_b200/csrc/common.cuh b/ddnm_b200/csrc/common.cuh
--- a/ddnm_b200/csrc/common.cuh
+++ b/ddnm_b200/csrc/common.cuh
@@ -259,6 +259,29 @@
 __device__ __forceinline__ double stat_value(const StatAcc& a) {
   return ((double)a.hi * 4294967296.0 + (double)a.lo) * (1.0 / 281474976710656.0);
 }
+template <class Sum>
+__device__ __forceinline__ void gn_channel_affine(Sum sum, int c, int cpg, double cnt, float eps, const float* gamma, const float* beta,
+                                                  const float* ss_row, int C, float& scale, float& shift) {
+  const int g0 = (c / cpg) * cpg;
+  double s1 = 0, s2 = 0;
+  for (int j = 0; j < cpg; ++j) {
+    s1 += sum(2 * (g0 + j));
+    s2 += sum(2 * (g0 + j) + 1);
+  }
+  const double mean = s1 / cnt;
+  double var = s2 / cnt - mean * mean;
+  var = var < 0 ? 0 : var;
+  const float rstd = (float)(1.0 / sqrt(var + (double)eps));
+  float a = rstd * gamma[c];
+  float b = beta[c] - (float)mean * a;
+  if (ss_row) {
+    const float one_plus = 1.0f + ss_row[c];
+    a *= one_plus;
+    b = fmaf(b, one_plus, ss_row[C + c]);
+  }
+  scale = a;
+  shift = b;
+}
 
 __device__ __forceinline__ float swishf_fast(float x) {
   float e;
diff --git a/ddnm_b200/csrc/engine.cu b/ddnm_b200/csrc/engine.cu
--- a/ddnm_b200/csrc/engine.cu
+++ b/ddnm_b200/csrc/engine.cu
@@ -173,12 +173,12 @@
   add_op(name, "tc", L.flops, bytes, [L](cudaStream_t s) { tc_run(L, s); });
 }
 
-bool UNetEngine::fused_ok(const View& x, const View* side, int Cout, const View& out) const {
-  return terms_ == 3 && x.st != nullptr && tc_gn_eligible(x, side, Cout, out);
-}
-
-void UNetEngine::emit_tcgn(const std::string& name, const View& x, const std::string& norm, const float* ss, int ss_ld, const View* side,
-                           const TcWeights& w, int Cout, const View& out, const float* chanadd, int ca_ld, const float* residual, int ldr) {
+bool UNetEngine::fused_ok(const View& x, int Cout, const View& out) const {
+  return terms_ == 3 && x.st != nullptr && tc_gn_eligible(x, Cout, out, num_sms_);
+}
+
+void UNetEngine::emit_tcgn(const std::string& name, const View& x, const std::string& norm, const float* ss, int ss_ld, const TcWeights& w,
+                           int Cout, const View& out, const float* chanadd, int ca_ld, const float* residual, int ldr) {
   GnAffine gn;
   gn.gamma = P(norm + ".weight", x.C);
   gn.beta = P(norm + ".bias", x.C);
@@ -187,9 +187,8 @@
   gn.silu = true;
   gn.ss = ss;
   gn.ss_ld = ss_ld;
-  TcLaunch L = tc_make_gn_launch(x, gn, side, w.hi, w.lo, Cout, out, chanadd, ca_ld, residual, ldr, num_sms_);
-  const double bytes = (double)x.pixels() * x.C * 4 + (side ? (double)side->pixels() * side->C * 4 : 0) + (double)Cout * w.ktot * 4 +
-                       (double)out.pixels() * Cout * 4 * (residual ? 2 : 1);
+  TcLaunch L = tc_make_gn_launch(x, gn, w.hi, w.lo, Cout, out, chanadd, ca_ld, residual, ldr, num_sms_);
+  const double bytes = (double)x.pixels() * x.C * 4 + (double)Cout * w.ktot * 4 + (double)out.pixels() * Cout * 4 * (residual ? 2 : 1);
   add_op(name, "tc", L.flops, bytes, [L](cudaStream_t s) { tc_run(L, s); });
 }
 
diff --git a/ddnm_b200/csrc/engine.cuh b/ddnm_b200/csrc/engine.cuh
--- a/ddnm_b200/csrc/engine.cuh
+++ b/ddnm_b200/csrc/engine.cuh
@@ -96,9 +96,9 @@
                      const float* ss = nullptr, int ss_ld = 0, SplitView* raw = nullptr);
   void emit_tc(const std::string& name, const SplitView& a, int mode, const SplitView* side, const TcWeights& w, int Cout,
                const View& out, const float* chanadd, int ca_ld, const float* residual, int ldr, int res_mode = 0);
-  bool fused_ok(const View& x, const View* side, int Cout, const View& out) const;
-  void emit_tcgn(const std::string& name, const View& x, const std::string& norm, const float* ss, int ss_ld, const View* side,
-                 const TcWeights& w, int Cout, const View& out, const float* chanadd, int ca_ld, const float* residual, int ldr);
+  bool fused_ok(const View& x, int Cout, const View& out) const;
+  void emit_tcgn(const std::string& name, const View& x, const std::string& norm, const float* ss, int ss_ld, const TcWeights& w,
+                 int Cout, const View& out, const float* chanadd, int ca_ld, const float* residual, int ldr);
   void emit_attention_core(const std::string& name, int T, int heads, int ch, int qkv_ld, int head_stride, int q_off, int k_off,
                            int v_off, float alpha);
   void alloc_attention(size_t qkv_elems, size_t s_elems, size_t o_elems);
diff --git a/ddnm_b200/csrc/kernels.cu b/ddnm_b200/csrc/kernels.cu
--- a/ddnm_b200/csrc/kernels.cu
+++ b/ddnm_b200/csrc/kernels.cu
@@ -92,27 +92,9 @@
     const StatAcc* gsrc = stats + (size_t)n * st_ld * 2;
     for (int c = threadIdx.x; c < 2 * C; c += blockDim.x) sd[c] = stat_value(gsrc[c]);
     __syncthreads();
-    for (int c = threadIdx.x; c < C; c += blockDim.x) {
-      const int g0 = (c / cpg) * cpg;
-      double s1 = 0, s2 = 0;
-      for (int j = 0; j < cpg; ++j) {
-        s1 += sd[2 * (g0 + j)];
-        s2 += sd[2 * (g0 + j) + 1];
-      }
-      const double mean = s1 / cnt;
-      double var = s2 / cnt - mean * mean;
-      var = var < 0 ? 0 : var;
-      const float rstd = (float)(1.0 / sqrt(var + (double)eps));
-      float a = rstd * gamma[c];
-      float b = beta[c] - (float)mean * a;
-      if (ss) {
-        const float one_plus = 1.0f + ss[(size_t)n * ss_ld + c];
-        a *= one_plus;
-        b = fmaf(b, one_plus, ss[(size_t)n * ss_ld + C + c]);
-      }
-      sc[c] = a;
-      sh[c] = b;
-    }
+    const float* ss_row = ss ? ss + (size_t)n * ss_ld : nullptr;
+    for (int c = threadIdx.x; c < C; c += blockDim.x)
+      gn_channel_affine([&](int k) { return sd[k]; }, c, cpg, cnt, eps, gamma, beta, ss_row, C, sc[c], sh[c]);
   } else {
     for (int c = threadIdx.x; c < C; c += blockDim.x) {
       sc[c] = 1.f;
diff --git a/ddnm_b200/csrc/tc_gemm.cu b/ddnm_b200/csrc/tc_gemm.cu
--- a/ddnm_b200/csrc/tc_gemm.cu
+++ b/ddnm_b200/csrc/tc_gemm.cu
@@ -24,8 +24,7 @@
   static constexpr int RING_BYTES = A_RING_BYTES + STAGES * STAGE_BYTES;
   static constexpr int PART_BYTES = 8 * BN * 8;
   static constexpr int RUN_BYTES = 4 * 2 * BN * 8;
-  static constexpr int GN_BYTES = 2 * kGnMaxC * 4;
-  static constexpr int SMEM_BYTES = RING_BYTES + 1024  + 256  + PART_BYTES + RUN_BYTES + GN_BYTES;
+  static constexpr int SMEM_BYTES = RING_BYTES + 1024  + 256  + PART_BYTES + RUN_BYTES;
   static constexpr int ACC = DUAL ? BN : BN / 2;
   static_assert(SMEM_BYTES <= 227 * 1024, "shared memory capacity");
 };
@@ -36,20 +35,6 @@
   if constexpr (N == 64) wgmma_m64n64k16(*reinterpret_cast<float(*)[32]>(&d[0]), a, b, accumulate);
   else if constexpr (N == 128) wgmma_m64n128k16(*reinterpret_cast<float(*)[64]>(&d[0]), a, b, accumulate);
   else wgmma_m64n256k16(*reinterpret_cast<float(*)[128]>(&d[0]), a, b, accumulate);
-}
-
-__device__ __forceinline__ void gn_store_row(uint8_t* a_hi, int row, int chunk0, const float (&v)[32]) {
-#pragma unroll
-  for (int q = 0; q < 4; ++q) {
-    uint4 h, l;
-    split2_f16(v[8 * q + 0], v[8 * q + 1], h.x, l.x);
-    split2_f16(v[8 * q + 2], v[8 * q + 3], h.y, l.y);
-    split2_f16(v[8 * q + 4], v[8 * q + 5], h.z, l.z);
-    split2_f16(v[8 * q + 6], v[8 * q + 7], h.w, l.w);
-    const int off = row * 128 + (((chunk0 + q) ^ (row & 7)) << 4);
-    *reinterpret_cast<uint4*>(a_hi + off) = h;
-    *reinterpret_cast<uint4*>(a_hi + A_PLANE_BYTES + off) = l;
-  }
 }
 
 __device__ __forceinline__ void tc_decode(const TcParams& p, int tile, int& n_idx, int& x0, int& y0, int& n0) {
@@ -88,7 +73,8 @@
   const int halo_w = p.bw + halo_r - 1;
   const bool lo = p.terms != 1;
   const uint32_t planes = lo ? 2u : 1u;
-  const uint32_t stage_tx = (GN || HALO) ? planes * Cfg::B_PLANE_BYTES : (uint32_t)(lo ? Cfg::STAGE_BYTES : Cfg::STAGE_BYTES / 2);
+  static_assert(!GN || HALO, "the GN form builds HALO units");
+  const uint32_t stage_tx = HALO ? planes * Cfg::B_PLANE_BYTES : (uint32_t)(lo ? Cfg::STAGE_BYTES : Cfg::STAGE_BYTES / 2);
   int n_idx, x0, y0, n0;
   tc_decode(p, tile, n_idx, x0, y0, n0);
   const int bz = p.b_batched == 1 ? n0 : 0;
@@ -97,7 +83,7 @@
     if constexpr (HALO) {
       const int ua = kb / halo_r, dx = kb - ua * halo_r, dy = ua / p.cb0, cs = ua - dy * p.cb0;
       bkb = (dy * halo_r + dx) * p.cb0 + cs;
-      if (dx == 0) {
+      if (!GN && dx == 0) {
         mbar_wait(bars.a_empty(r.aunit), r.aphase ^ 1u);
         const uint32_t ua_s = smem_base + r.aunit * Cfg::A_UNIT_BYTES;
         const uint32_t fa = bars.a_full(r.aunit);
@@ -118,7 +104,7 @@
     const uint32_t sb = HALO ? sa : sa + 2 * A_PLANE_BYTES;
     const uint32_t fb = bars.full(r.stage);
     mbar_expect_tx(fb, stage_tx);
-    if (GN || HALO) {
+    if (HALO) {
     } else if (kb < p.kb0) {
       const int tap = kb / p.cb0;
       const int c = (kb - tap * p.cb0) * BK;
@@ -247,14 +233,12 @@
   }
 }
 
-template <int BN, bool PAIR, bool DUAL, bool GN, bool HALO, bool NTAIL>
+template <int BN, bool PAIR, bool DUAL, bool HALO, bool NTAIL>
 __global__ void __launch_bounds__(kTcThreads, 1)
 conv_tc_kernel(const __grid_constant__ CUtensorMap tm_a0h, const __grid_constant__ CUtensorMap tm_a0l,
                const __grid_constant__ CUtensorMap tm_a1h, const __grid_constant__ CUtensorMap tm_a1l,
-               const __grid_constant__ CUtensorMap tm_bh, const __grid_constant__ CUtensorMap tm_bl, const TcParams p,
-               const TcGnArgs g) {
-  static_assert(!GN || !PAIR, "the GN form runs on single CTAs");
-  static_assert(!HALO || (!PAIR && !GN), "the HALO form runs on single CTAs with TMA-loaded A");
+               const __grid_constant__ CUtensorMap tm_bh, const __grid_constant__ CUtensorMap tm_bl, const TcParams p) {
+  static_assert(!HALO || !PAIR, "the HALO form runs on single CTAs");
   using Cfg = TcCfg<BN, DUAL, HALO>;
   constexpr int STAGES = Cfg::STAGES;
   extern __shared__ uint8_t smem_raw[];
@@ -270,8 +254,6 @@
   uint8_t* stat_smem = smem_raw + (bar_base + 256u - smem_u32(smem_raw));
   float2* part = reinterpret_cast<float2*>(stat_smem);
   float2* run = reinterpret_cast<float2*>(stat_smem + Cfg::PART_BYTES);
-  float* gn_sc = reinterpret_cast<float*>(stat_smem + Cfg::PART_BYTES + Cfg::RUN_BYTES);
-  float* gn_sh = gn_sc + kGnMaxC;
 
   pdl_prologue();
   const int warp = threadIdx.x >> 5;
@@ -295,13 +277,11 @@
   };
 
   if (warp == 8 && lane == 0) {
-    if (!GN) {
-      tma_prefetch_desc(&tm_a0h);
-      tma_prefetch_desc(&tm_a0l);
-    }
+    tma_prefetch_desc(&tm_a0h);
+    tma_prefetch_desc(&tm_a0l);
     tma_prefetch_desc(&tm_bh);
     tma_prefetch_desc(&tm_bl);
-    if (p.kb1 && !GN) {
+    if (p.kb1) {
       tma_prefetch_desc(&tm_a1h);
       tma_prefetch_desc(&tm_a1l);
     }
@@ -326,7 +306,7 @@
     if (lane == 0) {
       TcRing ring;
       for (int u = unit_begin; u < unit_end; u += unit_step)
-        tc_produce_tile<Cfg, PAIR, GN, HALO>(&tm_a0h, &tm_a0l, &tm_a1h, &tm_a1l, &tm_bh, &tm_bl, p, smem_base, bars, tile_of(u), k_lo(u),
+        tc_produce_tile<Cfg, PAIR, false, HALO>(&tm_a0h, &tm_a0l, &tm_a1h, &tm_a1l, &tm_bh, &tm_bl, p, smem_base, bars, tile_of(u), k_lo(u),
                                              k_hi(u), rank, ring);
     }
   } else {
@@ -345,7 +325,6 @@
   }
   float d[Cfg::ACC];
   const bool dual = DUAL && p.terms != 1;
-  int gn_image = -1;
   auto release = [&](int s) {
     if (lane == 0) {
       mbar_arrive(empty_bar(s));
@@ -358,38 +337,6 @@
   for (int u = unit_begin; u < unit_end; u += unit_step) {
     const int kb_lo = k_lo(u), kb_hi = k_hi(u);
     int prev = -1;
-    int t_nidx, t_x0, t_y0, t_n0;
-    decode(tile_of(u), t_nidx, t_x0, t_y0, t_n0);
-    if constexpr (GN) {
-      if (g.norm && t_n0 != gn_image && t_n0 < p.N) {
-        named_bar_sync(1, kConsumerThreads);
-        const int cpg = g.C / g.groups;
-        const double cnt = (double)p.H * p.W * cpg;
-        for (int c = tid; c < g.C; c += kConsumerThreads) {
-          const int g0 = (c / cpg) * cpg;
-          double s1 = 0, s2 = 0;
-          for (int j = 0; j < cpg; ++j) {
-            s1 += stat_value(g.st[((size_t)t_n0 * g.st_ld + g0 + j) * 2]);
-            s2 += stat_value(g.st[((size_t)t_n0 * g.st_ld + g0 + j) * 2 + 1]);
-          }
-          const double mean = s1 / cnt;
-          double var = s2 / cnt - mean * mean;
-          var = var < 0 ? 0 : var;
-          const float rstd = (float)(1.0 / sqrt(var + (double)g.eps));
-          float a = rstd * g.gamma[c];
-          float b = g.beta[c] - (float)mean * a;
-          if (g.ss) {
-            const float one_plus = 1.0f + g.ss[(size_t)t_n0 * g.ss_ld + c];
-            a *= one_plus;
-            b = fmaf(b, one_plus, g.ss[(size_t)t_n0 * g.ss_ld + g.C + c]);
-          }
-          gn_sc[c] = a;
-          gn_sh[c] = b;
-        }
-        named_bar_sync(1, kConsumerThreads);
-        gn_image = t_n0;
-      }
-    }
     for (int kb = kb_lo; kb < kb_hi; ++kb) {
       uint32_t a_base = smem_base + stage * Cfg::STAGE_BYTES + a_row_off;
       uint32_t a_plane = A_PLANE_BYTES;
@@ -410,47 +357,6 @@
       mbar_wait(full_bar(stage), phase);
       const uint32_t sa = smem_base + Cfg::A_RING_BYTES + stage * Cfg::STAGE_BYTES;
       const uint32_t sb = HALO ? sa : sa + 2 * A_PLANE_BYTES;
-      if constexpr (GN) {
-        const int rr = (tid & 127) >> 1, half = tid & 1, row = wg * 64 + rr;
-        float v[32];
-        bool valid = t_n0 < p.N;
-        const float* src;
-        if (kb < p.kb0) {
-          const int tap = kb / p.cb0, c0 = (kb - tap * p.cb0) * BK + half * 32;
-          const int yy = t_y0 + tap / 3 - 1, xx = t_x0 + row + tap % 3 - 1;
-          valid = valid && yy >= 0 && yy < p.H && xx >= 0 && xx < p.W;
-          src = g.x + (((long long)t_n0 * p.H + yy) * p.W + xx) * g.x_ld + c0;
-          if (valid) {
-#pragma unroll
-            for (int q = 0; q < 8; ++q) {
-              const float4 f = __ldg(reinterpret_cast<const float4*>(src + 4 * q));
-              v[4 * q] = f.x; v[4 * q + 1] = f.y; v[4 * q + 2] = f.z; v[4 * q + 3] = f.w;
-            }
-#pragma unroll
-            for (int j = 0; j < 32; ++j) {
-              if (g.norm) v[j] = fmaf(v[j], gn_sc[c0 + j], gn_sh[c0 + j]);
-              if (g.silu) v[j] = swishf_fast(v[j]);
-            }
-          }
-        } else {
-          const int c0 = (kb - p.kb0) * BK + half * 32;
-          src = g.xs + (((long long)t_n0 * p.H + t_y0) * p.W + t_x0 + row) * g.xs_ld + c0;
-          if (valid) {
-#pragma unroll
-            for (int q = 0; q < 8; ++q) {
-              const float4 f = __ldg(reinterpret_cast<const float4*>(src + 4 * q));
-              v[4 * q] = f.x; v[4 * q + 1] = f.y; v[4 * q + 2] = f.z; v[4 * q + 3] = f.w;
-            }
-          }
-        }
-        if (!valid) {
-#pragma unroll
-          for (int j = 0; j < 32; ++j) v[j] = 0.f;
-        }
-        gn_store_row(smem_raw + (sa - smem_u32(smem_raw)), row, half * 4, v);
-        asm volatile("fence.proxy.async.shared::cta;" ::: "memory");
-        named_bar_sync(2 + wg, 128);
-      }
       const uint64_t ah = wgmma_desc_sw128(a_base);
       const uint64_t al = wgmma_desc_sw128(a_base + a_plane);
       const uint64_t bh = wgmma_desc_sw128(sb);
@@ -529,24 +435,142 @@
 }
 
 static constexpr int kPpThreads = 384;
-
-template <int BN, bool HALO>
+static constexpr int kGnThreads = 96;
+static constexpr int kGnInFlight = 4;
+
+__device__ __forceinline__ void prefetch_l2(const void* ptr) { asm volatile("prefetch.global.L2 [%0];" ::"l"(ptr)); }
+
+template <int STAGES>
+__device__ __forceinline__ void gn_build_units(const TcParams& p, const TcGnArgs& g, uint8_t* ring, TcBars<STAGES> bars, float* gsc,
+                                               int unit_begin, int unit_end, int unit_step, int t) {
+  float* gsh = gsc + kGnMaxC;
+  const int lane = t & 31;
+  const int halo_w = p.bw + 2;
+  const int rows = halo_w * p.bh;
+  const int items = rows * 8;
+  const int upt = 3 * p.cb0;
+  const float* x = g.x;
+  auto source = [&](int u, int ua, const float*& src, int& cy, int& cx, int& c0) {
+    int n_idx, x0, y0, n0;
+    tc_decode(p, u, n_idx, x0, y0, n0);
+    const int dy = ua / p.cb0;
+    cy = y0 + dy - 1;
+    cx = x0 - 1;
+    c0 = (ua - dy * p.cb0) * BK;
+    src = x + ((((long long)n0 * p.H + cy) * p.W + cx) * g.x_ld + c0);
+  };
+  if (!g.norm) {
+    for (int c = t; c < g.C; c += kGnThreads) {
+      gsc[c] = 1.f;
+      gsh[c] = 0.f;
+    }
+    named_bar_sync(3, kGnThreads);
+  }
+  int img = -1;
+  uint32_t unit = 0;
+  for (int u = unit_begin; u < unit_end; u += unit_step) {
+    if (g.norm) {
+      int n_idx, x0, y0, n0;
+      tc_decode(p, u, n_idx, x0, y0, n0);
+      if (n0 != img) {
+        named_bar_sync(3, kGnThreads);
+        const StatAcc* st = g.st + (size_t)n0 * g.st_ld * 2;
+        const int cpg = g.C / g.groups;
+        const double cnt = (double)p.H * p.W * cpg;
+        const float* ss_row = g.ss ? g.ss + (size_t)n0 * g.ss_ld : nullptr;
+        for (int c = t; c < g.C; c += kGnThreads)
+          gn_channel_affine([&](int k) { return stat_value(st[k]); }, c, cpg, cnt, g.eps, g.gamma, g.beta, ss_row, g.C, gsc[c], gsh[c]);
+        named_bar_sync(3, kGnThreads);
+        img = n0;
+      }
+    }
+    for (int ua = 0; ua < upt; ++ua, ++unit) {
+      int cy, cx, c0;
+      const float* src;
+      {
+        int nu = u, nua = ua + 1;
+        if (nua == upt) {
+          nu += unit_step;
+          nua = 0;
+        }
+        if (nu < unit_end) {
+          source(nu, nua, src, cy, cx, c0);
+          for (int i = t; i < 2 * rows; i += kGnThreads) {
+            const int r = i >> 1, yi = r >= halo_w ? 1 : 0, xi = r - yi * halo_w;
+            if (cy + yi >= 0 && cy + yi < p.H && cx + xi >= 0 && cx + xi < p.W) prefetch_l2(src + (yi * p.W + xi) * g.x_ld + (i & 1) * 32);
+          }
+        }
+      }
+      source(u, ua, src, cy, cx, c0);
+      const uint32_t slot = unit % HALO_UNITS;
+      mbar_wait(bars.a_empty(slot), ((unit / HALO_UNITS) & 1u) ^ 1u);
+      uint8_t* a_hi = ring + slot * (2 * HALO_PLANE_BYTES);
+      for (int i0 = t; i0 < items; i0 += kGnInFlight * kGnThreads) {
+        float4 v[kGnInFlight][2];
+        bool in[kGnInFlight];
+#pragma unroll
+        for (int k = 0; k < kGnInFlight; ++k) {
+          const int i = i0 + k * kGnThreads;
+          const int r = i >> 3, yi = r >= halo_w ? 1 : 0, xi = r - yi * halo_w;
+          in[k] = i < items && cy + yi >= 0 && cy + yi < p.H && cx + xi >= 0 && cx + xi < p.W;
+          v[k][0] = v[k][1] = make_float4(0.f, 0.f, 0.f, 0.f);
+          if (in[k]) {
+            const float* s = src + (yi * p.W + xi) * g.x_ld + (i & 7) * 8;
+            v[k][0] = __ldg(reinterpret_cast<const float4*>(s));
+            v[k][1] = __ldg(reinterpret_cast<const float4*>(s + 4));
+          }
+        }
+#pragma unroll
+        for (int k = 0; k < kGnInFlight; ++k) {
+          const int i = i0 + k * kGnThreads;
+          if (i < items) {
+            const int r = i >> 3, q = i & 7, c = c0 + q * 8;
+            uint4 h = make_uint4(0u, 0u, 0u, 0u), l = h;
+            if (in[k]) {
+              float f[8] = {v[k][0].x, v[k][0].y, v[k][0].z, v[k][0].w, v[k][1].x, v[k][1].y, v[k][1].z, v[k][1].w};
+#pragma unroll
+              for (int j = 0; j < 8; ++j) {
+                f[j] = fmaf(f[j], gsc[c + j], gsh[c + j]);
+                if (g.silu) f[j] = swishf_fast(f[j]);
+              }
+              split2_f16(f[0], f[1], h.x, l.x);
+              split2_f16(f[2], f[3], h.y, l.y);
+              split2_f16(f[4], f[5], h.z, l.z);
+              split2_f16(f[6], f[7], h.w, l.w);
+            }
+            const int off = r * 128 + ((q ^ (r & 7)) << 4);
+            *reinterpret_cast<uint4*>(a_hi + off) = h;
+            *reinterpret_cast<uint4*>(a_hi + HALO_PLANE_BYTES + off) = l;
+          }
+        }
+      }
+      asm volatile("fence.proxy.async.shared::cta;" ::: "memory");
+      __syncwarp();
+      if (lane == 0) mbar_arrive(bars.a_full(slot));
+    }
+  }
+}
+
+template <int BN, bool HALO, bool GN = false>
 struct PpCfg {
   using Ring = TcCfg<BN, false, HALO>;
   static constexpr int PART_BYTES = 8 * BN * 8;
   static constexpr int RUN_BYTES = 2 * BN * 8;
   static constexpr int STAT_BYTES = PART_BYTES + RUN_BYTES;
-  static constexpr int SMEM_BYTES = Ring::RING_BYTES + 1024  + 256  + 2 * STAT_BYTES;
+  static constexpr int GN_BYTES = GN ? 2 * kGnMaxC * 4 : 0;
+  static constexpr int SMEM_BYTES = Ring::RING_BYTES + 1024  + 256  + 2 * STAT_BYTES + GN_BYTES;
   static_assert(SMEM_BYTES <= 227 * 1024, "shared memory capacity");
 };
 
-template <int BN, int TERMS, bool HALO, bool NTAIL>
+template <int BN, int TERMS, bool HALO, bool NTAIL, bool GN>
 __global__ void __launch_bounds__(kPpThreads, 1)
 conv_tc_pingpong_kernel(const __grid_constant__ CUtensorMap tm_a0h, const __grid_constant__ CUtensorMap tm_a0l,
                         const __grid_constant__ CUtensorMap tm_a1h, const __grid_constant__ CUtensorMap tm_a1l,
-                        const __grid_constant__ CUtensorMap tm_bh, const __grid_constant__ CUtensorMap tm_bl, const TcParams p) {
+                        const __grid_constant__ CUtensorMap tm_bh, const __grid_constant__ CUtensorMap tm_bl, const TcParams p,
+                        const TcGnArgs g) {
   static_assert(TERMS == 1 || TERMS == 3, "1 or 3 fp16 products per MAC");
-  using Cfg = PpCfg<BN, HALO>;
+  static_assert(!GN || (HALO && TERMS == 3 && !NTAIL), "the GN form builds fp32-grade HALO units");
+  using Cfg = PpCfg<BN, HALO, GN>;
   using Ring = typename Cfg::Ring;
   constexpr int STAGES = Ring::STAGES;
   extern __shared__ uint8_t smem_raw[];
@@ -566,8 +590,10 @@
   auto k_hi = [&](int u) { return (int)((long long)(u % p.split_k + 1) * KB / p.split_k); };
 
   if (threadIdx.x == 0) {
-    tma_prefetch_desc(&tm_a0h);
-    tma_prefetch_desc(&tm_a0l);
+    if (!GN) {
+      tma_prefetch_desc(&tm_a0h);
+      tma_prefetch_desc(&tm_a0l);
+    }
     tma_prefetch_desc(&tm_bh);
     tma_prefetch_desc(&tm_bl);
     if (p.kb1) {
@@ -580,7 +606,7 @@
     }
     if (HALO) {
       for (int u = 0; u < HALO_UNITS; ++u) {
-        mbar_init(bars.a_full(u), 1);
+        mbar_init(bars.a_full(u), GN ? kGnThreads / 32 : 1);
         mbar_init(bars.a_empty(u), 4);
       }
     }
@@ -591,16 +617,21 @@
   __syncthreads();
 
   if (warp < 4) {
-    setmaxnreg_dec<40>();
+    if constexpr (GN) setmaxnreg_dec<80>();
+    else setmaxnreg_dec<40>();
     if (threadIdx.x == 0) {
       TcRing ring;
       for (int u = unit_begin; u < unit_end; u += unit_step)
-        tc_produce_tile<Ring, false, false, HALO>(&tm_a0h, &tm_a0l, &tm_a1h, &tm_a1l, &tm_bh, &tm_bl, p, smem_base, bars,
-                                                  u / p.split_k, k_lo(u), k_hi(u), 0u, ring);
+        tc_produce_tile<Ring, false, GN, HALO>(&tm_a0h, &tm_a0l, &tm_a1h, &tm_a1l, &tm_bh, &tm_bl, p, smem_base, bars,
+                                               u / p.split_k, k_lo(u), k_hi(u), 0u, ring);
+    } else if (GN && warp > 0) {
+      float* gsc = reinterpret_cast<float*>(smem_raw + (bars.base + 256u - smem_u32(smem_raw)) + 2 * Cfg::STAT_BYTES);
+      gn_build_units(p, g, smem_raw + (smem_base - smem_u32(smem_raw)), bars, gsc, unit_begin, unit_end, unit_step, threadIdx.x - 32);
     }
     return;
   }
-  setmaxnreg_inc<232>();
+  if constexpr (GN) setmaxnreg_inc<208>();
+  else setmaxnreg_inc<232>();
   const int c = (warp >> 2) - 1;
   const int wq = warp & 3;
   const int tid = threadIdx.x - 128 * (c + 1);
@@ -942,15 +973,15 @@
   return L;
 }
 
-template <int BN, bool PAIR, bool DUAL, bool GN = false, bool HALO = false, bool NTAIL = false>
+template <int BN, bool PAIR, bool DUAL, bool HALO = false, bool NTAIL = false>
 static void launch_bn(const TcLaunch& L, cudaStream_t stream) {
   using Cfg = TcCfg<BN, DUAL, HALO>;
   static bool attr_set[64] = {};
   if (first_use_on_device(attr_set))
-    CUDA_CHECK(cudaFuncSetAttribute(conv_tc_kernel<BN, PAIR, DUAL, GN, HALO, NTAIL>, cudaFuncAttributeMaxDynamicSharedMemorySize,
+    CUDA_CHECK(cudaFuncSetAttribute(conv_tc_kernel<BN, PAIR, DUAL, HALO, NTAIL>, cudaFuncAttributeMaxDynamicSharedMemorySize,
                                     Cfg::SMEM_BYTES));
-  launch_pdl(conv_tc_kernel<BN, PAIR, DUAL, GN, HALO, NTAIL>, dim3(L.grid), dim3(kTcThreads), (size_t)Cfg::SMEM_BYTES, stream, PAIR ? 2 : 1,
-             HALO ? L.hh : L.a0h, HALO ? L.hl : L.a0l, L.a1h, L.a1l, L.bh, L.bl, L.p, L.g);
+  launch_pdl(conv_tc_kernel<BN, PAIR, DUAL, HALO, NTAIL>, dim3(L.grid), dim3(kTcThreads), (size_t)Cfg::SMEM_BYTES, stream, PAIR ? 2 : 1,
+             HALO ? L.hh : L.a0h, HALO ? L.hl : L.a0l, L.a1h, L.a1l, L.bh, L.bl, L.p);
   CUDA_CHECK(cudaGetLastError());
 }
 
@@ -958,31 +989,29 @@
 static void launch_forms(const TcLaunch& L, cudaStream_t stream) {
   if (L.ntail) {
     if constexpr (BN == 64) {
-      if (L.dual) launch_bn<BN, false, true, false, false, true>(L, stream);
-      else launch_bn<BN, false, false, false, false, true>(L, stream);
+      if (L.dual) launch_bn<BN, false, true, false, true>(L, stream);
+      else launch_bn<BN, false, false, false, true>(L, stream);
       return;
     }
     throw Error("partial N tiles need BN = 64");
   }
-  if (L.halo && L.dual) launch_bn<BN, false, true, false, true>(L, stream);
-  else if (L.halo) launch_bn<BN, false, false, false, true>(L, stream);
-  else if (L.gn && L.dual) launch_bn<BN, false, true, true>(L, stream);
-  else if (L.gn) launch_bn<BN, false, false, true>(L, stream);
+  if (L.halo && L.dual) launch_bn<BN, false, true, true>(L, stream);
+  else if (L.halo) launch_bn<BN, false, false, true>(L, stream);
   else if (L.pair && L.dual) launch_bn<BN, true, true>(L, stream);
   else if (L.pair) launch_bn<BN, true, false>(L, stream);
   else if (L.dual) launch_bn<BN, false, true>(L, stream);
   else launch_bn<BN, false, false>(L, stream);
 }
 
-template <int BN, int TERMS, bool HALO, bool NTAIL = false>
+template <int BN, int TERMS, bool HALO, bool NTAIL = false, bool GN = false>
 static void launch_pingpong(const TcLaunch& L, cudaStream_t stream) {
-  using Cfg = PpCfg<BN, HALO>;
+  using Cfg = PpCfg<BN, HALO, GN>;
   static bool attr_set[64] = {};
   if (first_use_on_device(attr_set))
-    CUDA_CHECK(cudaFuncSetAttribute(conv_tc_pingpong_kernel<BN, TERMS, HALO, NTAIL>, cudaFuncAttributeMaxDynamicSharedMemorySize,
+    CUDA_CHECK(cudaFuncSetAttribute(conv_tc_pingpong_kernel<BN, TERMS, HALO, NTAIL, GN>, cudaFuncAttributeMaxDynamicSharedMemorySize,
                                     Cfg::SMEM_BYTES));
-  launch_pdl(conv_tc_pingpong_kernel<BN, TERMS, HALO, NTAIL>, dim3(L.grid), dim3(kPpThreads), (size_t)Cfg::SMEM_BYTES, stream, 1,
-             HALO ? L.hh : L.a0h, HALO ? L.hl : L.a0l, L.a1h, L.a1l, L.bh, L.bl, L.p);
+  launch_pdl(conv_tc_pingpong_kernel<BN, TERMS, HALO, NTAIL, GN>, dim3(L.grid), dim3(kPpThreads), (size_t)Cfg::SMEM_BYTES, stream, 1,
+             HALO ? L.hh : L.a0h, HALO ? L.hl : L.a0l, L.a1h, L.a1l, L.bh, L.bl, L.p, L.g);
   CUDA_CHECK(cudaGetLastError());
 }
 
@@ -996,6 +1025,10 @@
     }
     throw Error("partial N tiles need BN = 64");
   }
+  if (L.gn) {
+    launch_pingpong<BN, 3, true, false, true>(L, stream);
+    return;
+  }
   if (L.p.terms == 1) {
     if (L.halo) launch_pingpong<BN, 1, true>(L, stream);
     else launch_pingpong<BN, 1, false>(L, stream);
@@ -1008,41 +1041,41 @@
 static int g_gn_enable = [] { const char* v = std::getenv("DDNM_GN_FUSED"); return v && *v ? std::atoi(v) : 0; }();
 void tc_debug_gn_fused(int on) { g_gn_enable = on; }
 
-static bool gn_shape_ok(const View& x, const View* side, int Cout, const View& out) {
-  if (out.W % 128 != 0 || x.C % BK != 0 || x.C > kGnMaxC || Cout % 64 != 0) return false;
+static bool gn_plan(const View& x, int Cout, const View& out, const __half* w_hi, const __half* w_lo, const float* chanadd, int ca_ld,
+                    const float* residual, int ldr, int num_sms, TcLaunch& L) {
+  const int bw = std::min(out.W, 128);
+  if (bw % 64 != 0 || out.W % bw != 0 || out.H % (128 / bw) != 0) return false;
+  if (x.C % BK != 0 || x.C > kGnMaxC || Cout % 64 != 0 || g_terms != 3) return false;
   if (x.H != out.H || x.W != out.W || x.N != out.N) return false;
   if (x.ld % 4 != 0 || ((uintptr_t)x.p & 15) != 0) return false;
-  if (side && (side->C % BK != 0 || side->ld % 4 != 0 || ((uintptr_t)side->p & 15) != 0 || side->H != out.H || side->W != out.W ||
-               side->N != out.N))
-    return false;
-  return true;
-}
-
-bool tc_gn_eligible(const View& x, const View* side, int Cout, const View& out) { return g_gn_enable != 0 && gn_shape_ok(x, side, Cout, out); }
-
-TcLaunch tc_make_gn_launch(const View& x, const GnAffine& gn, const View* side, const __half* w_hi, const __half* w_lo, int Cout,
-                           const View& out, const float* chanadd, int ca_ld, const float* residual, int ldr, int num_sms) {
-  DDNM_CHECK(gn_shape_ok(x, side, Cout, out), "fused GroupNorm convolution: unsupported shape");
-  DDNM_CHECK(g_terms == 3, "the fused GroupNorm convolution implements the fp32-grade (3-term) arithmetic only");
   SplitView a;
   a.hi = const_cast<__half*>(w_hi);
   a.lo = const_cast<__half*>(w_lo);
   a.N = x.N; a.H = x.H; a.W = x.W; a.C = x.C;
-  SplitView s1;
-  if (side) {
-    s1 = a;
-    s1.C = side->C;
-  }
   const int gp = g_pair_mode;
   g_pair_mode = 0;
-  TcLaunch L = tc_make_launch(a, TAPS_3X3, side ? &s1 : nullptr, w_hi, w_lo, 1, Cout, out, chanadd, ca_ld, residual, ldr, 1.0f, num_sms, 0);
+  L = tc_make_launch(a, TAPS_3X3, nullptr, w_hi, w_lo, 1, Cout, out, chanadd, ca_ld, residual, ldr, 1.0f, num_sms, 0);
   g_pair_mode = gp;
+  const int units = L.p.tiles_x * L.p.tiles_y * L.p.tiles_n * L.p.n_tiles;
+  return L.halo && L.pingpong && units > L.grid && L.p.mode0 == TAPS_3X3;
+}
+
+bool tc_gn_applies(const View& x, int Cout, const View& out, int num_sms) {
+  TcLaunch L;
+  const __half* w = reinterpret_cast<const __half*>(x.p);
+  return gn_plan(x, Cout, out, w, w, nullptr, 0, nullptr, 0, num_sms, L);
+}
+
+bool tc_gn_eligible(const View& x, int Cout, const View& out, int num_sms) { return g_gn_enable != 0 && tc_gn_applies(x, Cout, out, num_sms); }
+
+TcLaunch tc_make_gn_launch(const View& x, const GnAffine& gn, const __half* w_hi, const __half* w_lo, int Cout, const View& out,
+                           const float* chanadd, int ca_ld, const float* residual, int ldr, int num_sms) {
+  TcLaunch L;
+  DDNM_CHECK(gn_plan(x, Cout, out, w_hi, w_lo, chanadd, ca_ld, residual, ldr, num_sms, L),
+             "fused GroupNorm convolution: not a ping-pong HALO launch (see tc_gn_applies)");
   L.gn = true;
-  L.halo = false;
-  L.dual = L.dual && L.BN == 64;
   TcGnArgs& g = L.g;
   g.x = x.p; g.x_ld = x.ld; g.C = x.C;
-  g.xs = side ? side->p : nullptr; g.xs_ld = side ? side->ld : 0;
   g.norm = gn.gamma != nullptr ? 1 : 0;
   if (g.norm) DDNM_CHECK(x.st != nullptr && x.C % gn.groups == 0, "normalisation needs the tensor's per-channel sums (View::st)");
   g.st = x.st; g.st_ld = x.st_ld;
@@ -1052,10 +1085,11 @@
 
 void tc_run(const TcLaunch& L, cudaStream_t stream) {
   DDNM_CHECK(!L.pair || L.p.split_k == 1, "CTA pairs do not split K");
-  DDNM_CHECK(!L.halo || (L.p.split_k == 1 && !L.pair && !L.gn && L.p.kb1 == 0),
-             "the HALO form runs unsplit single-CTA launches with TMA-loaded A and no 1x1 side input");
+  DDNM_CHECK(!L.halo || (L.p.split_k == 1 && !L.pair && L.p.kb1 == 0),
+             "the HALO form runs unsplit single-CTA launches with no 1x1 side input");
   const int units = L.p.tiles_x * L.p.tiles_y * L.p.tiles_n * L.p.n_tiles * L.p.split_k;
-  if (L.pingpong && !L.pair && !L.gn && units > L.grid) {
+  DDNM_CHECK(!L.gn || (L.halo && L.pingpong && units > L.grid), "the GN form runs on the ping-pong HALO kernel");
+  if (L.pingpong && !L.pair && units > L.grid) {
     switch (L.BN) {
       case 128: launch_pingpong_forms<128>(L, stream); return;
       case 64: launch_pingpong_forms<64>(L, stream); return;
diff --git a/ddnm_b200/csrc/tc_gemm.cuh b/ddnm_b200/csrc/tc_gemm.cuh
--- a/ddnm_b200/csrc/tc_gemm.cuh
+++ b/ddnm_b200/csrc/tc_gemm.cuh
@@ -41,8 +41,6 @@
 struct TcGnArgs {
   const float* x = nullptr;
   int x_ld = 0, C = 0;
-  const float* xs = nullptr;
-  int xs_ld = 0;
   const StatAcc* st = nullptr;
   int st_ld = 0;
   const float* gamma = nullptr;
@@ -94,9 +92,10 @@
   const float* ss = nullptr;
   int ss_ld = 0;
 };
-bool tc_gn_eligible(const View& x, const View* side, int Cout, const View& out);
-TcLaunch tc_make_gn_launch(const View& x, const GnAffine& gn, const View* side, const __half* w_hi, const __half* w_lo, int Cout,
-                           const View& out, const float* chanadd, int ca_ld, const float* residual, int ldr, int num_sms);
+bool tc_gn_applies(const View& x, int Cout, const View& out, int num_sms);
+bool tc_gn_eligible(const View& x, int Cout, const View& out, int num_sms);
+TcLaunch tc_make_gn_launch(const View& x, const GnAffine& gn, const __half* w_hi, const __half* w_lo, int Cout, const View& out,
+                           const float* chanadd, int ca_ld, const float* residual, int ldr, int num_sms);
 void tc_debug_gn_fused(int on);
 
 void tc_debug_force_bn(int bn);
diff --git a/ddnm_b200/csrc/unet_openai.cu b/ddnm_b200/csrc/unet_openai.cu
--- a/ddnm_b200/csrc/unet_openai.cu
+++ b/ddnm_b200/csrc/unet_openai.cu
@@ -23,27 +23,25 @@
   View h;
   h.p = hbuf_; h.N = B_; h.H = out.H; h.W = out.W; h.C = Cout; h.ld = Cout;
   h.st = new_stats(Cout); h.st_ld = Cout;
-  if (kind == RES_PLAIN && fused_ok(x, nullptr, Cout, h) && fused_ok(h, has_skip_conv ? &x : nullptr, Cout, out)) {
+  if (kind == RES_PLAIN && fused_ok(x, Cout, h)) {
     TcWeights w1 = prep_weights(p + ".in_layers.2.weight", Cout, Cin, 9, "", 0);
-    emit_tcgn(p + ".conv1", x, p + ".in_layers.0", nullptr, 0, nullptr, w1, Cout, h, P(p + ".in_layers.2.bias", Cout), 0, nullptr, 0);
-    if (has_skip_conv) {
-      TcWeights w2 = prep_weights(p + ".out_layers.3.weight", Cout, Cout, 9, p + ".skip_connection.weight", Cin);
-      emit_tcgn(p + ".conv2+skip", h, p + ".out_layers.0", ss_all_ + ss_off_.at(p), ss_total_, &x, w2, Cout, out,
-                bias_sum(p + ".out_layers.3.bias", p + ".skip_connection.bias", Cout), 0, nullptr, 0);
+    emit_tcgn(p + ".conv1", x, p + ".in_layers.0", nullptr, 0, w1, Cout, h, P(p + ".in_layers.2.bias", Cout), 0, nullptr, 0);
+    if (has_skip_conv) emit_gn_split(p + ".skip_in", x, "", false, SPLIT_SAME, Bs);
+  } else {
+    emit_gn_split(p + ".in", x, p + ".in_layers.0", true, mode1, A, nullptr, 0, has_skip_conv ? &Bs : nullptr);
+    if (kind == RES_UP) {
+      emit_up2_conv(p + ".conv1", A, p + ".in_layers.2.weight", Cout, h, P(p + ".in_layers.2.bias", Cout), 0);
     } else {
-      DDNM_CHECK(Cin == Cout, "identity skip needs equal channels");
-      TcWeights w2 = prep_weights(p + ".out_layers.3.weight", Cout, Cout, 9, "", 0);
-      emit_tcgn(p + ".conv2", h, p + ".out_layers.0", ss_all_ + ss_off_.at(p), ss_total_, nullptr, w2, Cout, out,
-                P(p + ".out_layers.3.bias", Cout), 0, x.p, x.ld);
-    }
+      TcWeights w1 = prep_weights(p + ".in_layers.2.weight", Cout, Cin, 9, "", 0);
+      emit_tc(p + ".conv1", A, TAPS_3X3, nullptr, w1, Cout, h, P(p + ".in_layers.2.bias", Cout), 0, nullptr, 0);
+    }
+  }
+  if (kind == RES_PLAIN && !has_skip_conv && fused_ok(h, Cout, out)) {
+    DDNM_CHECK(Cin == Cout, "identity skip needs equal channels");
+    TcWeights w2 = prep_weights(p + ".out_layers.3.weight", Cout, Cout, 9, "", 0);
+    emit_tcgn(p + ".conv2", h, p + ".out_layers.0", ss_all_ + ss_off_.at(p), ss_total_, w2, Cout, out, P(p + ".out_layers.3.bias", Cout), 0,
+              x.p, x.ld);
     return;
-  }
-  emit_gn_split(p + ".in", x, p + ".in_layers.0", true, mode1, A, nullptr, 0, has_skip_conv ? &Bs : nullptr);
-  if (kind == RES_UP) {
-    emit_up2_conv(p + ".conv1", A, p + ".in_layers.2.weight", Cout, h, P(p + ".in_layers.2.bias", Cout), 0);
-  } else {
-    TcWeights w1 = prep_weights(p + ".in_layers.2.weight", Cout, Cin, 9, "", 0);
-    emit_tc(p + ".conv1", A, TAPS_3X3, nullptr, w1, Cout, h, P(p + ".in_layers.2.bias", Cout), 0, nullptr, 0);
   }
   emit_gn_split(p + ".out", h, p + ".out_layers.0", true, SPLIT_SAME, A, ss_all_ + ss_off_.at(p), ss_total_);
   if (has_skip_conv) {
diff --git a/ddnm_b200/csrc/unet_simple.cu b/ddnm_b200/csrc/unet_simple.cu
--- a/ddnm_b200/csrc/unet_simple.cu
+++ b/ddnm_b200/csrc/unet_simple.cu
@@ -16,22 +16,19 @@
   View h;
   h.p = hbuf_; h.N = B_; h.H = x.H; h.W = x.W; h.C = Cout; h.ld = Cout;
   h.st = new_stats(Cout); h.st_ld = Cout;
-  if (fused_ok(x, nullptr, Cout, h) && fused_ok(h, Cin != Cout ? &x : nullptr, Cout, out)) {
-    TcWeights w1 = prep_weights(p + ".conv1.weight", Cout, Cin, 9, "", 0);
-    emit_tcgn(p + ".conv1", x, p + ".norm1", nullptr, 0, nullptr, w1, Cout, h, ca_all_ + ca_off_.at(p), ca_total_, nullptr, 0);
-    if (Cin != Cout) {
-      TcWeights w2 = prep_weights(p + ".conv2.weight", Cout, Cout, 9, p + ".nin_shortcut.weight", Cin);
-      emit_tcgn(p + ".conv2+nin", h, p + ".norm2", nullptr, 0, &x, w2, Cout, out,
-                bias_sum(p + ".conv2.bias", p + ".nin_shortcut.bias", Cout), 0, nullptr, 0);
-    } else {
-      TcWeights w2 = prep_weights(p + ".conv2.weight", Cout, Cout, 9, "", 0);
-      emit_tcgn(p + ".conv2", h, p + ".norm2", nullptr, 0, nullptr, w2, Cout, out, P(p + ".conv2.bias", Cout), 0, x.p, x.ld);
-    }
+  TcWeights w1 = prep_weights(p + ".conv1.weight", Cout, Cin, 9, "", 0);
+  if (fused_ok(x, Cout, h)) {
+    emit_tcgn(p + ".conv1", x, p + ".norm1", nullptr, 0, w1, Cout, h, ca_all_ + ca_off_.at(p), ca_total_, nullptr, 0);
+    if (Cin != Cout) emit_gn_split(p + ".nin_in", x, "", false, SPLIT_SAME, Bs);
+  } else {
+    emit_gn_split(p + ".norm1", x, p + ".norm1", true, SPLIT_SAME, A, nullptr, 0, Cin != Cout ? &Bs : nullptr);
+    emit_tc(p + ".conv1", A, TAPS_3X3, nullptr, w1, Cout, h, ca_all_ + ca_off_.at(p), ca_total_, nullptr, 0);
+  }
+  if (Cin == Cout && fused_ok(h, Cout, out)) {
+    TcWeights w2 = prep_weights(p + ".conv2.weight", Cout, Cout, 9, "", 0);
+    emit_tcgn(p + ".conv2", h, p + ".norm2", nullptr, 0, w2, Cout, out, P(p + ".conv2.bias", Cout), 0, x.p, x.ld);
     return;
   }
-  emit_gn_split(p + ".norm1", x, p + ".norm1", true, SPLIT_SAME, A, nullptr, 0, Cin != Cout ? &Bs : nullptr);
-  TcWeights w1 = prep_weights(p + ".conv1.weight", Cout, Cin, 9, "", 0);
-  emit_tc(p + ".conv1", A, TAPS_3X3, nullptr, w1, Cout, h, ca_all_ + ca_off_.at(p), ca_total_, nullptr, 0);
   emit_gn_split(p + ".norm2", h, p + ".norm2", true, SPLIT_SAME, A);
   if (Cin != Cout) {
     TcWeights w2 = prep_weights(p + ".conv2.weight", Cout, Cout, 9, p + ".nin_shortcut.weight", Cin);
```

After: 3.101 (median of 6 runs). Within noise of the previous version (-0.1%).
